# cchao0116/EasyDGL

Hardware: AMD Instinct MI355X
Metric: sequences/sec (fwd+bwd+Adam) B=512 L=100 d=128 |I|=20K (higher is better)
Workload: dtype bf16

## Files before the change

easydgl_amd/_lib.py:

```python
from __future__ import annotations

import ctypes
import os
from ctypes import c_char_p, c_float, c_int, c_int64, c_long, c_uint32, c_uint64, c_void_p

import torch

_HERE = os.path.dirname(os.path.abspath(__file__))
LIB_PATH = os.environ.get("EDGL_LIB_PATH") or os.path.join(_HERE, "libeasydgl_hip.so")

F32, BF16 = 0, 1
EPI_BIAS, EPI_GELU, EPI_SAVE_PRE, EPI_MUL_DGELU, EPI_ACCUM, EPI_OUT_F32, EPI_RELU = 1, 2, 4, 8, 16, 32, 64
MAU_CAUSAL, MAU_NO_DIAG, MAU_DIAG_ZERO = 1, 2, 4
MAU_NO_SKIP = 8
MAU_STREAM = 16
TATTN_CAUSAL = 1
LOSS_SOFTMAX, LOSS_BCE, LOSS_BPR = 0, 1, 2
TATTN_ORDERED = 2

P, I, F, L, U32, I64, U64 = c_void_p, c_int, c_float, c_long, c_uint32, c_int64, c_uint64

SIGNATURES = {
    "edgl_last_error": (c_char_p, []),
    "edgl_version": (I, []),
    "edgl_profile_next": (I, [I, P, P]),
    "edgl_rng_advance": (I, [P, P]),
    "edgl_mask_random": (I, [P, I, I, I, I64, P, U32, P, P, P, P]),
    "edgl_mask_last": (I, [P, I, I, I64, P, P]),
    "edgl_loader_state_words": (I, []),
    "edgl_loader_batch": (I, [P, P, P, L, I, I, I, I, I64, P, U32, P, P, P, P, P]),
    "edgl_loader_advance": (I, [P, I, P]),
    "edgl_encode_fwd": (I, [P, P, P, P, P, P, P, I, I, I, I, I, I64, F, F, P, U32, P, P, P, I, P]),
    "edgl_encode_bwd_workspace": (L, [I, I, I]),
    "edgl_encode_bwd": (I, [P, P, P, I, I, I, I, I, F, P, U32, P, P, P, P, I, P]),
    "edgl_encode_bwd_add": (I, [P, P, P, P, P, I, I, I, I, I, F, P, U32, P, P, P, P, I, P]),
    "edgl_encode_fwd_ct": (I, [P, P, P, P, P, P, P, I, I, I, I, I, I64, F, F, P, U32, P, P, P, I, I, I, P]),
    "edgl_encode_fwd_prep": (I, [P, P, P, P, P, P, P, I, I, I, I, I, I64, F, F, P, U32, P, P, P, I, I, P, I, P, P, P, P, P, P, I, P]),
    "edgl_encode_bwd_add_ct": (I, [P, P, P, P, P, I, I, I, I, I, F, P, U32, P, P, P, P, I, I, P]),
    "edgl_encode_bwd_label_fused": (I, [I, I]),
    "edgl_encode_bwd_add_label": (I, [P, P, P, P, P, I, I, I, I, I, F, P, U32, P, P, P, P, I, P, P, P, P, I, P, I, P]),
    "edgl_dx_encode_supported": (I, [I, I, I, I]),
    "edgl_dx_encode_bwd_label": (I, [P, P, I, I, P, P, P, P, P, I, I, I, I, I, F, P, U32, P, P, P, P, I, P, P, P, P, I, P, I, P]),
    "edgl_segsum_passes": (I, [I]),
    "edgl_segsum_plan_bytes": (L, [I, I]),
    "edgl_segsum_plan": (I, [P, I, P, I, I, I, P, P]),
    "edgl_encode_bwd_add_det": (I, [P, P, P, P, P, I, I, I, I, I, F, P, U32, P, P, P, P, I, P, I, P]),
    "edgl_embed_pos_fwd": (I, [P, P, P, P, P, I, I, I, I, F, F, P, U32, P, P, P, I, P]),
    "edgl_embed_pos_bwd": (I, [P, P, I, I, I, I, F, P, U32, P, P, I, P]),
    "edgl_embed_pos_fwd_ct": (I, [P, P, P, P, P, I, I, I, I, F, F, P, U32, P, P, P, I, I, P]),
    "edgl_embed_pos_bwd_ct": (I, [P, P, I, I, I, I, F, P, U32, P, P, I, I, P]),
    "edgl_embed_pos_bwd_det": (I, [P, P, I, I, I, I, F, P, U32, P, P, I, P, I, P]),
    "edgl_gemm": (I, [P, P, P, I, I, I, I, I, I, I, I, P, P, I, I, P, I, P]),
    "edgl_colsum": (I, [P, I, I, I, P, I, P, I, I, P]),
    "edgl_gemm_dw_workspace": (L, [I, I, I, I]),
    "edgl_gemm_dw": (I, [P, P, P, P, I, I, I, I, I, I, P, I, P]),
    "edgl_gemm_dw_defer": (I, [I, P]),
    "edgl_gemm_dw_ride": (I, [I]),
    "edgl_bimau_pack_bytes": (L, [I, I, I, I]),
    "edgl_bimau_pack": (I, [P, P, P, P, I, I, I, P, I, P]),
    "edgl_bimau_saved_bytes": (L, [I, I, I, I, I]),
    "edgl_bimau_saved_bytes_ex": (L, [I, I, I, I, I, I]),
    "edgl_bimau_form": (I, [I, I, I, I, I]),
    "edgl_bimau_bwd_workspace_ex": (L, [I, I, I, I, I, I, I]),
    "edgl_bimau_mark_group": (I, [I, I, I]),
    "edgl_bimau_fwd": (I, [P, P, I, P, P, P, P, I, I, I, I, I, F, P, U32, P, P, P, I, I, P]),
    "edgl_bimau_fwd_zr": (I, [P, P, I, P, P, P, P, I, I, I, I, I, F, P, U32, P, P, P, P, I, I, P]),
    "edgl_bimau_dropbits_bytes": (L, [I, I, I]),
    "edgl_bimau_dropbits": (I, [I, I, I, F, P, U32, P, P]),
    "edgl_bimau_fwd_db": (I, [P, P, I, P, P, P, P, I, I, I, I, I, F, P, U32, P, F, P, P, P, P, I, I, P]),
    "edgl_bimau_bwd_db": (I, [P, P, P, P, P, P, P, P, P, I, I, I, I, I, F, P, U32, P, F, P, P, P, P, P, P, I, I, P]),
    "edgl_bimau_job_order": (I, [P, I, I, P, P]),
    "edgl_bimau_fwd_ord": (I, [P, P, I, P, P, P, P, I, I, I, I, I, F, P, U32, P, F, P, P, P, P, P, I, I, P]),
    "edgl_bimau_bwd_ord": (I, [P, P, P, P, P, P, P, P, I, P, F, P, P, P, I, I, I, I, I, F, P, U32, P, F, P, P, P, P, P, P, P, I, I, P]),
    "edgl_bimau_bwd_workspace": (L, [I, I, I, I, I, I]),
    "edgl_bimau_bwd": (I, [P, P, P, P, P, P, P, P, P, I, I, I, I, I, F, P, U32, P, P, P, P, P, P, I, I, P]),
    "edgl_add_layernorm_fwd": (I, [P, P, I, P, P, I, I, I, F, P, U32, P, I, P, P, I, P]),
    "edgl_add_layernorm_bwd": (I, [P, P, I, P, P, P, I, I, I, F, P, U32, P, I, P, P, P, P, P, P, I, P]),
    "edgl_add_layernorm_bwd_act": (I, [P, P, I, P, P, P, I, I, I, F, P, U32, P, I, P, P, P, P, P, P, P, I, P]),
    "edgl_add_layernorm_fwd_ct": (I, [P, P, I, P, P, I, I, I, F, P, U32, P, I, P, P, I, I, I, P]),
    "edgl_add_layernorm_bwd_act_ct": (I, [P, P, I, P, P, P, I, I, I, F, P, U32, P, I, P, P, P, P, P, P, P, I, I, I, P]),
    "edgl_score_chunks": (I, [I, I]),
    "edgl_compact_rows": (I, [P, P, I, I, P, P, P, P, P, I, P]),
    "edgl_compact_scan": (I, [P, I, P, P, P, P]),
    "edgl_compact_scan_labels": (I, [P, I, P, P, P, P, P]),
    "edgl_compact_gather": (I, [P, P, P, I, I, P, P, I, P]),
    "edgl_scatter_rows": (I, [P, P, I, I, P, I, P]),
    "edgl_score_lse_fwd": (I, [P, P, P, P, I, I, I, I, I, P, P, P, P, P, I, P]),
    "edgl_ce_loss_fwd": (I, [P, P, P, I, P, P, P]),
    "edgl_ce_loss_fwd_add": (I, [P, P, P, I, P, P, P, P, P]),
    "edgl_ce_loss_fwd_add_w": (I, [P, P, P, I, P, P, P, P, P, P]),
    "edgl_score_bwd_workspace": (L, [I, I, I, I, I]),
    "edgl_score_ce_bwd": (I, [P, P, P, P, P, P, P, I, I, I, I, I, P, P, P, P, P, I, P]),
    "edgl_score_flash_workspace": (L, [I, I, I, I, I]),
    "edgl_score_flash_fwd": (I, [P, P, P, P, I, I, I, I, I, P, P, P, P, I, P]),
    "edgl_score_prepare_table": (I, [P, I, I, I, I, I, P, I, P]),
    "edgl_score_flash_fwd_pre": (I, [P, P, P, P, I, I, I, I, I, P, P, P, P, I, I, P]),
    "edgl_score_flash_fwd_coef": (I, [P, P, P, P, I, I, I, P, P, P, P, P, I, P]),
    "edgl_score_flash_fwd_coef_w": (I, [P, P, P, P, I, I, I, P, P, P, P, P, P, I, P]),
    "edgl_score_flash_fwd_rows_w": (I, [P, P, P, P, I, I, I, P, P, P, P, P, P, P, P, I, P]),
    "edgl_score_ce_nparts": (I, [I, I]),
    "edgl_score_flash_fwd_rows_wp": (I, [P, P, P, P, I, I, I, P, P, P, P, P, P, P, P, P, I, P]),
    "edgl_ce_loss_parts": (I, [P, I, P, P, P, P, P]),
    "edgl_score_flash_bwd": (I, [P, P, P, P, P, P, P, I, I, I, I, I, P, P, P, P, P, I, P]),
    "edgl_score_flash_bwd_ex": (I, [P, P, P, P, P, P, P, I, I, I, I, I, P, P, P, P, P, I, I, P]),
    "edgl_score_flash_label_term": (I, [P, P, P, P, I, I, I, I, I, P, P, P, I, P]),
    "edgl_score_flash_label_term_det": (I, [P, P, P, P, I, I, I, I, I, P, P, P, P, I, P]),
    "edgl_reduce_defer": (I, [I, P]),
    "edgl_reduce_flush": (I, [P]),
    "edgl_reduce_partials": (I, [P, I, I, L, P, I, P]),
    "edgl_reduce_ride": (I, [I]),
    "edgl_mask_topk": (I, [P, I, I, I, P, I, I, P, P, P]),
    "edgl_score_topk_fused_supported": (I, [I, I, I, I, I, I]),
    "edgl_score_topk_fused_workspace": (L, [I, I, I, I, I]),
    "edgl_score_topk_fused": (I, [P, P, P, P, I, I, I, I, I, I, I, P, P, P, I, P]),
    "edgl_score_rank_supported": (I, [I, I, I, I, I]),
    "edgl_score_rank_workspace": (L, [I, I, I, I]),
    "edgl_score_rank_slices": (I, [I, I, I, I]),
    "edgl_score_label_value": (I, [P, P, P, P, I, P, I, I, I, P, I, P]),
    "edgl_score_rank_fused": (I, [P, P, P, P, I, P, P, I, I, I, I, I, P, P, I, P]),
    "edgl_label_value_tile": (I, [P, I, I, I, P, I, P, P, P]),
    "edgl_rank_count_tile": (I, [P, I, I, I, P, I, P, P, P, P]),
    "edgl_rank_metrics_from_rank": (I, [P, I, P, I, P, P]),
    "edgl_score_candidates_chunk": (I, [I, I, I, I]),
    "edgl_score_candidates": (I, [P, P, P, P, P, I, P, I, I, I, I, P, P, P, I, P]),
    "edgl_sample_negatives": (I, [P, I, P, I, I, I, I, I, U64, U64, I, P, P]),
    "edgl_sample_negatives_alias": (I, [P, I, P, I, I, I, I, I, P, U64, U64, I, P, P]),
# ... 182 lines not shown
```

easydgl_amd/csrc/bimau_bwd_impl.h:

```cpp
#pragma once
#include <algorithm>

#include "bimau_common.h"

#ifdef EDGL_PHASE_TIMING
extern __device__ unsigned long long g_phase_cycles[16];
#endif

namespace bimau {


constexpr int KY_ECH = 8;
constexpr int KY_NY = EP / KY_ECH;
constexpr int KY_BLOCKS = 384;

constexpr int WG_NJ64 = 4;
constexpr int big_nj(int dh) { return dh == 64 ? WG_NJ64 : 32 / (dh / 16); }
inline int big_row_splits(int dh, int E) {
    const int nc = big_nj(dh) * 16;
    const int groups = std::max(1, (dh * E + nc - 1) / nc);
    return std::max(16, 512 / groups);
}

struct WsLayout { size_t dz, dh, rowdot, dsc, wpart, total; };
inline WsLayout ws_layout(int B, int T_, int C, int H, int E, long dsc_rows = 0) {
    const int dh = C / H;
    const bool big = dh >= 64;
    const size_t R = (size_t)B * H * T_;
    WsLayout w;
    size_t o = 0;
    auto take = [&](size_t bytes) { const size_t at = o; o += (bytes + 255) & ~(size_t)255; return at; };
    w.dz = take(R * EP * sizeof(float));
    w.dh = take((size_t)(big ? 1 : KY_NY) * R * dh * sizeof(float));
    w.rowdot = take(R * sizeof(float));
    w.dsc = take((size_t)(dsc_rows > 0 ? dsc_rows : (long)B * H) * EP * sizeof(float));
    w.wpart = take((size_t)(big ? big_row_splits(dh, E) : KY_BLOCKS) * ((size_t)(dh + 3) * dh * E + EP) * sizeof(float));
    w.total = o;
    return w;
}

struct BwdP {
    const void* qkvt; const int64_t* ids; const float* spans; const uint8_t* marks; const char* pack;
    const void* d_out; const float* d_lam_ext; const float* lam; const float* z; const void* hin;
    int B, T, C, H, E;
    float rate; const uint64_t* rng; uint32_t stream_id;
    void* d_qkvt;
    float* dz_ws; float* dh_ws; float* rowdot_ws; float* dsc_part; float* wpart;
    int waves;
    int flags;
    int noskip;
    const uint32_t* dbits;
    float qk_scale;
    const void* tpp_desc; int tpp_M; const float* tpp_sums; float tpp_coef;
    const int32_t* order;
    float* tpp_part;
};

template <typename T>
__device__ __forceinline__ void st_frag(T* dst, const f32x4& a) {
    Frag4<T> f = frag_from_acc<T>(a);
    if constexpr (sizeof(T) == 4) *reinterpret_cast<uint4*>(dst) = *reinterpret_cast<uint4*>(&f);
    else *reinterpret_cast<uint2*>(dst) = *reinterpret_cast<uint2*>(&f);
}

template <typename T, int DT, int NT, int EC, bool PREF = true, int FL = -1, bool DB = false, bool TP = false, bool SK = false>
__global__ __launch_bounds__(256) void bimau_bwd_sweep1_kernel(BwdP p) {
    constexpr int dh = 16 * DT, Tp = 16 * NT, LDT = Tp + 4;
    extern __shared__ __attribute__((aligned(16))) char smem[];
    const int E = EC ? EC : p.E;
    const int lane = threadIdx.x & 63, wave = __builtin_amdgcn_readfirstlane(threadIdx.x >> 6);
    const long slot = (long)blockIdx.x * p.waves + wave;
    if (slot >= (long)p.B * p.H) return;
    const int sb = (int)(slot / p.H), head = (int)(slot % p.H);
    const int b = p.order ? __builtin_amdgcn_readfirstlane(p.order[sb]) : sb;
    const long job = (long)b * p.H + head;
    const long bp = (long)head * p.B + b;
    const int g4 = (lane >> 4) * 4, l15 = lane & 15;
    constexpr bool SWZ = img_swz<T>();
    const int g4s = SWZ ? swz_col<16>(l15, g4) : g4;
    int cw[DT];
#pragma unroll
    for (int ub = 0; ub < DT; ++ub) cw[ub] = SWZ ? swz_col<16 * DT>(l15, ub * 16 + g4) : ub * 16 + g4;

    constexpr bool TR = sizeof(T) == 2;
    constexpr size_t EXTRA = TR ? 0 : (size_t)EP * LDT;
    constexpr size_t MASK_ELEMS = (size_t)Tp * sizeof(float) / sizeof(T);
    constexpr size_t WAVE_ELEMS = 2 * (size_t)Tp * dh + (size_t)Tp * EP + EXTRA + MASK_ELEMS;
    T* Ks = reinterpret_cast<T*>(smem) + (size_t)wave * WAVE_ELEMS;
    T* Vs = Ks + Tp * dh;
    T* Ms = Vs + Tp * dh;
    T* MTs = Ms + Tp * EP;
    const T* qkvt = reinterpret_cast<const T*>(p.qkvt) + (long)b * p.T * 4 * p.C;
    const T* dout = reinterpret_cast<const T*>(p.d_out) + (long)b * p.T * p.C;
    T* dqkvt = reinterpret_cast<T*>(p.d_qkvt) + (long)b * p.T * 4 * p.C;
    const int ldq = 4 * p.C;
    const KeyMask<NT> km = stage_wave<T, DT, NT, EC>(
        qkvt + p.C + head * dh, Ks, nullptr, static_cast<const T*>(nullptr), static_cast<T*>(nullptr), static_cast<T*>(nullptr),
        qkvt + 2 * p.C + head * dh, Vs, nullptr, ldq, p.marks + (long)b * p.T * E, E, Ms, TR ? nullptr : MTs,
        p.ids + (long)b * p.T, reinterpret_cast<float*>(Ks + WAVE_ELEMS - MASK_ELEMS), p.T, LDT, lane);
    __builtin_amdgcn_fence(__ATOMIC_RELEASE, "wavefront");
    __builtin_amdgcn_wave_barrier();

    const PackDims pd = pack_dims<T>(dh, E);
    const float* iscs_g = reinterpret_cast<const float*>(p.pack + pd.off_f32) + 3 * pd.JE + EP;
    float isc[4];
#pragma unroll
    for (int i = 0; i < 4; ++i) isc[i] = iscs_g[g4 + i];

    const float cscale = p.qk_scale > 0.f ? p.qk_scale : rsqrtf((float)dh);
    const DropKey dk = make_dropkey(p.rng, p.stream_id, p.rate);
    const Frag4<T> ident = identity_frag<T>(lane);
    const f32x4 zero4 = {0.f, 0.f, 0.f, 0.f};

    struct QOps { Frag4<T> qf[DT], dof[DT]; float4 z; float lam[4], dlx[4]; uint32_t kb; uint32_t nmw; float spr; };
    const float* dlx_src = p.d_lam_ext ? p.d_lam_ext : p.lam;
    const float dlx_on = p.d_lam_ext ? 1.0f : 0.0f;
    TppDesc td{};
    int tp_novf = 0;
    float tp_k = 0.f;
    if constexpr (TP) {
        td = tpp_desc(p.tpp_desc, p.B, p.T, p.tpp_M);
        tp_novf = __builtin_amdgcn_readfirstlane(td.novf[b]);
        int cnt;
        if (p.tpp_sums) {
            cnt = reinterpret_cast<const int*>(p.tpp_sums)[4];
        } else {
            cnt = 0;
            for (int i = lane; i < p.B; i += 64) cnt += td.cntp[i];
            for (int o = 32; o > 0; o >>= 1) cnt += __shfl_xor(cnt, o, 64);
        }
        tp_k = -p.tpp_coef / ((float)cnt * (float)p.H);
        if (job == 0 && lane == 0) reinterpret_cast<int*>(p.tpp_part)[2 * p.B * p.H] = cnt;
    }
    auto load_q = [&](int qt) {
        QOps o;
        const int q = min(qt * 16 + l15, p.T - 1);
        const long row = bp * p.T + q;
#pragma unroll
        for (int ub = 0; ub < DT; ++ub) {
            o.qf[ub] = frag_ld<T>(qkvt + (long)q * ldq + head * dh + ub * 16 + g4);
            o.dof[ub] = frag_ld<T>(dout + (long)q * p.C + head * dh + ub * 16 + g4);
        }
        o.z = *reinterpret_cast<const float4*>(p.z + row * EP + g4);
        if constexpr (DB) o.kb = p.dbits[(bp * NT + qt) * 64 + lane];
        if constexpr (TP) {
            const float4 l4 = *reinterpret_cast<const float4*>(p.lam + row * EC + g4);
            o.lam[0] = l4.x; o.lam[1] = l4.y; o.lam[2] = l4.z; o.lam[3] = l4.w;
            o.dlx[0] = 0.f; o.dlx[1] = 0.f; o.dlx[2] = 0.f; o.dlx[3] = 0.f;
            o.nmw = td.nmw[((long)b * p.T + q) * 4 + (lane >> 4)];
            o.spr = td.spr[(long)b * p.T + q];
        } else if constexpr (EC == 16) {
            const float4 l4 = *reinterpret_cast<const float4*>(p.lam + row * EC + g4), d4 = *reinterpret_cast<const float4*>(dlx_src + row * EC + g4);
            o.lam[0] = l4.x; o.lam[1] = l4.y; o.lam[2] = l4.z; o.lam[3] = l4.w;
            o.dlx[0] = d4.x; o.dlx[1] = d4.y; o.dlx[2] = d4.z; o.dlx[3] = d4.w;
        } else {
#pragma unroll
            for (int i = 0; i < 4; ++i) {
                const int e = min(g4 + i, E - 1);
                o.lam[i] = p.lam[row * E + e];
                o.dlx[i] = dlx_src[row * E + e];
            }
        }
        return o;
    };
    auto mask_q = [&](QOps& o, bool ok) {
#pragma unroll
        for (int ub = 0; ub < DT; ++ub)
            if (!ok) o.dof[ub] = frag_zero<T>();
#pragma unroll
        for (int i = 0; i < 4; ++i) {
            const bool oke = ok && (EC == 16 || (g4 + i) < E);
            o.lam[i] = oke ? o.lam[i] : 0.f;
            o.dlx[i] = oke ? o.dlx[i] * dlx_on : 0.f;
        }
    };
    PH_DECL
    auto run = [&](auto nk_c) {
    constexpr int NK = decltype(nk_c)::value, K0 = NT - NK;
    const KeyMask<NK> kmk = keymask_tail<NK, NT>(km);
    float dsc_acc[4] = {0.f, 0.f, 0.f, 0.f}, tp_a = 0.f, tp_b = 0.f;
    f32x4 dVa[DT][NK];
#pragma unroll
    for (int u = 0; u < DT; ++u)
#pragma unroll
        for (int kt = 0; kt < NK; ++kt) dVa[u][kt] = zero4;
    QOps qcur = load_q(0);
    touch_regs(qcur);
    float pend_dz[4] = {0.f, 0.f, 0.f, 0.f}, pend_rowdot = 0.f;
    int pend_q = p.T;
    auto flush_pending = [&]() {
        if (pend_q < p.T) {
            *reinterpret_cast<float4*>(p.dz_ws + (bp * p.T + pend_q) * EP + g4) = make_float4(pend_dz[0], pend_dz[1], pend_dz[2], pend_dz[3]);
            if (lane < 16) p.rowdot_ws[bp * p.T + pend_q] = pend_rowdot;
        }
    };
    for (int qt = 0; qt < NT; ++qt) {
        asm volatile("" ::: "memory");
        const int q = qt * 16 + l15;
        const bool qok = q < p.T;
        QOps qnext;
        if constexpr (PREF) qnext = load_q(qt + 1 < NT ? qt + 1 : qt);
        asm volatile("" ::: "memory");
        mask_q(qcur, qok);
        if constexpr (TP) {
            float gr[4] = {0.f, 0.f, 0.f, 0.f};
            tpp_slot(qcur.lam, qcur.nmw, qcur.spr, qok && qcur.spr >= 0.f, tp_k, gr, tp_a, tp_b);
            for (int j = 0; j < tp_novf; ++j) {
                const int tj = td.ovf_pos[(long)b * td.M + j];
                if ((tj >> 4) != qt) continue;
                tpp_slot(qcur.lam, td.ovf_nm[((long)b * td.M + j) * 4 + (lane >> 4)], qcur.spr, qok && q == tj, tp_k, gr, tp_a, tp_b);
            }
#pragma unroll
            for (int i = 0; i < 4; ++i) qcur.dlx[i] = gr[i];
        }
        const float zq4[4] = {qcur.z.x, qcur.z.y, qcur.z.z, qcur.z.w};
        f32x4 s[NK];
#pragma unroll
        for (int kt = 0; kt < NK; ++kt) {
            f32x4 a = zero4;
#pragma unroll
            for (int ub = 0; ub < DT; ++ub)
                a = mma16(frag_ld<T>(Ks + ((K0 + kt) * 16 + l15) * dh + cw[ub]), qcur.qf[ub], a);
            s[kt] = a;
        }
        if constexpr (FL == 0) masked_softmax_impl<NK, false, false>(s, kmk, cscale, lane, q, dk.scale);
        else {
            masked_softmax<NK, 0>(s, kmk, cscale, lane, q, (p.flags & MAU_CAUSAL) != 0);
#pragma unroll
            for (int kt = 0; kt < NK; ++kt)
#pragma unroll
                for (int r = 0; r < 4; ++r) s[kt][r] *= dk.scale;
        }
        asm volatile("" ::: "memory");
        flush_pending();
        asm volatile("" ::: "memory");
        PH_MARK(0);
        Frag4<T> lf;
#pragma unroll
        for (int i = 0; i < 4; ++i) lf.v[i] = from_f32<T>(qcur.lam[i]);
        Frag4<T> dOT[DT];
#pragma unroll
        for (int vt = 0; vt < DT; ++vt) dOT[vt] = frag_from_acc<T>(mma16(qcur.dof[vt], ident, zero4));
        float rowdot = 0.f;
        f32x4 dlamT = zero4;
        const uint32_t dbase = (uint32_t)((bp * p.T + q) * p.T);
#pragma unroll
        for (int kt = 0; kt < NK; ++kt) {
            const f32x4 gacc = mma16(frag_ld<T>(Ms + ((K0 + kt) * 16 + l15) * EP + g4s), lf, zero4);
            f32x4 da = zero4;
#pragma unroll
            for (int vb = 0; vb < DT; ++vb)
                da = mma16(frag_ld<T>(Vs + ((K0 + kt) * 16 + l15) * dh + cw[vb]), qcur.dof[vb], da);
            f32x4 ap, dg, gv = gacc;
            const bool dtile = K0 + kt == qt && (FL == 0 || !(p.flags & MAU_NO_DIAG));
            if constexpr (FL == 0) {
#pragma unroll
                for (int r = 0; r < 4; ++r) gv[r] = (dtile && g4 + r == l15) ? 1.0f : gacc[r];
            } else if (dtile) {
#pragma unroll
                for (int r = 0; r < 4; ++r) gv[r] = (g4 + r == l15) ? ((p.flags & MAU_DIAG_ZERO) ? 0.0f : 1.0f) : gacc[r];
            }
            uint64_t hw = 0ull;
            if constexpr (!DB) hw = drop_hash_quad(dk, dbase + (K0 + kt) * 16 + g4);
            const bool keep[4] = {drop_quad_keep<0>(dk, hw), drop_quad_keep<1>(dk, hw), drop_quad_keep<2>(dk, hw), drop_quad_keep<3>(dk, hw)};
#pragma unroll
            for (int r = 0; r < 4; ++r) {
                float fp;
                if constexpr (DB) fp = keep_bit(qcur.kb, (K0 + kt) * 4 + r, s[kt][r]);
                else fp = keep[r] ? s[kt][r] : 0.f;
                ap[r] = gv[r] * fp;
                dg[r] = da[r] * fp;
                rowdot = fmaf(dg[r], gv[r], rowdot);
            }
            if constexpr (FL == 0) {
#pragma unroll
                for (int r = 0; r < 4; ++r) dg[r] = (dtile && g4 + r == l15) ? 0.f : dg[r];
            } else if (dtile) {
#pragma unroll
// ... 14 lines not shown
            dz4[i] = dl * sg;
            if (qok && (EC == 16 || (g4 + i) < E)) dsc_acc[i] += dl * (qcur.lam[i] - zq4[i] * sg);
        }
        pend_rowdot = group_sum4(rowdot);
#pragma unroll
        for (int i = 0; i < 4; ++i) pend_dz[i] = dz4[i];
        pend_q = q;
        if constexpr (PREF) qcur = qnext;
        else if (qt + 1 < NT) qcur = load_q(qt + 1);
        PH_MARK(2);
    }
#pragma unroll
    for (int i = 0; i < 4; ++i) {
        float v = dsc_acc[i];
        v += __shfl_xor(v, 1, 64); v += __shfl_xor(v, 2, 64); v += __shfl_xor(v, 4, 64); v += __shfl_xor(v, 8, 64);
        dsc_acc[i] = v;
    }
    if constexpr (TP) {
#pragma unroll
        for (int o = 1; o < 16; o <<= 1) { tp_a += __shfl_xor(tp_a, o, 64); tp_b += __shfl_xor(tp_b, o, 64); }
    }
    flush_pending();
    if constexpr (TP) {
        if (lane == 0) *reinterpret_cast<float2*>(p.tpp_part + job * 2) = make_float2(tp_a, tp_b);
    }
    if (l15 == 0) *reinterpret_cast<float4*>(p.dsc_part + job * EP + g4) = make_float4(dsc_acc[0], dsc_acc[1], dsc_acc[2], dsc_acc[3]);
#pragma unroll
    for (int kt = 0; kt < NT; ++kt) {
        const int k = kt * 16 + l15;
        if (k < p.T) {
#pragma unroll
            for (int ut = 0; ut < DT; ++ut) {
                T* dst = dqkvt + (long)k * ldq + 2 * p.C + head * dh + ut * 16 + g4;
                if constexpr (K0 > 0) {
                    if (kt < K0) st_frag<T>(dst, zero4);
                    else st_frag<T>(dst, dVa[ut][kt < K0 ? 0 : kt - K0]);
                } else {
                    st_frag<T>(dst, dVa[ut][kt]);
                }
            }
        }
    }
    };
    if constexpr (SK) {
        static_assert(FL == 0 && sizeof(T) == 2, "the key-tile skip exists for the bidirectional bf16 form");
        dispatch_nk<NT>(NT - km.kt0, run);
    } else {
        run(std::integral_constant<int, NT>{});
    }
    PH_MARK(3);
    PH_FLUSH(0);
}

template <typename T, int DT, int NT, int EC, int NYP = KY_NY, bool PREF = true, int FL = -1, bool DB = false, int US = 1, int SL = 0, bool SK = false>
__global__ __launch_bounds__(256) void bimau_bwd_sweep2_kernel(BwdP p) {
    constexpr int dh = 16 * DT, Tp = 16 * NT, LDT = Tp + 4;
    static_assert(DT % US == 0 && SL < US, "channel slices");
    constexpr int DTS = DT / US, U0 = SL * DTS;
    extern __shared__ __attribute__((aligned(16))) char smem[];
    const int E = EC ? EC : p.E;
    const int lane = threadIdx.x & 63, wave = __builtin_amdgcn_readfirstlane(threadIdx.x >> 6);
    const long slot = (long)blockIdx.x * p.waves + wave;
    if (slot >= (long)p.B * p.H) return;
    const int sb = (int)(slot / p.H), head = (int)(slot % p.H);
    const int b = p.order ? __builtin_amdgcn_readfirstlane(p.order[sb]) : sb;
    const long job = (long)b * p.H + head;
    const long bp = (long)head * p.B + b;
    const int g4 = (lane >> 4) * 4, l15 = lane & 15;
    constexpr bool SWZ = img_swz<T>();
    const int g4s = SWZ ? swz_col<16>(l15, g4) : g4;
    int cw[DT];
#pragma unroll
    for (int ub = 0; ub < DT; ++ub) cw[ub] = SWZ ? swz_col<16 * DT>(l15, ub * 16 + g4) : ub * 16 + g4;

    constexpr bool TR = sizeof(T) == 2;
    constexpr size_t EXTRA = TR ? 0 : (size_t)dh * LDT;
    constexpr size_t MASK_ELEMS = (size_t)Tp * sizeof(float) / sizeof(T);
    constexpr size_t WAVE_ELEMS = 3 * (size_t)Tp * dh + (size_t)Tp * EP + EXTRA + MASK_ELEMS;
    T* Ks = reinterpret_cast<T*>(smem) + (size_t)wave * WAVE_ELEMS;
    T* Ts = Ks + Tp * dh;
    T* Vs = Ts + Tp * dh;
    T* Ms = Vs + Tp * dh;
    T* KTs = Ms + Tp * EP;
    const T* qkvt = reinterpret_cast<const T*>(p.qkvt) + (long)b * p.T * 4 * p.C;
    const T* dout = reinterpret_cast<const T*>(p.d_out) + (long)b * p.T * p.C;
    const T* hin = reinterpret_cast<const T*>(p.hin);
    T* dqkvt = reinterpret_cast<T*>(p.d_qkvt) + (long)b * p.T * 4 * p.C;
    const int ldq = 4 * p.C;
    const KeyMask<NT> km = stage_wave<T, DT, NT, EC>(
        qkvt + p.C + head * dh, Ks, TR ? nullptr : KTs, qkvt + 3 * p.C + head * dh, Ts, static_cast<T*>(nullptr),
        qkvt + 2 * p.C + head * dh, Vs, static_cast<T*>(nullptr), ldq, p.marks + (long)b * p.T * E, E, Ms, static_cast<T*>(nullptr),
        p.ids + (long)b * p.T, reinterpret_cast<float*>(Ks + WAVE_ELEMS - MASK_ELEMS), p.T, LDT, lane);
    __builtin_amdgcn_fence(__ATOMIC_RELEASE, "wavefront");
    __builtin_amdgcn_wave_barrier();

    const float cscale = p.qk_scale > 0.f ? p.qk_scale : rsqrtf((float)dh);
    const DropKey dk = make_dropkey(p.rng, p.stream_id, p.rate);
    float cz = cscale;
    if constexpr (FL == 0) {
        bool real = false;
        for (int k = lane; k < Tp; k += 64) real |= km.madd[k] == 0.f;
        cz = __any(real) ? cscale : 0.f;
    }
    (void)cz;
    const Frag4<T> ident = identity_frag<T>(lane);
    const f32x4 zero4 = {0.f, 0.f, 0.f, 0.f};
    const long R = (long)p.B * p.H * p.T;

    struct QOps { Frag4<T> qf[DT], dof[DT], hf[DT]; float4 dHp[DT][NYP]; float lam[4], rowdot; uint32_t kb; };
    auto load_q = [&](int qt) {
        QOps o;
        const int q = min(qt * 16 + l15, p.T - 1);
        const long row = bp * p.T + q;
#pragma unroll
        for (int ub = 0; ub < DT; ++ub) {
            o.qf[ub] = frag_ld<T>(qkvt + (long)q * ldq + head * dh + ub * 16 + g4);
            o.dof[ub] = frag_ld<T>(dout + (long)q * p.C + head * dh + ub * 16 + g4);
            o.hf[ub] = frag_ld<T>(hin + row * dh + ub * 16 + g4);
#pragma unroll
            for (int y = 0; y < NYP; ++y)
                o.dHp[ub][y] = *reinterpret_cast<const float4*>(p.dh_ws + ((long)y * R + row) * dh + ub * 16 + g4);
        }
        if constexpr (EC == 16) {
            const float4 l4 = *reinterpret_cast<const float4*>(p.lam + row * EC + g4);
            o.lam[0] = l4.x; o.lam[1] = l4.y; o.lam[2] = l4.z; o.lam[3] = l4.w;
        } else {
#pragma unroll
            for (int i = 0; i < 4; ++i) o.lam[i] = p.lam[row * E + min(g4 + i, E - 1)];
        }
        o.rowdot = p.rowdot_ws[row];
        if constexpr (DB) o.kb = p.dbits[(bp * NT + qt) * 64 + lane];
        return o;
    };
    PH_DECL
#ifdef EDGL_PHASE_TIMING
    const unsigned long long clk_m0 = __builtin_readcyclecounter(), clk_r0 = wall_clock64();
#endif
    auto run = [&](auto nk_c) {
    constexpr int NK = decltype(nk_c)::value, K0 = NT - NK;
    const KeyMask<NK> kmk = keymask_tail<NK, NT>(km);
    f32x4 dKa[DTS][NK], dTa[DTS][NK];
#pragma unroll
    for (int u = 0; u < DTS; ++u)
#pragma unroll
        for (int kt = 0; kt < NK; ++kt) { dKa[u][kt] = zero4; dTa[u][kt] = zero4; }
    QOps qcur = load_q(0);
    touch_regs(qcur);
    Frag4<T> pend_dq[DTS];
    int pend_q = p.T;
    auto flush_pending = [&]() {
        if (pend_q < p.T) {
#pragma unroll
            for (int ut = 0; ut < DTS; ++ut) {
                T* dst = dqkvt + (long)pend_q * ldq + head * dh + (U0 + ut) * 16 + g4;
                if constexpr (sizeof(T) == 4) *reinterpret_cast<uint4*>(dst) = *reinterpret_cast<uint4*>(&pend_dq[ut]);
                else *reinterpret_cast<uint2*>(dst) = *reinterpret_cast<uint2*>(&pend_dq[ut]);
            }
        }
    };
#pragma unroll
    for (int ut = 0; ut < DTS; ++ut) pend_dq[ut] = frag_zero<T>();
    for (int qt = 0; qt < NT; ++qt) {
        asm volatile("" ::: "memory");
        const int q = qt * 16 + l15;
        const bool qok = q < p.T;
        (void)qok;
        QOps qnext;
        if constexpr (PREF) qnext = load_q(qt + 1 < NT ? qt + 1 : qt);
        asm volatile("" ::: "memory");
        PH_MARK(3);
        f32x4 dHq[DT];
#pragma unroll
        for (int ub = 0; ub < DT; ++ub) {
            f32x4 a = zero4;
#pragma unroll
            for (int y = 0; y < NYP; ++y) {
                a[0] += qcur.dHp[ub][y].x; a[1] += qcur.dHp[ub][y].y; a[2] += qcur.dHp[ub][y].z; a[3] += qcur.dHp[ub][y].w;
            }
#pragma unroll
            for (int r = 0; r < 4; ++r) dHq[ub][r] = qok ? a[r] : 0.f;
            if (!qok) qcur.dof[ub] = frag_zero<T>();
        }
        const float rowdot1 = qok ? qcur.rowdot : 0.f;
        PH_MARK(4);
        f32x4 s[NK];
#pragma unroll
        for (int kt = 0; kt < NK; ++kt) {
            f32x4 a = zero4;
#pragma unroll
            for (int ub = 0; ub < DT; ++ub)
                a = mma16(frag_ld<T>(Ks + ((K0 + kt) * 16 + l15) * dh + cw[ub]), qcur.qf[ub], a);
            s[kt] = a;
        }
        PH_MARK(5);
        if constexpr (FL == 0) masked_softmax_impl<NK, false, false>(s, kmk, cscale, lane, q);
        else masked_softmax<NK, 0>(s, kmk, cscale, lane, q, (p.flags & MAU_CAUSAL) != 0);
        asm volatile("" ::: "memory");
        flush_pending();
        asm volatile("" ::: "memory");
        PH_MARK(0);
        Frag4<T> lf;
#pragma unroll
        for (int i = 0; i < 4; ++i) lf.v[i] = from_f32<T>((EC == 16 || (g4 + i) < E) ? qcur.lam[i] * dk.scale : 0.f);
        float rowdot = 0.f;
        Frag4<T> dhf[DT], QT[DTS], dHT[DTS];
#pragma unroll
        for (int ut = 0; ut < DT; ++ut) {
#pragma unroll
            for (int r = 0; r < 4; ++r) rowdot = fmaf(dHq[ut][r], to_f32(qcur.hf[ut].v[r]), rowdot);
            dhf[ut] = frag_from_acc<T>(dHq[ut]);
        }
#pragma unroll
        for (int ut = 0; ut < DTS; ++ut) {
            QT[ut] = frag_from_acc<T>(mma16(qcur.qf[U0 + ut], ident, zero4));
            dHT[ut] = frag_from_acc<T>(transpose_tile<T>(dHq[U0 + ut], ident));
        }
        rowdot = group_sum4(rowdot) + rowdot1;
        f32x4 dQ[DTS];
#pragma unroll
        for (int ut = 0; ut < DTS; ++ut) dQ[ut] = zero4;
        const uint32_t dbase = (uint32_t)((bp * p.T + q) * p.T);
#pragma unroll
        for (int kt = 0; kt < NK; ++kt) {
            const f32x4 gacc = mma16(frag_ld<T>(Ms + ((K0 + kt) * 16 + l15) * EP + g4s), lf, zero4);
            f32x4 da = zero4;
#pragma unroll
            for (int vb = 0; vb < DT; ++vb)
                da = mma16(frag_ld<T>(Vs + ((K0 + kt) * 16 + l15) * dh + cw[vb]), qcur.dof[vb], da);
            f32x4 gv = gacc;
            if constexpr (FL == 0) {
                const bool dtile = K0 + kt == qt;
#pragma unroll
                for (int r = 0; r < 4; ++r) gv[r] = (dtile && g4 + r == l15) ? dk.scale : gacc[r];
            } else if (kt == qt && !(p.flags & MAU_NO_DIAG)) {
#pragma unroll
                for (int r = 0; r < 4; ++r) gv[r] = (g4 + r == l15) ? ((p.flags & MAU_DIAG_ZERO) ? 0.0f : dk.scale) : gacc[r];
            }
            uint64_t hw = 0ull;
            if constexpr (!DB) hw = drop_hash_quad(dk, dbase + (K0 + kt) * 16 + g4);
            const bool keep[4] = {drop_quad_keep<0>(dk, hw), drop_quad_keep<1>(dk, hw), drop_quad_keep<2>(dk, hw), drop_quad_keep<3>(dk, hw)};
            f32x4 a;
#pragma unroll
            for (int r = 0; r < 4; ++r) {
                if constexpr (DB) a[r] = keep_bit(qcur.kb, (K0 + kt) * 4 + r, da[r] * gv[r]);
                else a[r] = keep[r] ? da[r] * gv[r] : 0.f;
            }
#pragma unroll
            for (int ub = 0; ub < DT; ++ub)
// ... 99 lines not shown
```

easydgl_amd/csrc/bimau_common.h:

```cpp
#pragma once
#include <cstdlib>
#include <type_traits>

#include "edgl_common.h"

namespace bimau {

constexpr int EP = 16;
constexpr float NLOG2E = -1.4426950408889634f;

__device__ __forceinline__ float sigmoid_pre(float xs) { return fast_rcp(1.0f + __builtin_amdgcn_exp2f(xs)); }

constexpr int XW = 8;
struct PackDims {
    int dh, E, JE, LDW, LDR;
    size_t off_w1x, off_f32, off_w1r, fwd_bytes, bytes;
};
template <typename T>
__host__ __device__ inline PackDims pack_dims(int dh, int E) {
    PackDims d;
    d.dh = dh; d.E = E; d.JE = dh * E; d.LDW = dh + 4; d.LDR = d.JE + 4;
    size_t w1t = (size_t)d.JE * d.LDW * sizeof(T);
    w1t = (w1t + 15) & ~(size_t)15;
    const size_t w1x = sizeof(T) == 2 ? (size_t)d.JE * XW * sizeof(T) : 0;
// ... 129 lines not shown
#pragma unroll
    for (int i = NR - 1; i >= 0; --i)
        if (real[i] != 0ull) first = 64 * i + (int)__builtin_ctzll(real[i]);
    return first < 0 ? 0 : first >> 4;
}
template <int NK, int NT>
__device__ __forceinline__ KeyMask<NK> keymask_tail(const KeyMask<NT>& km) {
    constexpr int K0 = NT - NK;
    return KeyMask<NK>{km.madd + K0 * 16, km.pad >> (K0 * 4), 0};
}
inline bool bimau_skip_enabled() {
    return edgl_env_on("EDGL_BIMAU_SKIP");
}
template <int N, typename F>
__device__ __forceinline__ void dispatch_nk(int nk, F&& f) {
    if constexpr (N <= 1) {
        f(std::integral_constant<int, 1>{});
    } else {
        if (nk >= N) f(std::integral_constant<int, N>{});
        else dispatch_nk<N - 1>(nk, f);
    }
}
template <int NT>
__device__ __forceinline__ KeyMask<NT> load_keymask(const int64_t* ids_row, int T, int lane, float* lds_madd) {
    KeyMask<NT> km;
    km.pad = 0ull;
    km.madd = lds_madd;
    constexpr int NR = (16 * NT + 63) / 64;
    uint64_t padded[NR], real[NR];
#pragma unroll
    for (int i = 0; i < NR; ++i) {
        const int k = lane + 64 * i;
        const int64_t id = ids_row[min(k, T - 1)];
        const bool pd = k < T && id == 0;
        padded[i] = __ballot(pd);
        real[i] = __ballot(k < T && id != 0);
        if (k < 16 * NT) lds_madd[k] = k >= T ? -INFINITY : (pd ? -4294967296.0f : 0.f);
    }
    km.kt0 = first_real_tile<NR>(real);
    const int g4 = (lane >> 4) * 4;
#pragma unroll
    for (int kt = 0; kt < NT; ++kt) {
        const uint64_t nib = (padded[kt / 4] >> ((kt % 4) * 16 + g4)) & 0xfull;
        km.pad |= nib << (kt * 4);
    }
    return km;
}

constexpr int MAU_CAUSAL = 1;
constexpr int MAU_NO_DIAG = 2;
constexpr int MAU_DIAG_ZERO = 4;
typedef __attribute__((ext_vector_type(2))) float f32x2;
template <int NT, bool CAUSAL, bool VEC, bool NORM = true>
__device__ __forceinline__ float masked_softmax_impl(f32x4 (&s)[NT], const KeyMask<NT>& km, float cscale, int lane, int q, float post = 1.0f) {
    const float c2 = cscale * 1.4426950408889634f;
    float mx = -INFINITY;
    const float* mrow = km.madd + (lane >> 4) * 4;
#pragma unroll
    for (int kt = 0; kt < NT; ++kt) {
        const f32x4 m4 = *reinterpret_cast<const f32x4*>(mrow + kt * 16);
        f32x4 v;
        if constexpr (VEC) {
            v = s[kt] * f32x4{c2, c2, c2, c2} + m4;
        } else {
#pragma unroll
            for (int r = 0; r < 4; ++r) v[r] = fmaf(s[kt][r], c2, m4[r]);
        }
        if constexpr (CAUSAL) {
#pragma unroll
            for (int r = 0; r < 4; ++r)
                if (kt * 16 + (lane >> 4) * 4 + r > q && m4[r] != -INFINITY) v[r] = -4294967296.0f;
        }
        s[kt] = v;
        mx = fmaxf(fmaxf(mx, v[0]), fmaxf(v[1], fmaxf(v[2], v[3])));
    }
    mx = group_max4(mx);
    float sum;
    if constexpr (VEC) {
        const f32x4 mx4 = {mx, mx, mx, mx};
        f32x4 sum4 = {0.f, 0.f, 0.f, 0.f};
#pragma unroll
        for (int kt = 0; kt < NT; ++kt) {
            const f32x4 d = s[kt] - mx4;
            f32x4 e;
#pragma unroll
            for (int r = 0; r < 4; ++r) e[r] = __builtin_amdgcn_exp2f(d[r]);
            s[kt] = e;
            sum4 += e;
        }
        sum = (sum4[0] + sum4[1]) + (sum4[2] + sum4[3]);
    } else {
        sum = 0.f;
#pragma unroll
        for (int kt = 0; kt < NT; ++kt)
#pragma unroll
            for (int r = 0; r < 4; ++r) {
                const float e = __builtin_amdgcn_exp2f(s[kt][r] - mx);
                s[kt][r] = e;
                sum += e;
            }
    }
    sum = group_sum4(sum);
    const float inv = fast_rcp(sum);
    if constexpr (!NORM) return inv;
    const float f = inv * post;
#pragma unroll
    for (int kt = 0; kt < NT; ++kt) {
        if constexpr (VEC) {
            s[kt] *= f32x4{f, f, f, f};
        } else {
#pragma unroll
            for (int r = 0; r < 4; ++r) s[kt][r] *= f;
        }
    }
    return inv;
}
template <int NT, int MODE = 0>
__device__ __forceinline__ void masked_softmax(f32x4 (&s)[NT], const KeyMask<NT>& km, float cscale, int lane, int q = 0,
                                               bool causal = false) {
    if constexpr (MODE != 0) {
        if (causal) masked_softmax_impl<NT, true, false>(s, km, cscale, lane, q);
        else masked_softmax_impl<NT, false, false>(s, km, cscale, lane, q);
    } else {
        const float c2 = cscale * 1.4426950408889634f;
        float mx = -INFINITY;
        const float* mrow = km.madd + (lane >> 4) * 4;
#pragma unroll
        for (int kt = 0; kt < NT; ++kt) {
            const float4 m4 = *reinterpret_cast<const float4*>(mrow + kt * 16);
            const float mm[4] = {m4.x, m4.y, m4.z, m4.w};
#pragma unroll
            for (int r = 0; r < 4; ++r) {
                float v = fmaf(s[kt][r], c2, mm[r]);
                if (causal && kt * 16 + (lane >> 4) * 4 + r > q && mm[r] != -INFINITY) v = -4294967296.0f;
                s[kt][r] = v;
                mx = fmaxf(mx, v);
            }
        }
        mx = group_max4(mx);
        float sum = 0.f;
#pragma unroll
        for (int kt = 0; kt < NT; ++kt)
#pragma unroll
            for (int r = 0; r < 4; ++r) {
                const float e = __builtin_amdgcn_exp2f(s[kt][r] - mx);
                s[kt][r] = e;
                sum += e;
            }
        sum = group_sum4(sum);
        const float inv = fast_rcp(sum);
#pragma unroll
        for (int kt = 0; kt < NT; ++kt)
#pragma unroll
            for (int r = 0; r < 4; ++r) s[kt][r] *= inv;
    }
}

template <int I>
__device__ __forceinline__ float keep_bit_c(uint32_t kb, float x) {
    int m;
    asm("v_bfe_i32 %0, %1, %2, 1" : "=v"(m) : "v"(kb), "n"(I));
    return __int_as_float(__float_as_int(x) & m);
}
__device__ __forceinline__ float keep_bit(uint32_t kb, int i, float x) {
    switch (i) {
#define EDGL_KB_CASE(n) case n: return keep_bit_c<n>(kb, x);
        EDGL_KB_CASE(0) EDGL_KB_CASE(1) EDGL_KB_CASE(2) EDGL_KB_CASE(3) EDGL_KB_CASE(4) EDGL_KB_CASE(5) EDGL_KB_CASE(6) EDGL_KB_CASE(7)
        EDGL_KB_CASE(8) EDGL_KB_CASE(9) EDGL_KB_CASE(10) EDGL_KB_CASE(11) EDGL_KB_CASE(12) EDGL_KB_CASE(13) EDGL_KB_CASE(14) EDGL_KB_CASE(15)
        EDGL_KB_CASE(16) EDGL_KB_CASE(17) EDGL_KB_CASE(18) EDGL_KB_CASE(19) EDGL_KB_CASE(20) EDGL_KB_CASE(21) EDGL_KB_CASE(22) EDGL_KB_CASE(23)
        EDGL_KB_CASE(24) EDGL_KB_CASE(25) EDGL_KB_CASE(26) EDGL_KB_CASE(27) EDGL_KB_CASE(28) EDGL_KB_CASE(29) EDGL_KB_CASE(30) EDGL_KB_CASE(31)
#undef EDGL_KB_CASE
    }
    return x;
}
template <int NT>
__global__ __launch_bounds__(256) void dropbits_kernel(const uint64_t* rng, uint32_t stream_id, float rate, int T, long njobs, uint32_t* bits) {
    static_assert(NT <= 8, "one 32-bit word per lane and query tile");
    const int lane = threadIdx.x & 63;
    const long job = (long)blockIdx.x * 4 + (threadIdx.x >> 6);
    if (job >= njobs) return;
    const long bp = job / NT;
    const int qt = (int)(job % NT), q = qt * 16 + (lane & 15), g4 = (lane >> 4) * 4;
    const DropKey dk = make_dropkey(rng, stream_id, rate);
    const uint32_t dbase = (uint32_t)((bp * T + q) * T);
    uint32_t w = 0u;
#pragma unroll
    for (int kt = 0; kt < NT; ++kt) {
        const uint64_t hw = drop_hash_quad(dk, dbase + kt * 16 + g4);
        w |= (drop_quad_keep<0>(dk, hw) ? 1u : 0u) << (kt * 4);
        w |= (drop_quad_keep<1>(dk, hw) ? 1u : 0u) << (kt * 4 + 1);
        w |= (drop_quad_keep<2>(dk, hw) ? 1u : 0u) << (kt * 4 + 2);
        w |= (drop_quad_keep<3>(dk, hw) ? 1u : 0u) << (kt * 4 + 3);
    }
    bits[job * 64 + lane] = w;
}

struct TppDesc {
    const uint32_t* nmw;
    const float* spr;
    const int32_t* novf;
    const int32_t* ovf_pos;
    const uint32_t* ovf_nm;
    const int32_t* cntp;
    int M;
};
struct TppLayout { size_t off_spr, off_novf, off_ovf_pos, off_ovf_nm, off_cntp, bytes; };
__host__ __device__ inline TppLayout tpp_layout(int B, int T, int M) {
    TppLayout l;
    l.off_spr = (size_t)B * T * 16;
// ... 283 lines not shown
```

easydgl_amd/csrc/bimau_fwd_impl.h:

```cpp
#pragma once
#include <type_traits>

#include "bimau_common.h"

namespace bimau {

constexpr int FWD_WAVES = 2;

struct FwdP {
    const void* qkvt; const void* resid; int ld_res;
    const int64_t* ids; const float* spans; const uint8_t* marks;
    const char* pack;
    int B, T, C, H, E;
    float rate; const uint64_t* rng; uint32_t stream_id;
    void* out; float* lam;
    void* hin_out; float* z_out;
    float* zero_rows;
    int waves;
    int flags;
    const uint32_t* dbits;
    float qk_scale;
    const int32_t* order;
    int noskip;
};

template <typename T, int DT, int NT, int PHASE>
__host__ __device__ constexpr size_t fwd_wave_bytes() {
    constexpr size_t dh = 16 * DT, Tp = 16 * NT, LDT = Tp + 4;
    constexpr size_t kv = sizeof(T) == 2 ? Tp * dh : dh * LDT;
    return (Tp * dh + (PHASE != 2 ? kv : 0) + (PHASE != 1 ? kv : 0) + (PHASE != 1 ? Tp * EP : 0)) * sizeof(T) + Tp * sizeof(float);
}

template <typename T, int DT, int NT, int EC, int PHASE = 0, bool DB = false, bool SK = false>
__global__ __launch_bounds__(256, (sizeof(T) == 2 && DT == 1 && EC == 16 && PHASE == 0) ? FWD_WAVES : 1) void bimau_fwd_kernel(FwdP p) {
    constexpr int dh = 16 * DT, Tp = 16 * NT, LDT = Tp + 4;
    extern __shared__ __attribute__((aligned(16))) char smem[];
    const int E = EC ? EC : p.E;
    constexpr bool FUSED = PHASE == 0, HAS_T = PHASE != 2, HAS_V = PHASE != 1, HAS_M = PHASE != 1;
    const PackDims pd = pack_dims<T>(dh, E);
    const size_t pack_bytes = FUSED ? pd.fwd_bytes : 0;
    if constexpr (FUSED) copy_pack_to_lds(smem, p.pack, pd.fwd_bytes);
    const T* W1T = reinterpret_cast<const T*>(smem);
    const T* W1X = reinterpret_cast<const T*>(smem + pd.off_w1x);
    const float* fW = reinterpret_cast<const float*>(smem + pd.off_f32);
    const float* w1s = fW; const float* b1s = fW + pd.JE; const float* wvs = fW + 2 * pd.JE;
    const float* scs = fW + 3 * pd.JE; const float* iscs = scs + EP;
    (void)W1T; (void)W1X; (void)w1s; (void)b1s; (void)wvs; (void)scs; (void)iscs;
    if constexpr (FUSED) __syncthreads();

    const int lane = threadIdx.x & 63, wave = __builtin_amdgcn_readfirstlane(threadIdx.x >> 6);
    const long slot = (long)blockIdx.x * p.waves + wave;
    if (slot >= (long)p.B * p.H) return;
    const int sb = (int)(slot / p.H), head = (int)(slot % p.H);
    const int b = p.order ? __builtin_amdgcn_readfirstlane(p.order[sb]) : sb;
    const long job = (long)b * p.H + head;
    const long bp = (long)head * p.B + b;

    constexpr bool TR = sizeof(T) == 2;
    constexpr size_t KV_ELEMS = TR ? (size_t)Tp * dh : (size_t)dh * LDT;
    constexpr size_t MASK_ELEMS = (size_t)Tp * sizeof(float) / sizeof(T);
    constexpr size_t WAVE_ELEMS = (size_t)Tp * dh + (HAS_T ? KV_ELEMS : 0) + (HAS_V ? KV_ELEMS : 0) + (HAS_M ? (size_t)Tp * EP : 0) + MASK_ELEMS;
    static_assert(WAVE_ELEMS * sizeof(T) == fwd_wave_bytes<T, DT, NT, PHASE>(), "host / device LDS layouts differ");
    T* Ks = reinterpret_cast<T*>(smem + pack_bytes) + (size_t)wave * WAVE_ELEMS;
    T* Ts = Ks + Tp * dh;
    T* Vs = Ts + (HAS_T ? KV_ELEMS : 0);
    T* Ms = Vs + (HAS_V ? KV_ELEMS : 0);
    const T* qkvt = reinterpret_cast<const T*>(p.qkvt) + (long)b * p.T * 4 * p.C;
    const int ldq = 4 * p.C;
    const KeyMask<NT> km = stage_wave<T, DT, NT, EC>(
        qkvt + p.C + head * dh, Ks, nullptr,
        HAS_T ? qkvt + 3 * p.C + head * dh : nullptr, TR ? Ts : nullptr, TR ? nullptr : Ts,
        HAS_V ? qkvt + 2 * p.C + head * dh : nullptr, TR ? Vs : nullptr, TR ? nullptr : Vs, ldq,
        HAS_M ? p.marks + (long)b * p.T * E : nullptr, E, Ms, nullptr, p.ids + (long)b * p.T,
        reinterpret_cast<float*>(Ms + (HAS_M ? Tp * EP : 0)), p.T, LDT, lane);
    __builtin_amdgcn_fence(__ATOMIC_RELEASE, "wavefront");
    __builtin_amdgcn_wave_barrier();
// ... 10 lines not shown
    struct QOps { Frag4<T> qf[DT], rf[DT]; float span; float lam[4]; uint32_t kb; };
    auto load_q = [&](int qt) {
        QOps o;
        const int q = min(qt * 16 + l15, p.T - 1);
#pragma unroll
        for (int ub = 0; ub < DT; ++ub) {
            o.qf[ub] = frag_ld<T>(qkvt + (long)q * ldq + head * dh + ub * 16 + g4);
            o.rf[ub] = frag_ld<T>(reinterpret_cast<const T*>(p.resid) + ((long)b * p.T + q) * p.ld_res + head * dh + ub * 16 + g4);
        }
        o.span = p.spans[(long)b * p.T + q];
        if constexpr (DB) o.kb = p.dbits[(bp * NT + qt) * 64 + lane];
        if constexpr (PHASE == 2) {
#pragma unroll
            for (int i = 0; i < 4; ++i) o.lam[i] = p.lam[(bp * p.T + q) * E + min(g4 + i, E - 1)];
        }
        return o;
    };
    auto run = [&](auto nk_c) {
    constexpr int NK = decltype(nk_c)::value, K0 = NT - NK;
    const KeyMask<NK> kmk = keymask_tail<NK, NT>(km);
    QOps qcur = load_q(0);
    touch_regs(qcur);
    Frag4<T> pend_o[DT];
#pragma unroll
    for (int ut = 0; ut < DT; ++ut) pend_o[ut] = frag_zero<T>();
    int pend_q = p.T;
    auto flush_pending = [&]() {
        if (pend_q < p.T) {
#pragma unroll
            for (int ut = 0; ut < DT; ++ut) {
                T* dst = reinterpret_cast<T*>(p.out) + ((long)b * p.T + pend_q) * p.C + head * dh + ut * 16 + g4;
                if constexpr (sizeof(T) == 4) *reinterpret_cast<uint4*>(dst) = *reinterpret_cast<uint4*>(&pend_o[ut]);
                else *reinterpret_cast<uint2*>(dst) = *reinterpret_cast<uint2*>(&pend_o[ut]);
            }
        }
    };
    for (int qt = 0; qt < NT; ++qt) {
        const int q = qt * 16 + l15;
        const bool qok = q < p.T;
        const QOps qnext = load_q(qt + 1 < NT ? qt + 1 : qt);
        asm volatile("" ::: "memory");
        Frag4<T> qf[DT];
#pragma unroll
        for (int ub = 0; ub < DT; ++ub) qf[ub] = qcur.qf[ub];
        f32x4 s[NK];
#pragma unroll
        for (int kt = 0; kt < NK; ++kt) {
            f32x4 a = {0.f, 0.f, 0.f, 0.f};
#pragma unroll
            for (int ub = 0; ub < DT; ++ub)
                a = mma16(frag_ld<T>(Ks + ((K0 + kt) * 16 + l15) * dh + cw[ub]), qf[ub], a);
            s[kt] = a;
        }
        float pinv = 1.0f;
        if constexpr (TR) {
            if constexpr (K0 == 0) {
                if (p.flags & MAU_CAUSAL) pinv = masked_softmax_impl<NT, true, false, false>(s, kmk, cscale, lane, q);
                else pinv = masked_softmax_impl<NT, false, false, false>(s, kmk, cscale, lane, q);
            } else {
                pinv = masked_softmax_impl<NK, false, false, false>(s, kmk, cscale, lane, q);
            }
        } else {
            masked_softmax<NT, 0>(s, kmk, cscale, lane, q, (p.flags & MAU_CAUSAL) != 0);
        }
        const float gfac = pinv * dk.scale;
        asm volatile("" ::: "memory");
        flush_pending();
        asm volatile("" ::: "memory");
        Frag4<T> pf[NK];
#pragma unroll
        for (int kt = 0; kt < NK; ++kt) pf[kt] = frag_from_acc<T>(s[kt]);
        Frag4<T> hf[DT];
        if constexpr (HAS_T) {
#pragma unroll
            for (int ut = 0; ut < DT; ++ut) {
                f32x4 a = {0.f, 0.f, 0.f, 0.f};
#pragma unroll
                for (int kt = 0; kt < NK; ++kt)
                    a = mma16(kfrag<T, SWZ ? 16 * DT : 0>(Ts, dh, Ts, LDT, (K0 + kt) * 16, ut * 16, lane), pf[kt], a);
                if constexpr (TR) {
#pragma unroll
                    for (int r = 0; r < 4; ++r) a[r] *= pinv;
                }
                hf[ut] = frag_from_acc<T>(a);
                if (p.hin_out && qok) {
                    T* dst = reinterpret_cast<T*>(p.hin_out) + (bp * p.T + q) * dh + ut * 16 + g4;
                    if constexpr (sizeof(T) == 4) *reinterpret_cast<uint4*>(dst) = *reinterpret_cast<uint4*>(&hf[ut]);
                    else *reinterpret_cast<uint2*>(dst) = *reinterpret_cast<uint2*>(&hf[ut]);
                }
            }
        }
        if constexpr (PHASE == 1) {
            qcur = qnext;
            continue;
        }
        Frag4<T> lf;
        if constexpr (FUSED) {
        const float span = qcur.span;
        float zp[16];
        struct MlpOps { Frag4<T> w[DT]; Frag4<T> wx; f32x4 ws, bs, wv; };
        Frag4<T> sf;
        if constexpr (TR) sf = span_frag(span, lane);
        auto load_ops = [&](int jt) {
            MlpOps o;
#pragma unroll
            for (int ub = 0; ub < DT; ++ub) o.w[ub] = frag_ld<T>(W1T + (jt * 16 + l15) * pd.LDW + ub * 16 + g4);
            if constexpr (TR) {
                o.wx = frag_ld<T>(W1X + (jt * 16 + l15) * XW + (g4 & 4));
            } else {
                o.ws = *reinterpret_cast<const f32x4*>(w1s + jt * 16 + g4);
                o.bs = *reinterpret_cast<const f32x4*>(b1s + jt * 16 + g4);
            }
            o.wv = *reinterpret_cast<const f32x4*>(wvs + jt * 16 + g4);
// ... 12 lines not shown
        };
        auto tile_post = [&](const f32x4& a, const MlpOps& o, float& acc, bool first) {
            float sg[4];
#pragma unroll
            for (int r = 0; r < 4; ++r) sg[r] = fast_rcp(1.0f + __builtin_amdgcn_exp2f(a[r]));
            acc = first ? sg[0] * o.wv[0] : fmaf(sg[0], o.wv[0], acc);
#pragma unroll
            for (int r = 1; r < 4; ++r) acc = fmaf(sg[r], o.wv[r], acc);
        };
        if constexpr (EC == 16) {
            MlpOps c0 = load_ops(0), c1 = load_ops(1);
            MlpOps n0 = load_ops(2), n1 = load_ops(3);
            f32x4 a0 = tile_pre(c0), a1 = tile_pre(c1);
            float zacc;
#pragma unroll
            for (int jt = 0; jt < 16 * DT; jt += 2) {
                const int jn = jt + 4 < 16 * DT ? jt + 4 : jt;
                const MlpOps m0 = load_ops(jn), m1 = load_ops(jn + 1);
                EDGL_PIN();
                f32x4 b0 = a0, b1 = a1;
                if (jt + 2 < 16 * DT) { b0 = tile_pre(n0); b1 = tile_pre(n1); }
                const int e0 = jt / DT, e1 = (jt + 1) / DT;
                tile_post(a0, c0, zacc, jt % DT == 0);
                if (e1 != e0) zp[e0] = zacc;
                tile_post(a1, c1, zacc, (jt + 1) % DT == 0);
                if ((jt + 2) % DT == 0) zp[e1] = zacc;
                c0 = n0; c1 = n1; n0 = m0; n1 = m1; a0 = b0; a1 = b1;
                EDGL_PIN();
            }
        } else {
            MlpOps cur = load_ops(0);
#pragma unroll
            for (int e = 0; e < 16; ++e) {
                zp[e] = 0.f;
                if (e < E) {
                    float zacc;
#pragma unroll
                    for (int d = 0; d < DT; ++d) {
                        const int jt = e * DT + d;
                        const MlpOps nxt = load_ops(jt + 1 < E * DT ? jt + 1 : jt);
                        EDGL_PIN();
                        const f32x4 a = tile_pre(cur);
                        tile_post(a, cur, zacc, d == 0);
                        cur = nxt;
                        EDGL_PIN();
                    }
                    zp[e] = zacc;
                }
            }
        }
        float z4[4];
        reduce_scatter16(zp, z4, lane);
        if (p.z_out && qok) *reinterpret_cast<float4*>(p.z_out + (bp * p.T + q) * EP + g4) = make_float4(z4[0], z4[1], z4[2], z4[3]);
        float lam4[4];
#pragma unroll
        for (int i = 0; i < 4; ++i) {
            const float sc = scs[g4 + i], isc = iscs[g4 + i];
            lam4[i] = sc * __logf(1.0f + __expf(z4[i] * isc));
            lf.v[i] = from_f32<T>(lam4[i] * gfac);
        }
        if (qok) {
            float* dst = p.lam + (bp * p.T + q) * E + g4;
            if constexpr (EC == 16) {
                *reinterpret_cast<float4*>(dst) = make_float4(lam4[0], lam4[1], lam4[2], lam4[3]);
                if (p.zero_rows) *reinterpret_cast<float4*>(p.zero_rows + (bp * p.T + q) * E + g4) = make_float4(0.f, 0.f, 0.f, 0.f);
            } else {
#pragma unroll
                for (int i = 0; i < 4; ++i)
                    if (g4 + i < E) { dst[i] = lam4[i]; if (p.zero_rows) p.zero_rows[(bp * p.T + q) * E + g4 + i] = 0.f; }
            }
        }
        } else {
#pragma unroll
            for (int i = 0; i < 4; ++i) lf.v[i] = from_f32<T>(qcur.lam[i] * gfac);
        }
        const uint32_t dbase = (uint32_t)((bp * p.T + q) * p.T);
        const bool set_diag = !(p.flags & MAU_NO_DIAG);
        const float dval = (p.flags & MAU_DIAG_ZERO) ? 0.0f : gfac;
        auto modulate = [&](auto drop_on) {
#pragma unroll
            for (int kt = 0; kt < NK; ++kt) {
                f32x4 gacc = mma16(frag_ld<T>(Ms + ((K0 + kt) * 16 + l15) * EP + g4s), lf, f32x4{0.f, 0.f, 0.f, 0.f});
                const bool dtile = set_diag && K0 + kt == qt;
#pragma unroll
                for (int r = 0; r < 4; ++r) {
                    gacc[r] = (dtile && g4 + r == l15) ? dval : gacc[r];
                    s[kt][r] = gacc[r] * s[kt][r];
                }
                if constexpr (decltype(drop_on)::value) {
                    if constexpr (DB) {
#pragma unroll
                        for (int r = 0; r < 4; ++r) s[kt][r] = keep_bit(qcur.kb, (K0 + kt) * 4 + r, s[kt][r]);
                    } else {
                        const uint64_t hw = drop_hash_quad(dk, dbase + (K0 + kt) * 16 + g4);
                        s[kt][0] = drop_quad_keep<0>(dk, hw) ? s[kt][0] : 0.f;
                        s[kt][1] = drop_quad_keep<1>(dk, hw) ? s[kt][1] : 0.f;
                        s[kt][2] = drop_quad_keep<2>(dk, hw) ? s[kt][2] : 0.f;
                        s[kt][3] = drop_quad_keep<3>(dk, hw) ? s[kt][3] : 0.f;
                    }
                }
                pf[kt] = frag_from_acc<T>(s[kt]);
            }
        };
        if (dk.thresh != 0u) modulate(std::true_type{});
        else modulate(std::false_type{});
#pragma unroll
// ... 84 lines not shown
```

easydgl_amd/csrc/k_bimau_bwd.hip:

```cpp
#include <algorithm>
#include <cstdlib>

#include "bimau_bwd_impl.h"

#ifdef EDGL_PHASE_TIMING
__device__ unsigned long long g_phase_cycles[16];
#endif

namespace {
using namespace bimau;

template <typename T>
constexpr int intensity_bwd_nreg(int DT) {
    return KY_ECH * DT * DT * 4 + (sizeof(T) == 2 ? (KY_ECH / 4) * DT * 4 : 2 * KY_ECH * DT) + KY_ECH * DT;
}

struct MlpP {
    const void* hin; const float* dz_ws; const float* spans; const char* pack;
    long R; int B, T, E; float* dh_ws; float* wpart; const float* dsc_part; long njobs;
    int slab_epi;
};

template <typename T, int DT, int EC>
__global__ __launch_bounds__(256, (sizeof(T) == 2 && DT == 1) ? 3 : 1) void intensity_bwd_kernel(MlpP p) {
// ... 292 lines not shown
size_t intensity_bwd_lds(int dh, int E) {
    const int NACC = dh * E * (dh + 4);
    return pack_dims<T>(dh, E).bytes + ((size_t)((NACC + 3) & ~3) + 4 * (16 * KY_ECH + 16)) * sizeof(float);
}

template <typename T, int DT>
int launch_intensity_bwd(const BwdP& p, long dsc_rows, hipStream_t st) {
    constexpr int dh = 16 * DT;
    MlpP mp{p.hin, p.dz_ws, p.spans, p.pack, (long)p.B * p.H * p.T, p.B, p.T, p.E, p.dh_ws, p.wpart, p.dsc_part, dsc_rows, 0};
    size_t smem_b = intensity_bwd_lds<T>(dh, p.E);
    const size_t slab_b = (size_t)4 * intensity_bwd_nreg<T>(DT) * 64 * sizeof(float);
    mp.slab_epi = slab_b <= std::max(smem_b, (size_t)52 * 1024);
    if (mp.slab_epi) smem_b = std::max(smem_b, slab_b);
    EDGL_REQUIRE(smem_b <= 160 * 1024, EDGL_ERR_SHAPE, "edgl_bimau_bwd: intensity kernel needs %zu B of LDS", smem_b);
    EDGL_REQUIRE((long)p.B * p.H * p.T < (1l << 31) - 16, EDGL_ERR_SHAPE, "edgl_bimau_bwd: B*H*T = %ld rows exceed the 32-bit row index", (long)p.B * p.H * p.T);
    auto kb = intensity_bwd_kernel<T, DT, 0>;
    EDGL_LDS_LIMIT(kb, smem_b, "edgl_bimau_bwd");
    hipLaunchKernelGGL(kb, dim3(KY_BLOCKS, KY_NY), dim3(256), smem_b, st, mp);
    EDGL_LAUNCH_CHECK();
    return EDGL_OK;
}

template <typename T, int DT, int NT>
int launch_bwd(BwdP p, char* ws, float* dW1, float* db1, float* dw, float* dscaling, hipStream_t st) {
    constexpr int dh = 16 * DT, Tp = 16 * NT, LDT = Tp + 4;
    const PackDims pd = pack_dims<T>(dh, p.E);
    const WsLayout wl = ws_layout(p.B, p.T, p.C, p.H, p.E);
    p.dz_ws = reinterpret_cast<float*>(ws + wl.dz); p.dh_ws = reinterpret_cast<float*>(ws + wl.dh);
    p.rowdot_ws = reinterpret_cast<float*>(ws + wl.rowdot);
    p.dsc_part = reinterpret_cast<float*>(ws + wl.dsc); p.wpart = reinterpret_cast<float*>(ws + wl.wpart);
    const long jobs = (long)p.B * p.H;
    constexpr bool TR = sizeof(T) == 2;
    edgl_prof_begin(EDGL_KERNEL_BIMAU_BWD_ALL, st);
    {
        const size_t wave_bytes = (2 * (size_t)Tp * dh + (size_t)Tp * EP + (TR ? 0 : (size_t)EP * LDT)) * sizeof(T) + (size_t)Tp * sizeof(float);
        int waves = 4;
        while (waves > 1 && waves * wave_bytes > 64 * 1024) waves >>= 1;
        const size_t smem = waves * wave_bytes;
        p.waves = waves;
        constexpr bool SPEC = sizeof(T) == 2 && DT == 1;
        auto kern = p.E == 16 ? bimau_bwd_sweep1_kernel<T, DT, NT, 16> : bimau_bwd_sweep1_kernel<T, DT, NT, 0>;
        if constexpr (SPEC) {
            if (p.flags == 0) kern = p.E == 16 ? bimau_bwd_sweep1_kernel<T, DT, NT, 16, true, 0> : bimau_bwd_sweep1_kernel<T, DT, NT, 0, true, 0>;
            if constexpr (NT <= 8) {
                constexpr bool SKC = NT >= 2;
                const bool sk = SKC && p.flags == 0 && p.E == 16 && bimau_skip_enabled() && !p.noskip;
                const bool db = p.dbits && p.rate > 0.f;
                if (p.flags == 0 && p.E == 16 && db) kern = sk ? bimau_bwd_sweep1_kernel<T, DT, NT, 16, true, 0, true, false, SKC> : bimau_bwd_sweep1_kernel<T, DT, NT, 16, true, 0, true>;
                else if (sk) kern = bimau_bwd_sweep1_kernel<T, DT, NT, 16, true, 0, false, false, SKC>;
                if (p.tpp_desc) {
                    if (sk) kern = db ? bimau_bwd_sweep1_kernel<T, DT, NT, 16, true, 0, true, true, SKC> : bimau_bwd_sweep1_kernel<T, DT, NT, 16, true, 0, false, true, SKC>;
                    else kern = db ? bimau_bwd_sweep1_kernel<T, DT, NT, 16, true, 0, true, true> : bimau_bwd_sweep1_kernel<T, DT, NT, 16, true, 0, false, true>;
                }
            }
        }
        EDGL_LDS_LIMIT(kern, smem, "edgl_bimau_bwd");
        hipLaunchKernelGGL(kern, dim3((unsigned)((jobs + waves - 1) / waves)), dim3(64 * waves), smem, st, p);
        EDGL_LAUNCH_CHECK();
    }
    {
        const int rc = launch_intensity_bwd<T, DT>(p, jobs, st);
        if (rc) return rc;
    }
    {
        const size_t wave_bytes = (3 * (size_t)Tp * dh + (size_t)Tp * EP + (TR ? 0 : (size_t)dh * LDT)) * sizeof(T) + (size_t)Tp * sizeof(float);
        int waves = 4;
        while (waves > 1 && waves * wave_bytes > 80 * 1024) waves >>= 1;
        const size_t smem = waves * wave_bytes;
        EDGL_REQUIRE(smem <= 160 * 1024, EDGL_ERR_SHAPE, "edgl_bimau_bwd: needs %zu B of LDS", smem);
        p.waves = waves;
        constexpr bool SPEC = sizeof(T) == 2 && DT == 1;
        auto kern = p.E == 16 ? bimau_bwd_sweep2_kernel<T, DT, NT, 16> : bimau_bwd_sweep2_kernel<T, DT, NT, 0>;
        if constexpr (SPEC) {
            if (p.flags == 0) kern = p.E == 16 ? bimau_bwd_sweep2_kernel<T, DT, NT, 16, KY_NY, true, 0> : bimau_bwd_sweep2_kernel<T, DT, NT, 0, KY_NY, true, 0>;
            if constexpr (NT <= 8) {
                constexpr bool SKC = NT >= 2;
                const bool sk = SKC && p.flags == 0 && p.E == 16 && bimau_skip_enabled() && !p.noskip;
                if (p.flags == 0 && p.E == 16 && p.dbits && p.rate > 0.f) kern = sk ? bimau_bwd_sweep2_kernel<T, DT, NT, 16, KY_NY, true, 0, true, 1, 0, SKC> : bimau_bwd_sweep2_kernel<T, DT, NT, 16, KY_NY, true, 0, true>;
                else if (sk) kern = bimau_bwd_sweep2_kernel<T, DT, NT, 16, KY_NY, true, 0, false, 1, 0, SKC>;
            }
        }
        EDGL_LDS_LIMIT(kern, smem, "edgl_bimau_bwd");
        edgl_prof_begin(EDGL_KERNEL_BIMAU_BWD, st);
        hipLaunchKernelGGL(kern, dim3((unsigned)((jobs + waves - 1) / waves)), dim3(64 * waves), smem, st, p);
        edgl_prof_end(EDGL_KERNEL_BIMAU_BWD, st);
        edgl_prof_end(EDGL_KERNEL_BIMAU_BWD_ALL, st);
        EDGL_LAUNCH_CHECK();
    }
    return reduce_wparts(p.wpart, KY_BLOCKS, dh, p.E, dW1, db1, dw, dscaling, st);
}

template <typename T, int DT>
int dispatch_nt(BwdP p, char* ws, float* dW1, float* db1, float* dw, float* dsc, hipStream_t st) {
    switch ((p.T + 15) / 16) {
        case 1: return launch_bwd<T, DT, 1>(p, ws, dW1, db1, dw, dsc, st);
        case 2: return launch_bwd<T, DT, 2>(p, ws, dW1, db1, dw, dsc, st);
        case 3: return launch_bwd<T, DT, 3>(p, ws, dW1, db1, dw, dsc, st);
        case 4: return launch_bwd<T, DT, 4>(p, ws, dW1, db1, dw, dsc, st);
        case 5: return launch_bwd<T, DT, 5>(p, ws, dW1, db1, dw, dsc, st);
        case 6: return launch_bwd<T, DT, 6>(p, ws, dW1, db1, dw, dsc, st);
        case 7: return launch_bwd<T, DT, 7>(p, ws, dW1, db1, dw, dsc, st);
        case 8: return launch_bwd<T, DT, 8>(p, ws, dW1, db1, dw, dsc, st);
        case 9: return launch_bwd<T, DT, 9>(p, ws, dW1, db1, dw, dsc, st);
        case 10: return launch_bwd<T, DT, 10>(p, ws, dW1, db1, dw, dsc, st);
        case 11: return launch_bwd<T, DT, 11>(p, ws, dW1, db1, dw, dsc, st);
        case 12: return launch_bwd<T, DT, 12>(p, ws, dW1, db1, dw, dsc, st);
        case 13: return launch_bwd<T, DT, 13>(p, ws, dW1, db1, dw, dsc, st);
    }
    edgl_set_error("edgl_bimau_bwd: T=%d not supported (T <= 208)", p.T);
    return EDGL_ERR_SHAPE;
}

}

namespace bimau {
int intensity_bwd_small(const BwdP& p, long dsc_rows, float* dW1, float* db1, float* dw, float* dsc, int dtype, hipStream_t st) {
    const bool f = dtype == EDGL_F32;
    const int dh = p.C / p.H;
    int rc;
    if (dh == 16) rc = f ? launch_intensity_bwd<float, 1>(p, dsc_rows, st) : launch_intensity_bwd<bf16, 1>(p, dsc_rows, st);
    else if (dh == 32) rc = f ? launch_intensity_bwd<float, 2>(p, dsc_rows, st) : launch_intensity_bwd<bf16, 2>(p, dsc_rows, st);
    else { edgl_set_error("edgl_bimau_bwd: head dim %d has no weights-in-LDS intensity backward (16 or 32)", dh); return EDGL_ERR_SHAPE; }
    if (rc) return rc;
    return reduce_wparts(p.wpart, KY_BLOCKS, dh, p.E, dW1, db1, dw, dsc, st);
}
}

extern "C" long edgl_bimau_bwd_workspace_ex(int B, int T, int C, int H, int E, int dtype, int flags) {
    if (H <= 0 || C % H) return -1;
    const int form = bimau::bimau_form(T, C, H, dtype == EDGL_BF16 ? EDGL_BF16 : EDGL_F32, flags);
    return (long)ws_layout_form(B, T, C, H, E, form).total;
}
extern "C" long edgl_bimau_bwd_workspace(int B, int T, int C, int H, int E, int dtype) {
    return edgl_bimau_bwd_workspace_ex(B, T, C, H, E, dtype, 0);
}

extern "C" int edgl_bimau_mark_group(int C, int H, int dtype) {
    if (H <= 0 || C % H || (dtype != EDGL_F32 && dtype != EDGL_BF16)) return -1;
    const int dh = C / H;
    if (dh >= 64) return bimau::EP;
    for (int E = bimau::EP; E >= 1; --E) {
        const size_t b = dtype == EDGL_BF16 ? intensity_bwd_lds<bf16>(dh, E) : intensity_bwd_lds<float>(dh, E);
        if (b <= 160 * 1024) return E;
    }
    return -1;
}

extern "C" int edgl_bimau_bwd_db(const void* qkvt, const int64_t* ids, const float* spans, const uint8_t* marks,
                                 const void* pack, const void* d_out, const float* d_lam_ext, const float* lam,
                                 const void* saved, int B, int T, int C, int H, int E, float drop_rate,
                                 const uint64_t* rng_state, uint32_t stream_id, const uint32_t* dropbits, float qk_scale, void* d_qkvt,
                                 float* dW1, float* db1, float* dw, float* dscaling, void* workspace, int flags, int dtype, void* stream);
extern "C" int edgl_bimau_bwd(const void* qkvt, const int64_t* ids, const float* spans, const uint8_t* marks,
                              const void* pack, const void* d_out, const float* d_lam_ext, const float* lam,
                              const void* saved, int B, int T, int C, int H, int E, float drop_rate,
                              const uint64_t* rng_state, uint32_t stream_id, void* d_qkvt, float* dW1, float* db1,
                              float* dw, float* dscaling, void* workspace, int flags, int dtype, void* stream) {
    return edgl_bimau_bwd_db(qkvt, ids, spans, marks, pack, d_out, d_lam_ext, lam, saved, B, T, C, H, E, drop_rate, rng_state, stream_id,
                             nullptr, 0.f, d_qkvt, dW1, db1, dw, dscaling, workspace, flags, dtype, stream);
}
static int bimau_bwd_impl(const void* qkvt, const int64_t* ids, const float* spans, const uint8_t* marks,
                          const void* pack, const void* d_out, const float* d_lam_ext, const float* lam,
                          const void* saved, int B, int T, int C, int H, int E, float drop_rate,
                          const uint64_t* rng_state, uint32_t stream_id, const uint32_t* dropbits, float qk_scale, void* d_qkvt,
                          float* dW1, float* db1, float* dw, float* dscaling, void* workspace, const void* tpp_desc, int tpp_M,
                          const float* tpp_sums, float tpp_coef, float* tpp_part, const int32_t* order, int flags, int dtype, void* stream) {
    EDGL_REQUIRE(qkvt && ids && spans && marks && pack && d_out && lam && saved && d_qkvt && dW1 && db1 && dw && dscaling && workspace,
                 EDGL_ERR_NULL, "edgl_bimau_bwd: null pointer");
    EDGL_REQUIRE(B > 0 && T > 0 && H > 0 && C % H == 0 && E >= 1 && E <= bimau::EP, EDGL_ERR_SHAPE,
                 "edgl_bimau_bwd: bad shape B=%d T=%d C=%d H=%d E=%d", B, T, C, H, E);
    EDGL_REQUIRE(dtype == EDGL_F32 || dtype == EDGL_BF16, EDGL_ERR_DTYPE, "edgl_bimau_bwd: bad dtype %d", dtype);
    EDGL_REQUIRE(drop_rate == 0.f || rng_state, EDGL_ERR_NULL, "edgl_bimau_bwd: dropout without rng_state");
    EDGL_REQUIRE((double)B * H * T * T < 4294967296.0, EDGL_ERR_SHAPE, "edgl_bimau_bwd: H*B*T*T must be < 2^32");
    BwdP p{};
    p.qkvt = qkvt; p.ids = ids; p.spans = spans; p.marks = marks; p.pack = (const char*)pack; p.d_out = d_out;
    p.d_lam_ext = d_lam_ext; p.lam = lam;
    const bimau::SavedLayout sl = bimau::saved_layout(B, T, C, H, dtype == EDGL_BF16 ? 2 : 4);
    p.hin = (const char*)saved + sl.off_hin;
    p.z = reinterpret_cast<const float*>((const char*)saved + sl.off_z);
    p.B = B; p.T = T; p.C = C; p.H = H; p.E = E; p.rate = drop_rate; p.rng = rng_state;
    p.noskip = (flags & EDGL_MAU_NO_SKIP) ? 1 : 0; flags &= ~EDGL_MAU_NO_SKIP;
    p.stream_id = stream_id; p.d_qkvt = d_qkvt; p.flags = flags; p.dbits = dropbits; p.qk_scale = qk_scale;
    p.tpp_desc = tpp_desc; p.tpp_M = tpp_M; p.tpp_sums = tpp_sums; p.tpp_coef = tpp_coef; p.tpp_part = tpp_part; p.order = order;
    EDGL_REQUIRE(!tpp_desc || (dtype == EDGL_BF16 && C / H == 16 && E == 16 && T <= 128 && flags == 0 && tpp_part && tpp_M > 0 && !d_lam_ext),
                 EDGL_ERR_SHAPE, "edgl_bimau_bwd_tpp: the fused TPP form exists for bf16, head dim 16, 16 marks, T <= 128, BiMAU flags "
                 "(C/H=%d E=%d T=%d flags=%d)", C / H, E, T, flags);
    hipStream_t st = (hipStream_t)stream;
    const int dh = C / H;
    char* ws = (char*)workspace;
    const int form = bimau::bimau_form(T, C, H, dtype, flags);
    p.flags = flags & ~EDGL_MAU_STREAM;
    if (form < 0) {
        edgl_set_error("edgl_bimau_bwd: head dim %d with T=%d not supported (head dims 16, 32, 64 or 128; T <= %d)", dh, T, bimau::STREAM_MAX_T);
        return EDGL_ERR_SHAPE;
    }
    if (form == 1) {
        EDGL_REQUIRE(!tpp_desc, EDGL_ERR_SHAPE, "edgl_bimau_bwd_tpp: the fused TPP form does not exist on the key-streamed path (T=%d, T <= 128)", T);
        const WsLayout wl = ws_layout_form(B, T, C, H, E, 1);
        p.dz_ws = reinterpret_cast<float*>(ws + wl.dz); p.dh_ws = reinterpret_cast<float*>(ws + wl.dh);
        p.rowdot_ws = reinterpret_cast<float*>(ws + wl.rowdot);
        p.dsc_part = reinterpret_cast<float*>(ws + wl.dsc); p.wpart = reinterpret_cast<float*>(ws + wl.wpart);
        const bimau::SavedLayoutStream ss = bimau::saved_layout_stream(B, T, C, H, dtype == EDGL_BF16 ? 2 : 4);
        return bimau::stream_bwd(p, reinterpret_cast<const float*>((const char*)saved + ss.off_stats), dW1, db1, dw, dscaling, dtype, st);
    }
    if (dtype == EDGL_F32) {
        if (dh == 16) return dispatch_nt<float, 1>(p, ws, dW1, db1, dw, dscaling, st);
        if (dh == 32) return dispatch_nt<float, 2>(p, ws, dW1, db1, dw, dscaling, st);
    } else {
        if (dh == 16) return dispatch_nt<bf16, 1>(p, ws, dW1, db1, dw, dscaling, st);
        if (dh == 32) return dispatch_nt<bf16, 2>(p, ws, dW1, db1, dw, dscaling, st);
    }
    if (dh == 64 || dh == 128) return bimau::big_bwd(p, ws, dW1, db1, dw, dscaling, dtype, st);
    edgl_set_error("edgl_bimau_bwd: head dim %d not supported (16, 32, 64 or 128)", dh);
    return EDGL_ERR_SHAPE;
}
extern "C" int edgl_bimau_bwd_db(const void* qkvt, const int64_t* ids, const float* spans, const uint8_t* marks,
                                 const void* pack, const void* d_out, const float* d_lam_ext, const float* lam,
                                 const void* saved, int B, int T, int C, int H, int E, float drop_rate,
                                 const uint64_t* rng_state, uint32_t stream_id, const uint32_t* dropbits, float qk_scale, void* d_qkvt,
                                 float* dW1, float* db1, float* dw, float* dscaling, void* workspace, int flags, int dtype, void* stream) {
    return bimau_bwd_impl(qkvt, ids, spans, marks, pack, d_out, d_lam_ext, lam, saved, B, T, C, H, E, drop_rate, rng_state, stream_id,
                          dropbits, qk_scale, d_qkvt, dW1, db1, dw, dscaling, workspace, nullptr, 0, nullptr, 0.f, nullptr, nullptr, flags, dtype, stream);
}
extern "C" int edgl_bimau_bwd_tpp(const void* qkvt, const int64_t* ids, const float* spans, const uint8_t* marks,
                                  const void* pack, const void* d_out, const void* tpp_desc, int M, const float* tpp_sums, float coef,
                                  float* tpp_part, const float* lam, const void* saved, int B, int T, int C, int H, int E, float drop_rate,
                                  const uint64_t* rng_state, uint32_t stream_id, const uint32_t* dropbits, float qk_scale, void* d_qkvt,
                                  float* dW1, float* db1, float* dw, float* dscaling, void* workspace, int flags, int dtype, void* stream) {
    EDGL_REQUIRE(tpp_desc && tpp_part, EDGL_ERR_NULL, "edgl_bimau_bwd_tpp: null pointer");
    return bimau_bwd_impl(qkvt, ids, spans, marks, pack, d_out, nullptr, lam, saved, B, T, C, H, E, drop_rate, rng_state, stream_id,
                          dropbits, qk_scale, d_qkvt, dW1, db1, dw, dscaling, workspace, tpp_desc, M, tpp_sums, coef, tpp_part, nullptr, flags, dtype,
                          stream);
}
extern "C" int edgl_bimau_bwd_ord(const void* qkvt, const int64_t* ids, const float* spans, const uint8_t* marks, const void* pack,
                                  const void* d_out, const float* d_lam_ext, const void* tpp_desc, int M, const float* tpp_sums, float coef,
                                  float* tpp_part, const float* lam, const void* saved, int B, int T, int C, int H, int E, float drop_rate,
                                  const uint64_t* rng_state, uint32_t stream_id, const uint32_t* dropbits, float qk_scale, void* d_qkvt,
                                  float* dW1, float* db1, float* dw, float* dscaling, void* workspace, const int32_t* order, int flags,
                                  int dtype, void* stream) {
    EDGL_REQUIRE(!tpp_desc || tpp_part, EDGL_ERR_NULL, "edgl_bimau_bwd_ord: tpp_desc without tpp_part");
    return bimau_bwd_impl(qkvt, ids, spans, marks, pack, d_out, d_lam_ext, lam, saved, B, T, C, H, E, drop_rate, rng_state, stream_id,
                          dropbits, qk_scale, d_qkvt, dW1, db1, dw, dscaling, workspace, tpp_desc, M, tpp_sums, coef, tpp_part, order, flags,
                          dtype, stream);
}

#ifdef EDGL_PHASE_TIMING
extern "C" int edgl_debug_phase_cycles(unsigned long long* out16, int reset) {
    if (hipMemcpyFromSymbol(out16, HIP_SYMBOL(g_phase_cycles), 16 * sizeof(unsigned long long)) != hipSuccess) return -1;
    if (reset) {
        unsigned long long z[16] = {0};
        if (hipMemcpyToSymbol(HIP_SYMBOL(g_phase_cycles), z, sizeof(z)) != hipSuccess) return -1;
    }
    return 0;
}
#endif
```

easydgl_amd/csrc/k_bimau_fwd.hip:

```cpp
#include "bimau_fwd_impl.h"

namespace {
using namespace bimau;

template <typename T>
int dispatch_dt(FwdP p, hipStream_t st) {
    const int dh = p.C / p.H;
    if (dh == 16) return dispatch_nt<T, 1>(p, st);
    if (dh == 32) return dispatch_nt<T, 2>(p, st);
    edgl_set_error("edgl_bimau_fwd: head dim %d not supported (16, 32, 64 or 128)", dh);
    return EDGL_ERR_SHAPE;
}

}

extern "C" long edgl_bimau_pack_bytes(int C, int H, int E, int dtype) {
    const int dh = C / (H > 0 ? H : 1);
    return (long)(dtype == EDGL_BF16 ? bimau::pack_dims<bf16>(dh, E).bytes : bimau::pack_dims<float>(dh, E).bytes);
}

extern "C" int edgl_bimau_form(int T, int C, int H, int dtype, int flags) {
    return bimau::bimau_form(T, C, H, dtype, flags);
}
extern "C" long edgl_bimau_saved_bytes_ex(int B, int T, int C, int H, int dtype, int flags) {
    if (H <= 0 || C % H) return -1;
    const size_t es = dtype == EDGL_BF16 ? 2 : 4;
    if (bimau::bimau_form(T, C, H, dtype == EDGL_BF16 ? EDGL_BF16 : EDGL_F32, flags) == 1) return (long)bimau::saved_layout_stream(B, T, C, H, es).bytes;
    return (long)bimau::saved_layout(B, T, C, H, es).bytes;
}
extern "C" long edgl_bimau_saved_bytes(int B, int T, int C, int H, int dtype) {
    return edgl_bimau_saved_bytes_ex(B, T, C, H, dtype, 0);
}

extern "C" int edgl_bimau_pack(const float* W1, const float* b1, const float* w, const float* scaling, int C, int H,
                               int E, void* pack, int dtype, void* stream) {
    EDGL_REQUIRE(W1 && b1 && w && scaling && pack, EDGL_ERR_NULL, "edgl_bimau_pack: null pointer");
    EDGL_REQUIRE(H > 0 && C % H == 0 && E >= 1 && E <= bimau::EP, EDGL_ERR_SHAPE, "edgl_bimau_pack: bad C=%d H=%d E=%d", C, H, E);
    const int dh = C / H;
    hipStream_t st = (hipStream_t)stream;
    if (dtype == EDGL_F32) hipLaunchKernelGGL((bimau::pack_kernel<float>), dim3(16), dim3(256), 0, st, W1, b1, w, scaling, dh, E, (char*)pack);
    else if (dtype == EDGL_BF16) hipLaunchKernelGGL((bimau::pack_kernel<bf16>), dim3(16), dim3(256), 0, st, W1, b1, w, scaling, dh, E, (char*)pack);
    else { edgl_set_error("edgl_bimau_pack: bad dtype %d", dtype); return EDGL_ERR_DTYPE; }
    EDGL_LAUNCH_CHECK();
    return EDGL_OK;
}

extern "C" int edgl_bimau_fwd_zr(const void* qkvt, const void* resid, int ld_res, const int64_t* ids, const float* spans,
                                 const uint8_t* marks, const void* pack, int B, int T, int C, int H, int E,
                                 float drop_rate, const uint64_t* rng_state, uint32_t stream_id, void* out,
                                 float* lam_out, void* saved, float* zero_rows, int flags, int dtype, void* stream);
extern "C" int edgl_bimau_fwd_db(const void* qkvt, const void* resid, int ld_res, const int64_t* ids, const float* spans,
                                 const uint8_t* marks, const void* pack, int B, int T, int C, int H, int E,
                                 float drop_rate, const uint64_t* rng_state, uint32_t stream_id, const uint32_t* dropbits, float qk_scale,
                                 void* out, float* lam_out, void* saved, float* zero_rows, int flags, int dtype, void* stream);

extern "C" int edgl_bimau_fwd_ord(const void* qkvt, const void* resid, int ld_res, const int64_t* ids, const float* spans,
                                  const uint8_t* marks, const void* pack, int B, int T, int C, int H, int E,
                                  float drop_rate, const uint64_t* rng_state, uint32_t stream_id, const uint32_t* dropbits, float qk_scale,
                                  void* out, float* lam_out, void* saved, float* zero_rows, const int32_t* order, int flags, int dtype,
                                  void* stream);

extern "C" long edgl_bimau_dropbits_bytes(int B, int T, int H) {
    if (B <= 0 || T <= 0 || H <= 0) return -1;
    const int nt = (T + 15) / 16;
    return nt <= 8 ? (long)B * H * nt * 64 * (long)sizeof(uint32_t) : 0;
}
extern "C" int edgl_bimau_dropbits(int B, int T, int H, float drop_rate, const uint64_t* rng_state, uint32_t stream_id,
                                   uint32_t* bits, void* stream) {
    EDGL_REQUIRE(rng_state && bits, EDGL_ERR_NULL, "edgl_bimau_dropbits: null pointer");
    EDGL_REQUIRE(B > 0 && T > 0 && H > 0 && T <= 128, EDGL_ERR_SHAPE, "edgl_bimau_dropbits: bad shape B=%d T=%d H=%d (T <= 128)", B, T, H);
    EDGL_REQUIRE((double)B * H * T * T < 4294967296.0, EDGL_ERR_SHAPE, "edgl_bimau_dropbits: H*B*T*T must be < 2^32");
    const int nt = (T + 15) / 16;
    const long njobs = (long)B * H * nt;
    const dim3 grid((unsigned)((njobs + 3) / 4));
    hipStream_t st = (hipStream_t)stream;
    switch (nt) {
#define EDGL_DB_CASE(N) case N: hipLaunchKernelGGL((bimau::dropbits_kernel<N>), grid, dim3(256), 0, st, rng_state, stream_id, drop_rate, T, njobs, bits); break;
        EDGL_DB_CASE(1) EDGL_DB_CASE(2) EDGL_DB_CASE(3) EDGL_DB_CASE(4) EDGL_DB_CASE(5) EDGL_DB_CASE(6) EDGL_DB_CASE(7) EDGL_DB_CASE(8)
#undef EDGL_DB_CASE
    }
    EDGL_LAUNCH_CHECK();
    return EDGL_OK;
}
extern "C" int edgl_bimau_fwd(const void* qkvt, const void* resid, int ld_res, const int64_t* ids, const float* spans,
                              const uint8_t* marks, const void* pack, int B, int T, int C, int H, int E,
                              float drop_rate, const uint64_t* rng_state, uint32_t stream_id, void* out,
                              float* lam_out, void* saved, int flags, int dtype, void* stream) {
    return edgl_bimau_fwd_zr(qkvt, resid, ld_res, ids, spans, marks, pack, B, T, C, H, E, drop_rate, rng_state, stream_id, out, lam_out,
                             saved, nullptr, flags, dtype, stream);
}
extern "C" int edgl_bimau_fwd_zr(const void* qkvt, const void* resid, int ld_res, const int64_t* ids, const float* spans,
                                 const uint8_t* marks, const void* pack, int B, int T, int C, int H, int E,
                                 float drop_rate, const uint64_t* rng_state, uint32_t stream_id, void* out,
                                 float* lam_out, void* saved, float* zero_rows, int flags, int dtype, void* stream) {
    return edgl_bimau_fwd_db(qkvt, resid, ld_res, ids, spans, marks, pack, B, T, C, H, E, drop_rate, rng_state, stream_id, nullptr, 0.f, out,
                             lam_out, saved, zero_rows, flags, dtype, stream);
}
extern "C" int edgl_bimau_fwd_db(const void* qkvt, const void* resid, int ld_res, const int64_t* ids, const float* spans,
                                 const uint8_t* marks, const void* pack, int B, int T, int C, int H, int E,
                                 float drop_rate, const uint64_t* rng_state, uint32_t stream_id, const uint32_t* dropbits, float qk_scale,
                                 void* out, float* lam_out, void* saved, float* zero_rows, int flags, int dtype, void* stream) {
    return edgl_bimau_fwd_ord(qkvt, resid, ld_res, ids, spans, marks, pack, B, T, C, H, E, drop_rate, rng_state, stream_id, dropbits, qk_scale,
                              out, lam_out, saved, zero_rows, nullptr, flags, dtype, stream);
}

namespace {
__global__ __launch_bounds__(256) void job_tiles_kernel(const int64_t* ids, int B, int T, int32_t* nk) {
    const int lane = threadIdx.x & 63, b = blockIdx.x * 4 + (threadIdx.x >> 6);
    if (b >= B) return;
    const int NT = (T + 15) / 16, NR = (T + 63) / 64;
    int first = -1;
    for (int r0 = 0; r0 < NR; r0 += 4) {
        int64_t v[4];
// ... 3 lines not shown
        for (int j = 3; j >= 0; --j) {
            const int k = lane + 64 * (r0 + j);
            const uint64_t real = __ballot(k < T && v[j] != 0);
            if (real != 0ull && (first < 0 || 64 * (r0 + j) < first)) first = 64 * (r0 + j) + (int)__builtin_ctzll(real);
        }
        if (first >= 0) break;
    }
    if (lane == 0) nk[b] = first < 0 ? NT : NT - (first >> 4);
}
constexpr int ORD_THREADS = 256;
__global__ __launch_bounds__(ORD_THREADS) void job_rank_kernel(const int32_t* nk, int B, int32_t* order) {
    extern __shared__ __attribute__((aligned(16))) int nk_s[];
    for (int b = threadIdx.x; b < B; b += ORD_THREADS) nk_s[b] = nk[b];
    __syncthreads();
    for (int b = threadIdx.x; b < B; b += ORD_THREADS) {
        const int mine = nk_s[b];
        int rank = 0;
        int o = 0;
        for (; o + 32 <= B; o += 32) {
            int4 v[8];
#pragma unroll
            for (int j = 0; j < 8; ++j) v[j] = *reinterpret_cast<const int4*>(nk_s + o + 4 * j);
#pragma unroll
            for (int j = 0; j < 8; ++j) {
                const int oo = o + 4 * j;
                rank += (v[j].x > mine || (v[j].x == mine && oo < b)) ? 1 : 0;
                rank += (v[j].y > mine || (v[j].y == mine && oo + 1 < b)) ? 1 : 0;
                rank += (v[j].z > mine || (v[j].z == mine && oo + 2 < b)) ? 1 : 0;
                rank += (v[j].w > mine || (v[j].w == mine && oo + 3 < b)) ? 1 : 0;
            }
        }
        for (; o < B; ++o) {
            const int v = nk_s[o];
            rank += (v > mine || (v == mine && o < b)) ? 1 : 0;
        }
        order[rank] = b;
    }
}
}
extern "C" int edgl_bimau_job_order(const int64_t* ids, int B, int T, int32_t* order, void* stream) {
    EDGL_REQUIRE(ids && order, EDGL_ERR_NULL, "edgl_bimau_job_order: null pointer");
    EDGL_REQUIRE(B > 0 && T > 0 && B <= 16384, EDGL_ERR_SHAPE, "edgl_bimau_job_order: bad shape B=%d T=%d (B <= 16384)", B, T);
    hipLaunchKernelGGL(job_tiles_kernel, dim3((B + 3) / 4), dim3(256), 0, (hipStream_t)stream, ids, B, T, order + B);
    hipLaunchKernelGGL(job_rank_kernel, dim3(1), dim3(ORD_THREADS), (size_t)((B + 3) & ~3) * sizeof(int), (hipStream_t)stream, order + B, B, order);
    EDGL_LAUNCH_CHECK();
    return EDGL_OK;
}

extern "C" int edgl_bimau_fwd_ord(const void* qkvt, const void* resid, int ld_res, const int64_t* ids, const float* spans,
                                  const uint8_t* marks, const void* pack, int B, int T, int C, int H, int E,
                                  float drop_rate, const uint64_t* rng_state, uint32_t stream_id, const uint32_t* dropbits, float qk_scale,
                                  void* out, float* lam_out, void* saved, float* zero_rows, const int32_t* order, int flags, int dtype,
                                  void* stream) {
    EDGL_REQUIRE(qkvt && resid && ids && spans && marks && pack && out && lam_out, EDGL_ERR_NULL,
                 "edgl_bimau_fwd: null pointer");
    EDGL_REQUIRE(B > 0 && T > 0 && H > 0 && C % H == 0 && E >= 1 && E <= bimau::EP, EDGL_ERR_SHAPE,
                 "edgl_bimau_fwd: bad shape B=%d T=%d C=%d H=%d E=%d", B, T, C, H, E);
    EDGL_REQUIRE(drop_rate == 0.f || rng_state, EDGL_ERR_NULL, "edgl_bimau_fwd: dropout without rng_state");
    EDGL_REQUIRE(ld_res % 4 == 0, EDGL_ERR_SHAPE, "edgl_bimau_fwd: ld_res must be a multiple of 4");
    EDGL_REQUIRE((double)B * H * T * T < 4294967296.0, EDGL_ERR_SHAPE, "edgl_bimau_fwd: H*B*T*T must be < 2^32");
    EDGL_REQUIRE(dtype == EDGL_F32 || dtype == EDGL_BF16, EDGL_ERR_DTYPE, "edgl_bimau_fwd: bad dtype %d", dtype);
    const int form = bimau::bimau_form(T, C, H, dtype, flags);
    flags &= ~EDGL_MAU_STREAM;
    FwdP p{qkvt, resid, ld_res, ids, spans, marks, (const char*)pack, B, T, C, H, E, drop_rate, rng_state, stream_id,
           out, lam_out, nullptr, nullptr, nullptr, 4, flags & ~EDGL_MAU_NO_SKIP, dropbits, qk_scale, order, (flags & EDGL_MAU_NO_SKIP) ? 1 : 0};
    flags &= ~EDGL_MAU_NO_SKIP;
    hipStream_t st = (hipStream_t)stream;
    if (form < 0) {
        edgl_set_error("edgl_bimau_fwd: head dim %d with T=%d not supported (head dims 16, 32, 64 or 128; T <= %d)", C / H, T, bimau::STREAM_MAX_T);
        return EDGL_ERR_SHAPE;
    }
    if (form == 1) {
        if (zero_rows && hipMemsetAsync(zero_rows, 0, (size_t)H * B * T * E * sizeof(float), st) != hipSuccess) {
            edgl_set_error("edgl_bimau_fwd: memset failed");
            return EDGL_ERR_LAUNCH;
        }
        float* stats = nullptr;
        if (saved) {
            const bimau::SavedLayoutStream ss = bimau::saved_layout_stream(B, T, C, H, dtype == EDGL_BF16 ? 2 : 4);
            p.hin_out = (char*)saved + ss.off_hin;
            p.z_out = reinterpret_cast<float*>((char*)saved + ss.off_z);
            stats = reinterpret_cast<float*>((char*)saved + ss.off_stats);
        }
        edgl_prof_begin(EDGL_KERNEL_BIMAU_FWD, st);
        const int rc = bimau::stream_fwd(p, stats, dtype, st);
        edgl_prof_end(EDGL_KERNEL_BIMAU_FWD, st);
        return rc;
    }
    if (C / H == 64 || C / H == 128) {
        if (zero_rows && hipMemsetAsync(zero_rows, 0, (size_t)H * B * T * E * sizeof(float), st) != hipSuccess) {
            edgl_set_error("edgl_bimau_fwd: memset failed");
            return EDGL_ERR_LAUNCH;
        }
    } else {
        p.zero_rows = zero_rows;
    }
    if (saved) {
        const bimau::SavedLayout sl = bimau::saved_layout(B, T, C, H, dtype == EDGL_BF16 ? 2 : 4);
        p.hin_out = (char*)saved + sl.off_hin;
        p.z_out = reinterpret_cast<float*>((char*)saved + sl.off_z);
    }
    EDGL_REQUIRE(dtype == EDGL_F32 || dtype == EDGL_BF16, EDGL_ERR_DTYPE, "edgl_bimau_fwd: bad dtype %d", dtype);
    edgl_prof_begin(EDGL_KERNEL_BIMAU_FWD, st);
    int rc;
    if (C / H == 64 || C / H == 128) rc = bimau::big_fwd(p, dtype, st);
    else if (dtype == EDGL_F32) rc = dispatch_dt<float>(p, st);
    else rc = dispatch_dt<bf16>(p, st);
    edgl_prof_end(EDGL_KERNEL_BIMAU_FWD, st);
    return rc;
}
```

easydgl_amd/csrc/k_bimau_stream.hip:

```cpp
#include "bimau_bwd_impl.h"
#include "bimau_fwd_impl.h"

namespace {
using namespace bimau;

constexpr float PAD_SCORE = -4294967296.0f;

template <typename T, int DT> constexpr bool stream_pref() { return sizeof(T) * DT <= 16; }

struct TileId { long bp; int b, head, t; };
__device__ __forceinline__ bool tile_of_wave(int B, int H, int NT, TileId& id) {
    const int wave = __builtin_amdgcn_readfirstlane(threadIdx.x >> 6);
    const long tile = (long)blockIdx.x * 4 + wave;
    if (tile >= (long)B * H * NT) return false;
    id.bp = tile / NT;
    id.t = (int)(tile - id.bp * NT);
    id.head = (int)(id.bp / B);
    id.b = (int)(id.bp - (long)id.head * B);
    return true;
}

__device__ __forceinline__ f32x4 key_madd(const int64_t* ids_row, int T, int kg) {
    f32x4 m;
#pragma unroll
// ... 127 lines not shown
__global__ __launch_bounds__(256) void stream_values_kernel(FwdP p, const float* stats) {
    constexpr int dh = 16 * DT;
    const int NT = (p.T + 15) / 16, E = p.E;
    TileId id;
    if (!tile_of_wave(p.B, p.H, NT, id)) return;
    const int lane = threadIdx.x & 63, g4 = (lane >> 4) * 4, l15 = lane & 15;
    const long ldq = 4 * (long)p.C;
    const T* qkvt = reinterpret_cast<const T*>(p.qkvt) + (long)id.b * p.T * ldq + id.head * dh + g4;
    const int64_t* ids = p.ids + (long)id.b * p.T;
    const uint8_t* marks = p.marks + (long)id.b * p.T * E;
    const int qt = id.t, q = qt * 16 + l15, qc = min(q, p.T - 1);
    const long row = id.bp * p.T + qc;
    const float cscale = p.qk_scale > 0.f ? p.qk_scale : rsqrtf((float)dh);
    const float c2 = cscale * 1.4426950408889634f;
    const bool causal = (p.flags & MAU_CAUSAL) != 0;
    const DropKey dk = make_dropkey(p.rng, p.stream_id, p.rate);
    const Frag4<T> ident = identity_frag<T>(lane);
    const f32x4 zero4 = {0.f, 0.f, 0.f, 0.f};
    Frag4<T> qf[DT], rf[DT];
    load_rows<T, DT>(qf, qkvt, ldq, q, p.T);
    load_rows<T, DT>(rf, reinterpret_cast<const T*>(p.resid) + (long)id.b * p.T * p.ld_res + id.head * dh + g4, p.ld_res, q, p.T);
    const float2 st = *reinterpret_cast<const float2*>(stats + row * 2);
    const float mx = st.x, gfac = st.y * dk.scale;
    Frag4<T> lf;
#pragma unroll
    for (int i = 0; i < 4; ++i) lf.v[i] = from_f32<T>(g4 + i < E ? p.lam[row * E + g4 + i] * gfac : 0.f);
    const bool set_diag = !(p.flags & MAU_NO_DIAG);
    const float dval = (p.flags & MAU_DIAG_ZERO) ? 0.0f : gfac;
    const uint32_t dbase = (uint32_t)((id.bp * p.T + q) * p.T);

    struct KOps { Frag4<T> kf[DT], vf[DT], mf; f32x4 madd; };
    auto load_k = [&](int kt) {
        KOps o;
        load_rows<T, DT>(o.kf, qkvt + p.C, ldq, kt * 16 + l15, p.T);
        load_rows<T, DT>(o.vf, qkvt + 2 * p.C, ldq, kt * 16 + l15, p.T);
        o.mf = marks_row_frag<T>(marks, E, p.T, kt * 16 + l15, g4);
        o.madd = key_madd(ids, p.T, kt * 16 + g4);
        return o;
    };
    f32x4 Oacc[DT];
#pragma unroll
    for (int vt = 0; vt < DT; ++vt) Oacc[vt] = zero4;
    KOps cur = load_k(0);
    for (int kt = 0; kt < NT; ++kt) {
        KOps nxt;
        if constexpr (stream_pref<T, DT>()) nxt = load_k(min(kt + 1, NT - 1));
        const f32x4 v = score_tile<T, DT>(cur.kf, qf, cur.madd, c2, causal, kt * 16 + g4, q);
        const f32x4 gacc = mma16(cur.mf, lf, zero4);
        const bool dtile = set_diag && kt == qt;
        f32x4 s;
#pragma unroll
        for (int r = 0; r < 4; ++r) {
            const float g = (dtile && g4 + r == l15) ? dval : gacc[r];
            s[r] = g * __builtin_amdgcn_exp2f(v[r] - mx);
        }
        if (dk.thresh != 0u) {
            bool keep[4];
            keep4<T>(dk, dbase + kt * 16 + g4, keep);
#pragma unroll
            for (int r = 0; r < 4; ++r) s[r] = keep[r] ? s[r] : 0.f;
        }
        const Frag4<T> pf = frag_from_acc<T>(s);
#pragma unroll
        for (int vt = 0; vt < DT; ++vt) Oacc[vt] = mma16(rows_to_contraction<T>(cur.vf[vt], ident), pf, Oacc[vt]);
        if constexpr (stream_pref<T, DT>()) cur = nxt;
        else if (kt + 1 < NT) cur = load_k(kt + 1);
    }
    if (q < p.T) {
#pragma unroll
        for (int vt = 0; vt < DT; ++vt) {
            f32x4 o4;
#pragma unroll
            for (int r = 0; r < 4; ++r) o4[r] = Oacc[vt][r] + to_f32(rf[vt].v[r]);
            st_frag<T>(reinterpret_cast<T*>(p.out) + ((long)id.b * p.T + q) * p.C + id.head * dh + vt * 16 + g4, o4);
        }
    }
}

template <typename T, int DT>
__global__ __launch_bounds__(256) void stream_sweep1_kernel(BwdP p, const float* stats) {
    constexpr int dh = 16 * DT;
    const int NT = (p.T + 15) / 16, E = p.E;
    TileId id;
    if (!tile_of_wave(p.B, p.H, NT, id)) return;
    const int lane = threadIdx.x & 63, g4 = (lane >> 4) * 4, l15 = lane & 15;
    const long ldq = 4 * (long)p.C;
    const T* qkvt = reinterpret_cast<const T*>(p.qkvt) + (long)id.b * p.T * ldq + id.head * dh + g4;
    const T* dout = reinterpret_cast<const T*>(p.d_out) + (long)id.b * p.T * p.C + id.head * dh + g4;
    const int64_t* ids = p.ids + (long)id.b * p.T;
    const uint8_t* marks = p.marks + (long)id.b * p.T * E;
    const int qt = id.t, q = qt * 16 + l15, qc = min(q, p.T - 1);
    const bool qok = q < p.T;
    const long row = id.bp * p.T + qc;
    const float cscale = p.qk_scale > 0.f ? p.qk_scale : rsqrtf((float)dh);
    const float c2 = cscale * 1.4426950408889634f;
    const bool causal = (p.flags & MAU_CAUSAL) != 0;
    const DropKey dk = make_dropkey(p.rng, p.stream_id, p.rate);
    const f32x4 zero4 = {0.f, 0.f, 0.f, 0.f};
    const PackDims pd = pack_dims<T>(dh, E);
    const float* iscs_g = reinterpret_cast<const float*>(p.pack + pd.off_f32) + 3 * pd.JE + EP;

    Frag4<T> qf[DT], dof[DT];
    load_rows<T, DT>(qf, qkvt, ldq, q, p.T);
    load_rows<T, DT>(dof, dout, p.C, q, p.T);
    if (!qok) {
#pragma unroll
        for (int ub = 0; ub < DT; ++ub) dof[ub] = frag_zero<T>();
    }
    const float4 z4v = *reinterpret_cast<const float4*>(p.z + row * EP + g4);
    const float zq4[4] = {z4v.x, z4v.y, z4v.z, z4v.w};
    float lam[4], dlx[4];
    Frag4<T> lf;
#pragma unroll
    for (int i = 0; i < 4; ++i) {
        const bool oke = qok && g4 + i < E;
        const long at = row * E + min(g4 + i, E - 1);
        lam[i] = oke ? p.lam[at] : 0.f;
        dlx[i] = (oke && p.d_lam_ext) ? p.d_lam_ext[at] : 0.f;
        lf.v[i] = from_f32<T>(lam[i]);
    }
    const float2 st = *reinterpret_cast<const float2*>(stats + row * 2);
    const float mx = st.x, pfac = st.y * dk.scale;
    const uint32_t dbase = (uint32_t)((id.bp * p.T + q) * p.T);
    const bool diag_on = !(p.flags & MAU_NO_DIAG);
    const float dval = (p.flags & MAU_DIAG_ZERO) ? 0.0f : 1.0f;

    struct KOps { Frag4<T> kf[DT], vf[DT], mf, mc; f32x4 madd; };
    auto load_k = [&](int kt) {
        KOps o;
        load_rows<T, DT>(o.kf, qkvt + p.C, ldq, kt * 16 + l15, p.T);
        load_rows<T, DT>(o.vf, qkvt + 2 * p.C, ldq, kt * 16 + l15, p.T);
        o.mf = marks_row_frag<T>(marks, E, p.T, kt * 16 + l15, g4);
        o.mc = marks_col_frag<T>(marks, E, p.T, kt * 16 + g4, l15);
        o.madd = key_madd(ids, p.T, kt * 16 + g4);
        return o;
    };
    float rowdot = 0.f;
    f32x4 dlamT = zero4;
    KOps cur = load_k(0);
    for (int kt = 0; kt < NT; ++kt) {
        KOps nxt;
        if constexpr (stream_pref<T, DT>()) nxt = load_k(min(kt + 1, NT - 1));
        const f32x4 v = score_tile<T, DT>(cur.kf, qf, cur.madd, c2, causal, kt * 16 + g4, q);
        const f32x4 gacc = mma16(cur.mf, lf, zero4);
        f32x4 da = zero4;
#pragma unroll
        for (int vb = 0; vb < DT; ++vb) da = mma16(cur.vf[vb], dof[vb], da);
        const bool dtile = diag_on && kt == qt;
        bool keep[4];
        keep4<T>(dk, dbase + kt * 16 + g4, keep);
        f32x4 dg;
#pragma unroll
        for (int r = 0; r < 4; ++r) {
            const bool dg_el = dtile && g4 + r == l15;
            const float gv = dg_el ? dval : gacc[r];
            const float fp = keep[r] ? __builtin_amdgcn_exp2f(v[r] - mx) * pfac : 0.f;
            const float d = da[r] * fp;
            rowdot = fmaf(d, gv, rowdot);
            dg[r] = dg_el ? 0.f : d;
        }
        dlamT = mma16(cur.mc, frag_from_acc<T>(dg), dlamT);
        if constexpr (stream_pref<T, DT>()) cur = nxt;
        else if (kt + 1 < NT) cur = load_k(kt + 1);
    }
    float dz4[4], dsc[4];
#pragma unroll
    for (int i = 0; i < 4; ++i) {
        const float dl = dlamT[i] + dlx[i];
        const float sg = sigmoid_f(zq4[i] * iscs_g[g4 + i]);
        dz4[i] = dl * sg;
        dsc[i] = (qok && g4 + i < E) ? dl * (lam[i] - zq4[i] * sg) : 0.f;
    }
    rowdot = group_sum4(rowdot);
#pragma unroll
    for (int i = 0; i < 4; ++i) {
        float s = dsc[i];
        s += __shfl_xor(s, 1, 64); s += __shfl_xor(s, 2, 64); s += __shfl_xor(s, 4, 64); s += __shfl_xor(s, 8, 64);
        dsc[i] = s;
    }
    if (qok) {
        *reinterpret_cast<float4*>(p.dz_ws + row * EP + g4) = make_float4(dz4[0], dz4[1], dz4[2], dz4[3]);
        if (lane < 16) p.rowdot_ws[row] = rowdot;
    }
    if (l15 == 0) *reinterpret_cast<float4*>(p.dsc_part + (id.bp * NT + qt) * EP + g4) = make_float4(dsc[0], dsc[1], dsc[2], dsc[3]);
}

template <typename T, int DT>
struct S2Q {
    Frag4<T> qf[DT], dof[DT];
    f32x4 dHq[DT];
    Frag4<T> lf;
    float mx, inv, rowdot;
};
template <typename T, int DT, bool FINAL>
__device__ __forceinline__ S2Q<T, DT> load_s2q(const BwdP& p, const float* stats, const TileId& id, int qt, int nyp, float scale, int lane) {
    constexpr int dh = 16 * DT;
    const int g4 = (lane >> 4) * 4, l15 = lane & 15, E = p.E;
    const long ldq = 4 * (long)p.C, R = (long)p.B * p.H * p.T;
    const int q = qt * 16 + l15;
    const bool qok = q < p.T;
    const long row = id.bp * p.T + min(q, p.T - 1);
    S2Q<T, DT> o;
    load_rows<T, DT>(o.qf, reinterpret_cast<const T*>(p.qkvt) + (long)id.b * p.T * ldq + id.head * dh + g4, ldq, q, p.T);
    load_rows<T, DT>(o.dof, reinterpret_cast<const T*>(p.d_out) + (long)id.b * p.T * p.C + id.head * dh + g4, p.C, q, p.T);
    float hdot = 0.f;
#pragma unroll
    for (int ub = 0; ub < DT; ++ub) {
        f32x4 a = {0.f, 0.f, 0.f, 0.f};
        for (int y = 0; y < nyp; ++y) {
            const float4 d = *reinterpret_cast<const float4*>(p.dh_ws + ((long)y * R + row) * dh + ub * 16 + g4);
            a[0] += d.x; a[1] += d.y; a[2] += d.z; a[3] += d.w;
        }
#pragma unroll
        for (int r = 0; r < 4; ++r) o.dHq[ub][r] = qok ? a[r] : 0.f;
        if (!qok) o.dof[ub] = frag_zero<T>();
        if constexpr (!FINAL) {
            const Frag4<T> hf = frag_ld<T>(reinterpret_cast<const T*>(p.hin) + row * dh + ub * 16 + g4);
#pragma unroll
            for (int r = 0; r < 4; ++r) hdot = fmaf(o.dHq[ub][r], to_f32(hf.v[r]), hdot);
        }
    }
#pragma unroll
    for (int i = 0; i < 4; ++i) o.lf.v[i] = from_f32<T>(g4 + i < E ? p.lam[row * E + g4 + i] * scale : 0.f);
    const float2 st = *reinterpret_cast<const float2*>(stats + row * 2);
    o.mx = st.x; o.inv = st.y;
    o.rowdot = qok ? p.rowdot_ws[row] : 0.f;
    if constexpr (!FINAL) o.rowdot += group_sum4(hdot);
    return o;
}
template <typename T, int DT>
__device__ __forceinline__ void s2_tile(const S2Q<T, DT>& qo, const Frag4<T> (&kf)[DT], const Frag4<T> (&tf)[DT], const Frag4<T> (&vf)[DT],
                                        const Frag4<T>& mf, const f32x4& madd, const DropKey& dk, uint32_t dbase, int flags, float cscale,
                                        int kt, int qt, int lane, f32x4& P, f32x4& ap, f32x4& ds) {
    const int g4 = (lane >> 4) * 4, l15 = lane & 15, q = qt * 16 + l15;
    const f32x4 zero4 = {0.f, 0.f, 0.f, 0.f};
    const bool causal = (flags & MAU_CAUSAL) != 0;
    const f32x4 v = score_tile<T, DT>(kf, qo.qf, madd, cscale * 1.4426950408889634f, causal, kt * 16 + g4, q);
    const f32x4 gacc = mma16(mf, qo.lf, zero4);
    f32x4 da = zero4;
#pragma unroll
    for (int vb = 0; vb < DT; ++vb) da = mma16(vf[vb], qo.dof[vb], da);
    const bool dtile = kt == qt && !(flags & MAU_NO_DIAG);
    const float dval = (flags & MAU_DIAG_ZERO) ? 0.0f : dk.scale;
    bool keep[4];
    keep4<T>(dk, dbase + kt * 16 + g4, keep);
    f32x4 a;
#pragma unroll
    for (int r = 0; r < 4; ++r) {
        const float gv = (dtile && g4 + r == l15) ? dval : gacc[r];
        P[r] = __builtin_amdgcn_exp2f(v[r] - qo.mx) * qo.inv;
        ap[r] = keep[r] ? gv * P[r] : 0.f;
        a[r] = keep[r] ? da[r] * gv : 0.f;
    }
#pragma unroll
    for (int ub = 0; ub < DT; ++ub) a = mma16(tf[ub], frag_from_acc<T>(qo.dHq[ub]), a);
#pragma unroll
    for (int r = 0; r < 4; ++r) {
        const bool replaced = madd[r] != 0.f || (causal && kt * 16 + g4 + r > q);
        ds[r] = replaced ? 0.f : P[r] * (a[r] - qo.rowdot) * cscale;
    }
}

template <typename T, int DT>
__global__ __launch_bounds__(256) void stream_sweep2q_kernel(BwdP p, const float* stats, int nyp) {
    constexpr int dh = 16 * DT;
    const int NT = (p.T + 15) / 16, E = p.E;
    TileId id;
    if (!tile_of_wave(p.B, p.H, NT, id)) return;
    const int lane = threadIdx.x & 63, g4 = (lane >> 4) * 4, l15 = lane & 15;
    const long ldq = 4 * (long)p.C;
    const T* qkvt = reinterpret_cast<const T*>(p.qkvt) + (long)id.b * p.T * ldq + id.head * dh + g4;
    const int64_t* ids = p.ids + (long)id.b * p.T;
    const uint8_t* marks = p.marks + (long)id.b * p.T * E;
    const int qt = id.t, q = qt * 16 + l15;
    const float cscale = p.qk_scale > 0.f ? p.qk_scale : rsqrtf((float)dh);
    const DropKey dk = make_dropkey(p.rng, p.stream_id, p.rate);
    const Frag4<T> ident = identity_frag<T>(lane);
    const f32x4 zero4 = {0.f, 0.f, 0.f, 0.f};
    const uint32_t dbase = (uint32_t)((id.bp * p.T + q) * p.T);
    const S2Q<T, DT> qo = load_s2q<T, DT, false>(p, stats, id, qt, nyp, dk.scale, lane);
    if (q < p.T && lane < 16) p.rowdot_ws[id.bp * p.T + q] = qo.rowdot;

    struct KOps { Frag4<T> kf[DT], tf[DT], vf[DT], mf; f32x4 madd; };
    auto load_k = [&](int kt) {
        KOps o;
        load_rows<T, DT>(o.kf, qkvt + p.C, ldq, kt * 16 + l15, p.T);
        load_rows<T, DT>(o.tf, qkvt + 3 * p.C, ldq, kt * 16 + l15, p.T);
        load_rows<T, DT>(o.vf, qkvt + 2 * p.C, ldq, kt * 16 + l15, p.T);
        o.mf = marks_row_frag<T>(marks, E, p.T, kt * 16 + l15, g4);
        o.madd = key_madd(ids, p.T, kt * 16 + g4);
        return o;
    };
    f32x4 dQ[DT];
#pragma unroll
    for (int ut = 0; ut < DT; ++ut) dQ[ut] = zero4;
    KOps cur = load_k(0);
    for (int kt = 0; kt < NT; ++kt) {
        KOps nxt;
        if constexpr (stream_pref<T, DT>()) nxt = load_k(min(kt + 1, NT - 1));
        f32x4 P, ap, ds;
        s2_tile<T, DT>(qo, cur.kf, cur.tf, cur.vf, cur.mf, cur.madd, dk, dbase, p.flags, cscale, kt, qt, lane, P, ap, ds);
        const Frag4<T> dsf = frag_from_acc<T>(ds);
#pragma unroll
// ... 136 lines not shown
```

easydgl_amd/engine.py:

```python
from __future__ import annotations

import ctypes
import os
from typing import Dict, Optional

import torch

from . import _lib, ops
from ._lib import check, lib
from .ops import _ptr, _stream

EPI_BIAS, EPI_GELU, EPI_SAVE_PRE, EPI_MUL_DGELU, EPI_ACCUM, EPI_OUT_F32 = 1, 2, 4, 8, 16, 32


class TrainEngine:
    _SIDE_STREAMS = {}

    def __init__(self, model, batch: int, use_graph: bool = True, process_group=None, fused_tail=None, flash_ce=None,
                 deterministic=None):
        if int(getattr(model, "train_negatives", 0) or 0) > 0:
            raise _lib.EdglError("TrainEngine: the static engine scores the whole catalogue; a model with train_negatives > 0 "
                                 "(sampled-softmax training, DESIGN 4.13) trains on the autograd path: model.train_step")
        if int(getattr(model, "shared_negatives", 0) or 0) > 0:
            raise _lib.EdglError("TrainEngine: the static engine scores the whole catalogue; a model with shared_negatives > 0 "
                                 "(sampled-softmax training, DESIGN 4.15) trains on the autograd path: model.train_step")
        if not getattr(model, "static_engine_ok", True):
            raise _lib.EdglError(f"TrainEngine: {type(model).__name__} is not run by the static engine (DESIGN 4.17: its step, with the "
                                 "model's own Adam hyper-parameters and gradient clipping, is model.train_step / graphed_train_step)")
        env = os.environ.get
        self.sw_flash_ce = env("EDGL_FLASH_CE", "1") != "0"
        self.sw_tpp_fused = env("EDGL_TPP_FUSED", "1") != "0"
        self.sw_prep_in_encoder = env("EDGL_PREP_IN_ENCODER", "1") != "0"
        self.sw_bimau_order = env("EDGL_BIMAU_ORDER", "0") == "1"
        self.sw_ce_parts = env("EDGL_CE_PARTS", "1") != "0"
        self.sw_defer_loss = env("EDGL_DEFER_LOSS", "1") != "0"
        self.sw_adam_ex = env("EDGL_ADAM_EX", "1") != "0"
        self.sw_reduce_ride = env("EDGL_REDUCE_RIDE", "1") != "0"
        self.sw_reduce_ride_behind = env("EDGL_REDUCE_RIDE", "1") == "2"
        self.sw_dx_encode = env("EDGL_DX_ENCODE", "1") != "0"
        self.sw_dw_ride = env("EDGL_DW_RIDE", "1") != "0"
        self.sw_score_strip = env("EDGL_SCORE_STRIP", "1") != "0"
        self.m = model
        self.B = batch
        self.use_graph = use_graph
        self.deterministic = bool(getattr(model, "deterministic", False)) if deterministic is None else bool(deterministic)
        self.group = process_group
        self.graph: Optional[torch.cuda.CUDAGraph] = None
        self.loader = None
        self._feed = False
        self._graph_feeds = False
        m = model
        dev = m._arena.device
        self.dev = dev
        self.dt = m.act_dtype
        self.code = ops._DT[self.dt]
        B, T, C, H, E, M, I = batch, m.seqslen, m.num_units, m.num_heads, m.num_events, m.masklen, m.num_items
        self.T, self.C, self.H, self.E, self.M, self.I = T, C, H, E, M, I
        self.pad = tuple(m.pad)
        self.c_true = int(m.width_true) if self.pad[0] else 0
        self.qk_scale = float(m.qk_scale)
        gmax = int(lib.edgl_bimau_mark_group(C, H, self.code))
        if gmax <= 0:
            raise _lib.EdglError(f"TrainEngine: head dim {C // H} / {self.dt} unsupported by the attention kernels")
        self.mgroups = [(e0, min(E, e0 + gmax)) for e0 in range(0, E, gmax)] if E > gmax else []
        self.R = B * M
        self.rows = B * T
        nb = len(m.layers)
        self.flash_ce = self.sw_flash_ce if flash_ce is None else bool(flash_ce)
        self.fused_tpp = (self.code == _lib.BF16 and C // H == 16 and E == 16 and not self.mgroups and M <= 256 and T <= 128
                          and m.ct_reg != 0.0 and self.flash_ce and nb > 0 and self.sw_tpp_fused)
        e = lambda *s, dtype=None: torch.empty(s, device=dev, dtype=dtype or self.dt)
        f32 = torch.float32
        self.ids = torch.zeros((B, T), device=dev, dtype=torch.int64)
        self.ts = torch.zeros((B, T), device=dev, dtype=f32)
        self.mpos = torch.zeros((B, M), device=dev, dtype=torch.int64)
        self.labels = torch.zeros((B, M), device=dev, dtype=torch.int64)
        self.x0 = e(B, T, 3 * C)
        self.spans = e(B, T, dtype=f32)
        self.marks = e(B, T, E, dtype=torch.uint8)
        self.blk = []
        for i in range(nb):
            d = dict(qkvt=e(B, T, 4 * C), att=e(B, T, C), lam=e(H * B, T, E, dtype=f32), ao=e(B, T, C), a1=e(B, T, C),
                     st1=e(B, 2, dtype=f32), pre_f=e(B, T, 2 * C), f=e(B, T, 2 * C), o=e(B, T, C), y=e(B, T, C),
                     st2=e(B, 2, dtype=f32),
                     pack=e(0 if self.mgroups else lib.edgl_bimau_pack_bytes(C, H, E, self.code), dtype=torch.uint8),
                     saved=e(0 if self.mgroups else lib.edgl_bimau_saved_bytes(B, T, C, H, self.code), dtype=torch.uint8),
                     dlam=None if self.fused_tpp else e(H * B, T, E, dtype=f32),
                     tpp_part=torch.zeros((B * H + 1, 2), device=dev, dtype=f32) if self.fused_tpp else None,
                     tpp=torch.zeros(max(lib.edgl_tpp_workspace(), lib.edgl_tpp_rows_workspace(B, H, M)), device=dev, dtype=f32))
            nb_bits = int(lib.edgl_bimau_dropbits_bytes(B, T, H)) if m.attention_probs_dropout_rate > 0 else 0
            d["dbits"] = e(nb_bits // 4, dtype=torch.int32) if nb_bits > 0 else None
            if self.mgroups:
                dh = C // H
                d["grp"] = []
                for (e0, e1) in self.mgroups:
                    eg = e1 - e0
                    d["grp"].append(dict(
                        marks=e(B, T, eg, dtype=torch.uint8), W1=e(dh + 1, dh * eg, dtype=f32), dW1=e(dh + 1, dh * eg, dtype=f32),
                        pack=e(lib.edgl_bimau_pack_bytes(C, H, eg, self.code), dtype=torch.uint8),
                        saved=e(lib.edgl_bimau_saved_bytes(B, T, C, H, self.code), dtype=torch.uint8),
                        lam=e(H * B, T, eg, dtype=f32), dlam=e(H * B, T, eg, dtype=f32),
                        out=e(B, T, C) if e0 else None, dqkvt=e(B, T, 4 * C) if e0 else None))
            self.blk.append(d)
        self.job_order = (torch.arange(2 * B, device=dev, dtype=torch.int32)
                          if (not self.mgroups and B <= 16384 and nb > 0 and self.sw_bimau_order) else None)
        self.tpp_desc = torch.zeros(int(lib.edgl_tpp_prep_bytes(B, T, M)), device=dev, dtype=torch.uint8) if self.fused_tpp else None
        self.zero_resid = torch.zeros((B, T, C), device=dev, dtype=self.dt) if self.mgroups else None
        self.pre_t, self.so, self.st3 = e(B, T, C), e(B, T, C), e(B, 2, dtype=f32)
        if m.ct_reg != 0.0 and (M > 256 or T > 1024):
            raise _lib.EdglError(f"TrainEngine: masklen {M} > 256 or T {T} > 1024 exceeds the fused TPP kernel (edgl_tpp_fwd_bwd_ex)")
        ok = bool(lib.edgl_tail_supported(T, C, self.code)) and M <= 256
        self.fused_tail = ok if fused_tail is None else (bool(fused_tail) and ok)
        self.tail_pack = [e(int(lib.edgl_tail_pack_elems(C))) for _ in range(nb)] if self.fused_tail else []
        if self.fused_tail:
            self.d_pre_t, self.d_o, self.d_pre_f, self.d_ao = e(B, T, C), e(B, T, C), e(B, T, 2 * C), e(B, T, C)
        self.ws_flash = e(int(lib.edgl_score_flash_workspace(self.R, C, I, I, self.code)), dtype=f32) if self.flash_ce else None
        self.hrows, self.hrows_c = e(self.R, C), e(self.R, C)
        self.hrows_c.zero_()
        self.labels_c = torch.zeros(self.R, device=dev, dtype=torch.int64)
        self.perm, self.inv = e(self.R, dtype=torch.int32), e(self.R, dtype=torch.int32)
        self.nvalid = torch.zeros(1, device=dev, dtype=torch.int32)
        self.lse, self.lab_logit, self.coef = e(self.R, dtype=f32), e(self.R, dtype=f32), e(self.R, dtype=f32)
        self.loss = e(1, dtype=f32)
        self.ce_nparts = int(lib.edgl_score_ce_nparts(self.R, C)) if (self.flash_ce and self.sw_ce_parts) else 0
        self.ce_part = torch.zeros(self.ce_nparts + 1, device=dev, dtype=f32) if self.ce_nparts > 0 else None
        self.loss_aux, self.loss_tpp = torch.zeros(1, device=dev, dtype=f32), torch.zeros(1, device=dev, dtype=f32)
        self.ws_l2 = e(1024, dtype=f32)
        self.l2_nparts = int(lib.edgl_adam_l2_parts(m._arena.numel()))
        self.l2_parts = [torch.zeros(self.l2_nparts, device=dev, dtype=f32) for _ in range(2)] \
            if (m.l2_reg != 0.0 and not use_graph and not self.deterministic) else None
        self._l2p_cur, self._l2p_ready = 0, False
        key = (dev.type, dev.index if dev.index is not None else torch.cuda.current_device())
        if key not in TrainEngine._SIDE_STREAMS:
            TrainEngine._SIDE_STREAMS[key] = (torch.cuda.Stream(device=dev), torch.cuda.Stream(device=dev))
        self.side, self.side2 = TrainEngine._SIDE_STREAMS[key]
        self._pending_loss = None
        self.accumulate_loss = False
        self.loss_sum = torch.zeros(1, device=dev, dtype=torch.float64)
        self._pending_label = None
        self._lazy_loss, self._side_has_grads, self._loss_unjoined = False, False, False
        self._label_fused = False
        self.mau_flags = _lib.MAU_NO_SKIP
        self.adam_ex = (not use_graph) and self.sw_adam_ex and not self.deterministic
        self.reduce_ride = self.sw_reduce_ride and not self.deterministic
# ... 176 lines not shown
                    for (e0, e1), gb in zip(self.mgroups, b["grp"]):
                        gb["W1"].copy_(att.st_kernel[:, e0 * dh:e1 * dh])
                        check(lib.edgl_bimau_pack(_ptr(gb["W1"]), _ptr(att.st_bias[e0 * dh:e1 * dh]), _ptr(att.weight[e0:e1]),
                                                  _ptr(att.scaling[e0:e1]), C, H, e1 - e0, _ptr(gb["pack"]), code, sst), "edgl_bimau_pack")
                else:
                    check(lib.edgl_bimau_pack(_ptr(att.st_kernel), _ptr(att.st_bias), _ptr(att.weight), _ptr(att.scaling), C, H, E,
                                              _ptr(b["pack"]), code, sst), "edgl_bimau_pack")
                if b["dbits"] is not None:
                    check(lib.edgl_bimau_dropbits(B, T, H, float(ad), _ptr(m._rng_state), 10 + 4 * i, _ptr(b["dbits"]), sst),
                          "edgl_bimau_dropbits")
            l2_behind = l2_from_parts and bool(self.blk)
            if not l2_behind:
                self._l2_term(l2_from_parts, sst)
            if not self.sw_prep_in_encoder:
                side.wait_stream(side2)
            ev_pack = side.record_event()
            if self._deferred_loss is not None:
                self._deferred_loss(sst)
                self._deferred_loss = None
            if l2_behind:
                self._l2_term(l2_from_parts, sst)
        return ev_pack

    def _issue_forward(self, main, ev_pack, drop, tab_c, st):
        m = self.m
        B, T, C, H, E, M, I, R = self.B, self.T, self.C, self.H, self.E, self.M, self.I, self.R
        code = self.code
        hd, ad = m.hidden_dropout_rate, m.attention_probs_dropout_rate
        d0 = drop(hd, 1)
        if self.sw_prep_in_encoder:
            check(lib.edgl_encode_fwd_prep(_ptr(self.ids), _ptr(self.ts), _ptr(tab_c), _ptr(m.pcoding.pembs.lookup_table),
                                           _ptr(m.mark_embs.lookup_table), _ptr(m.mark_lookup_table), _ptr(m.tcoding.scale), B, T, C,
                                           E, I, int(m.mask), float(m.time_scale), float(d0.rate), d0.ptr(), d0.stream_id,
                                           _ptr(self.x0), _ptr(self.spans), _ptr(self.marks), self.pad[0], self.pad[1],
                                           _ptr(self.labels), M, _ptr(self.perm), _ptr(self.inv), _ptr(self.nvalid), _ptr(self.labels_c),
                                           _ptr(self.mpos), _ptr(self.tpp_desc) if self.fused_tpp else None, code, st),
                  "edgl_encode_fwd_prep")
        else:
            check(lib.edgl_encode_fwd_ct(_ptr(self.ids), _ptr(self.ts), _ptr(tab_c), _ptr(m.pcoding.pembs.lookup_table),
                                         _ptr(m.mark_embs.lookup_table), _ptr(m.mark_lookup_table), _ptr(m.tcoding.scale), B, T, C,
                                         E, I, int(m.mask), float(m.time_scale), float(d0.rate), d0.ptr(), d0.stream_id,
                                         _ptr(self.x0), _ptr(self.spans), _ptr(self.marks), self.pad[0], self.pad[1], code, st),
                  "edgl_encode_fwd")
        x, cin = self.x0, 3 * C
        for i, (blk, b) in enumerate(zip(m.layers, self.blk)):
            att = blk.attention
            self._dense_fwd(x, att.dense_kernel, att.dense_bias, b["qkvt"], cin, 4 * C)
            if i == 0:
                main.wait_event(ev_pack)
            da = drop(ad, 10 + 4 * i)
            if self.mgroups:
                self._attention_fwd_groups(b, x, cin, da, st)
            else:
                check(lib.edgl_bimau_fwd_ord(_ptr(b["qkvt"]), x.data_ptr(), cin, _ptr(self.ids), _ptr(self.spans), _ptr(self.marks),
                                             _ptr(b["pack"]), B, T, C, H, E, float(da.rate), da.ptr(), da.stream_id, _ptr(b["dbits"]),
                                             self.qk_scale, _ptr(b["att"]), _ptr(b["lam"]), _ptr(b["saved"]),
                                             _ptr(b["dlam"]) if (m.ct_reg != 0.0 and not self.fused_tpp) else None, _ptr(self.job_order),
                                             self.mau_flags, code, st), "edgl_bimau_fwd_ord")
            if m.ct_reg != 0.0 and not self.fused_tpp:
                check(lib.edgl_tpp_fwd_bwd_rows(_ptr(b["lam"]), _ptr(self.mpos), _ptr(self.labels), _ptr(self.ts),
                                                _ptr(m.mark_lookup_table), B, T, H, E, M, float(m.ct_reg / H), _ptr(b["tpp"]),
                                                _ptr(self.loss_tpp), 1 if i > 0 else 0, _ptr(b["dlam"]), st), "edgl_tpp_fwd_bwd_rows")
            if self.fused_tail:
                last = i == len(self.blk) - 1
                pk = self.tail_pack[i]
                dh1 = drop(hd, 11 + 4 * i)
                check(lib.edgl_tail_fwd_ct(_ptr(b["att"]), x.data_ptr(), cin, _ptr(pk), _ptr(blk.att_out.bias), _ptr(blk.inter.bias),
                                        _ptr(blk.out.bias), _ptr(m.transform.bias), _ptr(blk.att_ln.gamma), _ptr(blk.att_ln.beta),
                                        _ptr(blk.out_ln.gamma), _ptr(blk.out_ln.beta), _ptr(m.transform_ln.gamma),
                                        _ptr(m.transform_ln.beta), B, T, C, float(dh1.rate), dh1.ptr(), 11 + 4 * i, 12 + 4 * i,
                                        _ptr(self.mpos), M, int(last), _ptr(b["ao"]), _ptr(b["a1"]), _ptr(b["st1"]), _ptr(b["pre_f"]),
                                        _ptr(b["f"]), _ptr(b["o"]), _ptr(b["y"]), _ptr(b["st2"]), _ptr(self.pre_t), _ptr(self.so),
                                        _ptr(self.st3), _ptr(self.hrows_c), _ptr(self.inv), self.pad[0], self.pad[1], code, st), "edgl_tail_fwd")
            else:
                self._dense_fwd(b["att"], blk.att_out.kernel, blk.att_out.bias, b["ao"], C, C)
                self._ln_fwd(b["ao"], x, cin, blk.att_ln, drop(hd, 11 + 4 * i), b["a1"], b["st1"])
                self._dense_fwd(b["a1"], blk.inter.kernel, blk.inter.bias, b["f"], C, 2 * C, gelu=True, pre=b["pre_f"])
                self._dense_fwd(b["f"], blk.out.kernel, blk.out.bias, b["o"], 2 * C, C)
                self._ln_fwd(b["o"], b["a1"], C, blk.out_ln, drop(hd, 12 + 4 * i), b["y"], b["st2"])
            x, cin = b["y"], C
        if not self.blk:
            main.wait_event(ev_pack)
        if not (self.fused_tail and self.blk):
            self._dense_fwd(x, m.transform.kernel, m.transform.bias, self.so, cin, C, gelu=True, pre=self.pre_t)
            self._ln_fwd(self.so, None, 0, m.transform_ln, ops.NO_DROP, self.hrows, self.st3, gpos=self.mpos)
        if not (self.fused_tail and self.blk):
            check(lib.edgl_compact_gather(_ptr(self.hrows), _ptr(self.labels), _ptr(self.perm), R, C, _ptr(self.hrows_c),
                                          _ptr(self.labels_c), code, st), "edgl_compact_gather")

    def _issue_scoring_fwd(self, tab_c, lab, st):
        m = self.m
        C, I, R, code = self.C, self.I, self.R, self.code
        aux = _ptr(self.loss_aux) if m.l2_reg != 0.0 else None
        tpp = _ptr(self.loss_tpp) if (m.ct_reg != 0.0 and self.blk) else None
        if self.flash_ce:
            wtot = self.counts.data_ptr() if self._dp else None
            check(lib.edgl_score_flash_fwd_rows_wp(_ptr(self.hrows_c), _ptr(tab_c), _ptr(m.output_bias), _ptr(lab), R, C, I,
                                                   _ptr(self.nvalid), wtot, None, _ptr(self.lse), _ptr(self.lab_logit), _ptr(self.coef),
                                                   _ptr(self.d_rows), _ptr(self.ce_part), _ptr(self.ws_flash), code, st),
                  "edgl_score_flash_fwd_rows")
            if self.ce_part is not None:
                self._pending_loss = lambda s, cp=self.ce_part: check(lib.edgl_ce_loss_parts(_ptr(cp), self.ce_nparts, _ptr(self.loss), aux,
                                                                                             tpp, wtot, s), "edgl_ce_loss_parts")
            else:
                self._pending_loss = lambda s: check(lib.edgl_ce_loss_fwd_add_w(_ptr(self.lse), _ptr(self.lab_logit), _ptr(lab), R,
                                                                                _ptr(self.loss), None, aux, tpp, wtot, s),
                                                     "edgl_ce_loss_fwd_add")
        else:
            check(lib.edgl_score_lse_fwd(_ptr(self.hrows_c), _ptr(tab_c), _ptr(m.output_bias), _ptr(lab), R, C, I, 0, I,
                                         _ptr(self.nvalid), _ptr(self.lse), _ptr(self.lab_logit), None, _ptr(self.ws), code, st),
                  "edgl_score_lse_fwd")
# ... 43 lines not shown
                                        _ptr(m.output_bias.grad), _ptr(self.ws), code, st), "edgl_score_ce_bwd")
        y_last, c_last = (self.blk[-1]["y"], C) if self.blk else (self.x0, 3 * C)
        if not (self.fused_tail and self.blk):
            self._ln_bwd(self.so, None, 0, m.transform_ln, self.st3, self.d_rows, ops.NO_DROP, self.G1, None, gpos=self.mpos,
                         rowmap=self.inv, act_pre=self.pre_t)
            self._dense_dw(y_last, self.G1, m.transform.kernel, m.transform.bias, c_last, C)
            self._dense_dx(self.G1, m.transform.kernel, self.G2 if self.blk else self.G3c, c_last, C)
        dY = self.G2 if self.blk else self.G3c
        for i in reversed(range(len(self.blk))):
            blk, b = m.layers[i], self.blk[i]
            x_in, cin = (self.x0, 3 * C) if i == 0 else (self.blk[i - 1]["y"], C)
            dh2, dh1 = drop(hd, 12 + 4 * i), drop(hd, 11 + 4 * i)
            if self.fused_tail:
                check(lib.edgl_gemm_dw_defer(1, st), "edgl_gemm_dw_defer")
                last = i == len(self.blk) - 1
                tl = m.transform_ln
                check(lib.edgl_tail_bwd_ct(x_in.data_ptr(), cin, _ptr(b["ao"]), _ptr(b["a1"]), _ptr(b["pre_f"]), _ptr(b["o"]),
                                        _ptr(self.pre_t), _ptr(self.so), _ptr(b["st1"]), _ptr(b["st2"]), _ptr(self.st3),
                                        _ptr(m.compute(blk.att_out.kernel)), _ptr(m.compute(blk.inter.kernel)),
                                        _ptr(m.compute(blk.out.kernel)), _ptr(m.compute(m.transform.kernel)),
                                        _ptr(blk.att_ln.gamma), _ptr(blk.out_ln.gamma), _ptr(tl.gamma), B, T, C, float(dh1.rate),
                                        dh1.ptr(), 11 + 4 * i, 12 + 4 * i, int(last), _ptr(self.d_rows), _ptr(self.mpos), M,
                                        _ptr(self.inv), None if last else _ptr(dY), _ptr(self.d_pre_t), _ptr(self.d_o),
                                        _ptr(self.d_pre_f), _ptr(self.d_ao), _ptr(self.G1), _ptr(self.G2),
                                        _ptr(blk.att_ln.gamma.grad), _ptr(blk.att_ln.beta.grad), _ptr(blk.out_ln.gamma.grad),
                                        _ptr(blk.out_ln.beta.grad), _ptr(tl.gamma.grad), _ptr(tl.beta.grad),
                                        _ptr(self._ws(lib.edgl_tail_bwd_workspace(B, C))), self.pad[0], self.pad[1], code, st), "edgl_tail_bwd")
                if self._pending_label is not None:
                    self.side.wait_stream(torch.cuda.current_stream())
                    self._pending_label(self.side.cuda_stream)
                    self._pending_label = None
                if last:
                    self._dense_dw(y_last, self.d_pre_t, m.transform.kernel, m.transform.bias, C, C)
                self._dense_dw(b["f"], self.d_o, blk.out.kernel, blk.out.bias, 2 * C, C)
                self._dense_dw(b["a1"], self.d_pre_f, blk.inter.kernel, blk.inter.bias, C, 2 * C)
                self._dense_dw(b["att"], self.d_ao, blk.att_out.kernel, blk.att_out.bias, C, C)
            else:
                self._ln_bwd(b["o"], b["a1"], C, blk.out_ln, b["st2"], dY, dh2, self.G3, self.G4 if dh2.active else None)
                d_o = self.G4 if dh2.active else self.G3
                self._dense_dw(b["f"], d_o, blk.out.kernel, blk.out.bias, 2 * C, C)
                self._dense_dx(d_o, blk.out.kernel, self.G2c, 2 * C, C, flags=EPI_MUL_DGELU, aux=b["pre_f"])
                self._dense_dw(b["a1"], self.G2c, blk.inter.kernel, blk.inter.bias, C, 2 * C)
                self._dense_dx(self.G2c, blk.inter.kernel, self.G3, C, 2 * C, flags=EPI_ACCUM)
                self._ln_bwd(b["ao"], x_in, cin, blk.att_ln, b["st1"], self.G3, dh1, self.G1, self.G4 if dh1.active else None)
                d_ao = self.G4 if dh1.active else self.G1
                self._dense_dw(b["att"], d_ao, blk.att_out.kernel, blk.att_out.bias, C, C)
                self._dense_dx(d_ao, blk.att_out.kernel, self.G2, C, C)
            att = blk.attention
            da = drop(ad, 10 + 4 * i)
            if self.mgroups:
                self._attention_bwd_groups(att, b, da, st)
            else:
                tp = self.fused_tpp
                check(lib.edgl_bimau_bwd_ord(_ptr(b["qkvt"]), _ptr(self.ids), _ptr(self.spans), _ptr(self.marks), _ptr(b["pack"]),
                                             _ptr(self.G2), None if tp else (_ptr(b["dlam"]) if m.ct_reg != 0.0 else None),
                                             _ptr(self.tpp_desc) if tp else None, M, (_ptr(b["tpp"]) if self._dp else None) if tp else None,
                                             float(m.ct_reg / H), _ptr(b["tpp_part"]) if tp else None,
                                             _ptr(b["lam"]), _ptr(b["saved"]), B, T, C, H, E,
                                             float(da.rate), da.ptr(), da.stream_id, _ptr(b["dbits"]), self.qk_scale, _ptr(self.G4c),
                                             _ptr(att.st_kernel.grad), _ptr(att.st_bias.grad), _ptr(att.weight.grad),
                                             _ptr(att.scaling.grad),
                                             _ptr(self._ws(lib.edgl_bimau_bwd_workspace(B, T, C, H, E, code), torch.uint8)),
                                             _ptr(self.job_order), self.mau_flags, code, st), "edgl_bimau_bwd_ord")
            self._dense_dw(x_in, self.G4c, att.dense_kernel, att.dense_bias, cin, 4 * C)
            dx_encode = i == 0 and self._label_fused and self.sw_dx_encode and not self.deterministic and cin == 3 * C and \
                bool(lib.edgl_dx_encode_supported(B, T, C, code))
            dw_ride = dx_encode and self.dw_ride and self.fused_tail and not self.mgroups
            if self.fused_tail and not dw_ride:
                check(lib.edgl_gemm_dw_defer(0, st), "edgl_gemm_dw_defer")
            d_in = self.G3c if i == 0 else self.G3
            if dx_encode:
                self._issue_backward_end()
                if self.reduce_ride:
                    check(lib.edgl_reduce_ride(2 if self.sw_reduce_ride_behind else 1), "edgl_reduce_ride")
                if dw_ride:
                    check(lib.edgl_gemm_dw_ride(1), "edgl_gemm_dw_ride")
                d0 = drop(hd, 1)
                check(lib.edgl_dx_encode_bwd_label(_ptr(self.G4c), _ptr(self.m.compute(att.dense_kernel)), 4 * C, 4 * C, None,
                                                   _ptr(self.ids), _ptr(self.marks), _ptr(self.G1), _ptr(self.G2), B, T, C, E, I,
                                                   float(d0.rate), d0.ptr(), d0.stream_id, _ptr(tab.grad),
                                                   _ptr(m.pcoding.pembs.lookup_table.grad), _ptr(m.mark_embs.lookup_table.grad),
                                                   _ptr(self._ws(lib.edgl_encode_bwd_workspace(B, T, C))), self.c_true,
                                                   _ptr(self.hrows_c), _ptr(lab), _ptr(self.coef), _ptr(self.nvalid), R,
                                                   _ptr(m.output_bias.grad), code, st), "edgl_dx_encode_bwd_label")
                if dw_ride:
                    check(lib.edgl_gemm_dw_defer(0, st), "edgl_gemm_dw_defer")
                return
            self._dense_dx(self.G4c, att.dense_kernel, d_in, cin, 4 * C)
            if i == 0:
                self._issue_backward_end()
            if i > 0:
                check(lib.edgl_add_cols(_ptr(d_in), cin, _ptr(self.G1), _ptr(self.G2), C, self.rows, C, code, st), "edgl_add_cols")
                self.G2.copy_(self.G3)
                dY = self.G2
            else:
                dY = d_in
        d0 = drop(hd, 1)
        add1, add2 = (self.G1, self.G2) if self.blk else (None, None)
        if self.deterministic:
            check(lib.edgl_encode_bwd_add_det(_ptr(self.ids), _ptr(self.marks), _ptr(dY), _ptr(add1), _ptr(add2), B, T, C, E, I,
                                              float(d0.rate), d0.ptr(), d0.stream_id, _ptr(tab.grad), _ptr(m.pcoding.pembs.lookup_table.grad),
                                              _ptr(m.mark_embs.lookup_table.grad), _ptr(self._ws(lib.edgl_encode_bwd_workspace(B, T, C))),
                                              self.c_true, _ptr(self.plan_emb), code, st), "edgl_encode_bwd_add_det")
            return
        if self.reduce_ride:
            check(lib.edgl_reduce_ride(2 if self.sw_reduce_ride_behind else 1), "edgl_reduce_ride")
        if self._label_fused:
            check(lib.edgl_encode_bwd_add_label(_ptr(self.ids), _ptr(self.marks), _ptr(dY), _ptr(add1), _ptr(add2), B, T, C, E, I,
                                                float(d0.rate), d0.ptr(), d0.stream_id, _ptr(tab.grad),
                                                _ptr(m.pcoding.pembs.lookup_table.grad), _ptr(m.mark_embs.lookup_table.grad),
                                                _ptr(self._ws(lib.edgl_encode_bwd_workspace(B, T, C))), self.c_true,
                                                _ptr(self.hrows_c), _ptr(lab), _ptr(self.coef), _ptr(self.nvalid), R,
                                                _ptr(m.output_bias.grad), code, st), "edgl_encode_bwd_add_label")
        else:
            check(lib.edgl_encode_bwd_add_ct(_ptr(self.ids), _ptr(self.marks), _ptr(dY), _ptr(add1), _ptr(add2), B, T, C, E, I,
                                             float(d0.rate), d0.ptr(), d0.stream_id, _ptr(tab.grad), _ptr(m.pcoding.pembs.lookup_table.grad),
# ... 264 lines not shown
```

include/easydgl_hip.h:

```cpp
#ifndef EASYDGL_HIP_H
#define EASYDGL_HIP_H

#include <stdint.h>

#ifdef __cplusplus
extern "C" {
#endif

typedef enum { EDGL_F32 = 0, EDGL_BF16 = 1 } edgl_dtype;

enum {
    EDGL_OK = 0,
    EDGL_ERR_SHAPE = -1,
    EDGL_ERR_DTYPE = -2,
    EDGL_ERR_LAUNCH = -3,
    EDGL_ERR_NULL = -4,
    EDGL_ERR_WORKSPACE = -5
};

enum {
    EDGL_EPI_BIAS = 1,
    EDGL_EPI_GELU = 2,
    EDGL_EPI_SAVE_PRE = 4,
    EDGL_EPI_MUL_DGELU = 8,
// ... 89 lines not shown
int edgl_gemm(const void* A, const void* Bm, void* Cm, int M, int N, int K, int lda, int ldb, int ldc,
              int a_kc, int b_kc, const float* bias, void* aux, int epi_flags, int splitk, float* workspace,
              int dtype, void* stream);

long edgl_gemm_dw_workspace(int R, int Kf, int N, int dtype);
int edgl_gemm_dw(const void* X, const void* dY, float* dW, float* dbias, int R, int Kf, int N, int ldx, int ldy,
                 int accumulate, float* workspace, int dtype, void* stream);
int edgl_gemm_dw_defer(int on, void* stream);
int edgl_gemm_dw_ride(int on);

int edgl_colsum(const void* X, int M, int N, int ld, float* out, int accumulate, float* workspace,
                int x_f32, int dtype, void* stream);

#define EDGL_MAU_CAUSAL 1
#define EDGL_MAU_NO_DIAG 2
#define EDGL_MAU_DIAG_ZERO 4
#define EDGL_MAU_NO_SKIP 8
#define EDGL_MAU_STREAM 16
int edgl_bimau_form(int T, int C, int H, int dtype, int flags);
long edgl_bimau_pack_bytes(int C, int H, int E, int dtype);
long edgl_bimau_saved_bytes(int B, int T, int C, int H, int dtype);
long edgl_bimau_saved_bytes_ex(int B, int T, int C, int H, int dtype, int flags);
int edgl_bimau_mark_group(int C, int H, int dtype);
int edgl_bimau_pack(const float* W1, const float* b1, const float* w, const float* scaling, int C, int H, int E,
                    void* pack, int dtype, void* stream);
int edgl_bimau_fwd(const void* qkvt, const void* resid, int ld_res, const int64_t* ids, const float* spans,
                   const uint8_t* marks, const void* pack, int B, int T, int C, int H, int E, float drop_rate,
                   const uint64_t* rng_state, uint32_t stream_id, void* out, float* lam_out, void* saved,
                   int flags, int dtype, void* stream);
int edgl_bimau_fwd_zr(const void* qkvt, const void* resid, int ld_res, const int64_t* ids, const float* spans,
                      const uint8_t* marks, const void* pack, int B, int T, int C, int H, int E, float drop_rate,
                      const uint64_t* rng_state, uint32_t stream_id, void* out, float* lam_out, void* saved,
                      float* zero_rows, int flags, int dtype, void* stream);

long edgl_bimau_dropbits_bytes(int B, int T, int H);
int edgl_bimau_dropbits(int B, int T, int H, float drop_rate, const uint64_t* rng_state, uint32_t stream_id, uint32_t* bits,
                        void* stream);
int edgl_bimau_fwd_db(const void* qkvt, const void* resid, int ld_res, const int64_t* ids, const float* spans,
                      const uint8_t* marks, const void* pack, int B, int T, int C, int H, int E, float drop_rate,
                      const uint64_t* rng_state, uint32_t stream_id, const uint32_t* dropbits, float qk_scale, void* out,
                      float* lam_out, void* saved, float* zero_rows, int flags, int dtype, void* stream);

int edgl_bimau_job_order(const int64_t* ids, int B, int T, int32_t* order, void* stream);
int edgl_bimau_fwd_ord(const void* qkvt, const void* resid, int ld_res, const int64_t* ids, const float* spans,
                       const uint8_t* marks, const void* pack, int B, int T, int C, int H, int E, float drop_rate,
                       const uint64_t* rng_state, uint32_t stream_id, const uint32_t* dropbits, float qk_scale, void* out,
                       float* lam_out, void* saved, float* zero_rows, const int32_t* order, int flags, int dtype, void* stream);
int edgl_bimau_bwd_ord(const void* qkvt, const int64_t* ids, const float* spans, const uint8_t* marks, const void* pack,
                       const void* d_out, const float* d_lam_ext, const void* tpp_desc, int M, const float* tpp_sums, float coef,
                       float* tpp_part, const float* lam, const void* saved, int B, int T, int C, int H, int E, float drop_rate,
                       const uint64_t* rng_state, uint32_t stream_id, const uint32_t* dropbits, float qk_scale, void* d_qkvt,
                       float* dW1, float* db1, float* dw, float* dscaling, void* workspace, const int32_t* order, int flags,
                       int dtype, void* stream);

long edgl_bimau_bwd_workspace(int B, int T, int C, int H, int E, int dtype);
long edgl_bimau_bwd_workspace_ex(int B, int T, int C, int H, int E, int dtype, int flags);
int edgl_bimau_bwd(const void* qkvt, const int64_t* ids, const float* spans, const uint8_t* marks,
                   const void* pack, const void* d_out, const float* d_lam_ext, const float* lam,
                   const void* saved, int B, int T, int C, int H, int E, float drop_rate,
                   const uint64_t* rng_state, uint32_t stream_id, void* d_qkvt, float* dW1, float* db1,
                   float* dw, float* dscaling, void* workspace, int flags, int dtype, void* stream);
int edgl_bimau_bwd_db(const void* qkvt, const int64_t* ids, const float* spans, const uint8_t* marks,
                      const void* pack, const void* d_out, const float* d_lam_ext, const float* lam,
                      const void* saved, int B, int T, int C, int H, int E, float drop_rate,
                      const uint64_t* rng_state, uint32_t stream_id, const uint32_t* dropbits, float qk_scale, void* d_qkvt,
                      float* dW1, float* db1, float* dw, float* dscaling, void* workspace, int flags, int dtype, void* stream);

int edgl_add_layernorm_fwd(const void* x, const void* resid, int ld_res, const float* gamma,
                           const float* beta, int B, int T, int C, float drop_rate,
                           const uint64_t* rng_state, uint32_t stream_id, const int64_t* gather_pos,
                           int Mg, void* y, float* stats, int dtype, void* stream);

int edgl_add_layernorm_bwd(const void* x, const void* resid, int ld_res, const float* gamma,
                           const float* stats, const void* dy, int B, int T, int C, float drop_rate,
                           const uint64_t* rng_state, uint32_t stream_id, const int64_t* gather_pos,
                           int Mg, const int32_t* dy_rowmap, void* dsum, void* dx_drop, float* dgamma,
                           float* dbeta, float* workspace, int dtype, void* stream);
int edgl_add_layernorm_bwd_act(const void* x, const void* resid, int ld_res, const float* gamma,
                               const float* stats, const void* dy, int B, int T, int C, float drop_rate,
                               const uint64_t* rng_state, uint32_t stream_id, const int64_t* gather_pos,
                               int Mg, const int32_t* dy_rowmap, const void* act_pre, void* dsum, void* dx_drop,
                               float* dgamma, float* dbeta, float* workspace, int dtype, void* stream);
int edgl_add_layernorm_fwd_ct(const void* x, const void* resid, int ld_res, const float* gamma, const float* beta, int B, int T,
                              int C, float drop_rate, const uint64_t* rng_state, uint32_t stream_id, const int64_t* gather_pos,
                              int Mg, void* y, float* stats, int dh_pad, int dh_true, int dtype, void* stream);
int edgl_add_layernorm_bwd_act_ct(const void* x, const void* resid, int ld_res, const float* gamma, const float* stats,
                                  const void* dy, int B, int T, int C, float drop_rate, const uint64_t* rng_state,
                                  uint32_t stream_id, const int64_t* gather_pos, int Mg, const int32_t* dy_rowmap,
                                  const void* act_pre, void* dsum, void* dx_drop, float* dgamma, float* dbeta, float* workspace,
                                  int dh_pad, int dh_true, int dtype, void* stream);

int edgl_score_chunks(int R, int n_items);
int edgl_compact_rows(const void* rows, const int64_t* labels, int R, int C, int32_t* perm, int32_t* inv,
                      int32_t* nvalid, void* rows_c, int64_t* labels_c, int dtype, void* stream);
int edgl_compact_scan(const int64_t* labels, int R, int32_t* perm, int32_t* inv, int32_t* nvalid, void* stream);
int edgl_compact_scan_labels(const int64_t* labels, int R, int32_t* perm, int32_t* inv, int32_t* nvalid, int64_t* labels_c,
                             void* stream);
int edgl_compact_gather(const void* rows, const int64_t* labels, const int32_t* perm, int R, int C, void* rows_c,
                        int64_t* labels_c, int dtype, void* stream);
int edgl_scatter_rows(const void* rows_c, const int32_t* inv, int R, int C, void* rows, int dtype,
                      void* stream);
int edgl_score_lse_fwd(const void* rows, const void* table, const float* out_bias, const int64_t* labels,
                       int R, int C, int I, int i0, int i1, const int32_t* nvalid, float* row_lse,
                       float* label_logit, float* logits, float* workspace, int dtype, void* stream);
int edgl_ce_loss_fwd(const float* row_lse, const float* label_logit, const int64_t* labels, int R,
                     float* loss_out, float* coef, void* stream);
// ... 322 lines not shown
```

Baseline: 755,200.

## Save softmax row max and inverse sum in forward for reuse in backward

The forward attention kernel now writes each query row's softmax max and inverse normalizer to a small stats buffer. Both backward sweeps can then rebuild probabilities directly from these saved statistics, skipping the max and sum reductions, when the bidirectional, unskipped, 16-mark form is in use. This adds a small global write in forward and a read per row in backward, in exchange for fewer cross-lane reductions. New API entry points and an engine buffer route the stats through.

```diff
diff --git a/easydgl_amd/_lib.py b/easydgl_amd/_lib.py
--- a/easydgl_amd/_lib.py
+++ b/easydgl_amd/_lib.py
@@ -72,6 +72,9 @@
     "edgl_bimau_job_order": (I, [P, I, I, P, P]),
     "edgl_bimau_fwd_ord": (I, [P, P, I, P, P, P, P, I, I, I, I, I, F, P, U32, P, F, P, P, P, P, P, I, I, P]),
     "edgl_bimau_bwd_ord": (I, [P, P, P, P, P, P, P, P, I, P, F, P, P, P, I, I, I, I, I, F, P, U32, P, F, P, P, P, P, P, P, P, I, I, P]),
+    "edgl_bimau_stats_bytes": (L, [I, I, I, I, I, I]),
+    "edgl_bimau_fwd_st": (I, [P, P, I, P, P, P, P, I, I, I, I, I, F, P, U32, P, F, P, P, P, P, P, P, I, I, P]),
+    "edgl_bimau_bwd_st": (I, [P, P, P, P, P, P, P, P, I, P, F, P, P, P, I, I, I, I, I, F, P, U32, P, F, P, P, P, P, P, P, P, P, I, I, P]),
     "edgl_bimau_bwd_workspace": (L, [I, I, I, I, I, I]),
     "edgl_bimau_bwd": (I, [P, P, P, P, P, P, P, P, P, I, I, I, I, I, F, P, U32, P, P, P, P, P, P, I, I, P]),
     "edgl_add_layernorm_fwd": (I, [P, P, I, P, P, I, I, I, F, P, U32, P, I, P, P, I, P]),
diff --git a/easydgl_amd/csrc/bimau_bwd_impl.h b/easydgl_amd/csrc/bimau_bwd_impl.h
--- a/easydgl_amd/csrc/bimau_bwd_impl.h
+++ b/easydgl_amd/csrc/bimau_bwd_impl.h
@@ -53,6 +53,7 @@
     float qk_scale;
     const void* tpp_desc; int tpp_M; const float* tpp_sums; float tpp_coef;
     const int32_t* order;
+    const float* stats;
     float* tpp_part;
 };
 
@@ -63,8 +64,9 @@
     else *reinterpret_cast<uint2*>(dst) = *reinterpret_cast<uint2*>(&f);
 }
 
-template <typename T, int DT, int NT, int EC, bool PREF = true, int FL = -1, bool DB = false, bool TP = false, bool SK = false>
+template <typename T, int DT, int NT, int EC, bool PREF = true, int FL = -1, bool DB = false, bool TP = false, bool SK = false, bool ST = false>
 __global__ __launch_bounds__(256) void bimau_bwd_sweep1_kernel(BwdP p) {
+    static_assert(!ST || (FL == 0 && !SK), "row statistics: the bidirectional, unskipped form");
     constexpr int dh = 16 * DT, Tp = 16 * NT, LDT = Tp + 4;
     extern __shared__ __attribute__((aligned(16))) char smem[];
     const int E = EC ? EC : p.E;
@@ -112,7 +114,7 @@
     const Frag4<T> ident = identity_frag<T>(lane);
     const f32x4 zero4 = {0.f, 0.f, 0.f, 0.f};
 
-    struct QOps { Frag4<T> qf[DT], dof[DT]; float4 z; float lam[4], dlx[4]; uint32_t kb; uint32_t nmw; float spr; };
+    struct QOps : StatOps<ST> { Frag4<T> qf[DT], dof[DT]; float4 z; float lam[4], dlx[4]; uint32_t kb; uint32_t nmw; float spr; };
     const float* dlx_src = p.d_lam_ext ? p.d_lam_ext : p.lam;
     const float dlx_on = p.d_lam_ext ? 1.0f : 0.0f;
     TppDesc td{};
@@ -143,6 +145,7 @@
         }
         o.z = *reinterpret_cast<const float4*>(p.z + row * EP + g4);
         if constexpr (DB) o.kb = p.dbits[(bp * NT + qt) * 64 + lane];
+        if constexpr (ST) { const float2 st = *reinterpret_cast<const float2*>(p.stats + row * 2); o.mx = st.x; o.inv = st.y; }
         if constexpr (TP) {
             const float4 l4 = *reinterpret_cast<const float4*>(p.lam + row * EC + g4);
             o.lam[0] = l4.x; o.lam[1] = l4.y; o.lam[2] = l4.z; o.lam[3] = l4.w;
@@ -223,7 +226,8 @@
                 a = mma16(frag_ld<T>(Ks + ((K0 + kt) * 16 + l15) * dh + cw[ub]), qcur.qf[ub], a);
             s[kt] = a;
         }
-        if constexpr (FL == 0) masked_softmax_impl<NK, false, false>(s, kmk, cscale, lane, q, dk.scale);
+        if constexpr (ST) masked_softmax_from_stats<NK>(s, kmk, cscale, lane, qcur.mx, qcur.inv * dk.scale);
+        else if constexpr (FL == 0) masked_softmax_impl<NK, false, false>(s, kmk, cscale, lane, q, dk.scale);
         else {
             masked_softmax<NK, 0>(s, kmk, cscale, lane, q, (p.flags & MAU_CAUSAL) != 0);
 #pragma unroll
@@ -344,8 +348,10 @@
     PH_FLUSH(0);
 }
 
-template <typename T, int DT, int NT, int EC, int NYP = KY_NY, bool PREF = true, int FL = -1, bool DB = false, int US = 1, int SL = 0, bool SK = false>
+template <typename T, int DT, int NT, int EC, int NYP = KY_NY, bool PREF = true, int FL = -1, bool DB = false, int US = 1, int SL = 0, bool SK = false,
+          bool ST = false>
 __global__ __launch_bounds__(256) void bimau_bwd_sweep2_kernel(BwdP p) {
+    static_assert(!ST || (FL == 0 && !SK), "row statistics: the bidirectional, unskipped form");
     constexpr int dh = 16 * DT, Tp = 16 * NT, LDT = Tp + 4;
     static_assert(DT % US == 0 && SL < US, "channel slices");
     constexpr int DTS = DT / US, U0 = SL * DTS;
@@ -399,7 +405,7 @@
     const f32x4 zero4 = {0.f, 0.f, 0.f, 0.f};
     const long R = (long)p.B * p.H * p.T;
 
-    struct QOps { Frag4<T> qf[DT], dof[DT], hf[DT]; float4 dHp[DT][NYP]; float lam[4], rowdot; uint32_t kb; };
+    struct QOps : StatOps<ST> { Frag4<T> qf[DT], dof[DT], hf[DT]; float4 dHp[DT][NYP]; float lam[4], rowdot; uint32_t kb; };
     auto load_q = [&](int qt) {
         QOps o;
         const int q = min(qt * 16 + l15, p.T - 1);
@@ -422,6 +428,7 @@
         }
         o.rowdot = p.rowdot_ws[row];
         if constexpr (DB) o.kb = p.dbits[(bp * NT + qt) * 64 + lane];
+        if constexpr (ST) { const float2 st = *reinterpret_cast<const float2*>(p.stats + row * 2); o.mx = st.x; o.inv = st.y; }
         return o;
     };
     PH_DECL
@@ -485,7 +492,8 @@
             s[kt] = a;
         }
         PH_MARK(5);
-        if constexpr (FL == 0) masked_softmax_impl<NK, false, false>(s, kmk, cscale, lane, q);
+        if constexpr (ST) masked_softmax_from_stats<NK>(s, kmk, cscale, lane, qcur.mx, qcur.inv);
+        else if constexpr (FL == 0) masked_softmax_impl<NK, false, false>(s, kmk, cscale, lane, q);
         else masked_softmax<NK, 0>(s, kmk, cscale, lane, q, (p.flags & MAU_CAUSAL) != 0);
         asm volatile("" ::: "memory");
         flush_pending();
diff --git a/easydgl_amd/csrc/bimau_common.h b/easydgl_amd/csrc/bimau_common.h
--- a/easydgl_amd/csrc/bimau_common.h
+++ b/easydgl_amd/csrc/bimau_common.h
@@ -205,7 +205,8 @@
 constexpr int MAU_DIAG_ZERO = 4;
 typedef __attribute__((ext_vector_type(2))) float f32x2;
 template <int NT, bool CAUSAL, bool VEC, bool NORM = true>
-__device__ __forceinline__ float masked_softmax_impl(f32x4 (&s)[NT], const KeyMask<NT>& km, float cscale, int lane, int q, float post = 1.0f) {
+__device__ __forceinline__ float masked_softmax_impl(f32x4 (&s)[NT], const KeyMask<NT>& km, float cscale, int lane, int q, float post = 1.0f,
+                                                     float* mx_out = nullptr) {
     const float c2 = cscale * 1.4426950408889634f;
     float mx = -INFINITY;
     const float* mrow = km.madd + (lane >> 4) * 4;
@@ -228,6 +229,7 @@
         mx = fmaxf(fmaxf(mx, v[0]), fmaxf(v[1], fmaxf(v[2], v[3])));
     }
     mx = group_max4(mx);
+    if (mx_out) *mx_out = mx;
     float sum;
     if constexpr (VEC) {
         const f32x4 mx4 = {mx, mx, mx, mx};
@@ -308,6 +310,21 @@
             for (int r = 0; r < 4; ++r) s[kt][r] *= inv;
     }
 }
+
+__device__ __forceinline__ float softmax_from_stats(float v, float mx, float f) { return __builtin_amdgcn_exp2f(v - mx) * f; }
+template <int NT>
+__device__ __forceinline__ void masked_softmax_from_stats(f32x4 (&s)[NT], const KeyMask<NT>& km, float cscale, int lane, float mx, float f) {
+    const float c2 = cscale * 1.4426950408889634f;
+    const float* mrow = km.madd + (lane >> 4) * 4;
+#pragma unroll
+    for (int kt = 0; kt < NT; ++kt) {
+        const f32x4 m4 = *reinterpret_cast<const f32x4*>(mrow + kt * 16);
+#pragma unroll
+        for (int r = 0; r < 4; ++r) s[kt][r] = softmax_from_stats(fmaf(s[kt][r], c2, m4[r]), mx, f);
+    }
+}
+template <bool ST> struct StatOps {};
+template <> struct StatOps<true> { float mx, inv; };
 
 template <int I>
 __device__ __forceinline__ float keep_bit_c(uint32_t kb, float x) {
diff --git a/easydgl_amd/csrc/bimau_fwd_impl.h b/easydgl_amd/csrc/bimau_fwd_impl.h
--- a/easydgl_amd/csrc/bimau_fwd_impl.h
+++ b/easydgl_amd/csrc/bimau_fwd_impl.h
@@ -22,6 +22,7 @@
     float qk_scale;
     const int32_t* order;
     int noskip;
+    float* stats_out;
 };
 
 template <typename T, int DT, int NT, int PHASE>
@@ -138,13 +139,13 @@
                 a = mma16(frag_ld<T>(Ks + ((K0 + kt) * 16 + l15) * dh + cw[ub]), qf[ub], a);
             s[kt] = a;
         }
-        float pinv = 1.0f;
+        float pinv = 1.0f, pmx = 0.f;
         if constexpr (TR) {
             if constexpr (K0 == 0) {
-                if (p.flags & MAU_CAUSAL) pinv = masked_softmax_impl<NT, true, false, false>(s, kmk, cscale, lane, q);
-                else pinv = masked_softmax_impl<NT, false, false, false>(s, kmk, cscale, lane, q);
+                if (p.flags & MAU_CAUSAL) pinv = masked_softmax_impl<NT, true, false, false>(s, kmk, cscale, lane, q, 1.0f, &pmx);
+                else pinv = masked_softmax_impl<NT, false, false, false>(s, kmk, cscale, lane, q, 1.0f, &pmx);
             } else {
-                pinv = masked_softmax_impl<NK, false, false, false>(s, kmk, cscale, lane, q);
+                pinv = masked_softmax_impl<NK, false, false, false>(s, kmk, cscale, lane, q, 1.0f, &pmx);
             }
         } else {
             masked_softmax<NT, 0>(s, kmk, cscale, lane, q, (p.flags & MAU_CAUSAL) != 0);
@@ -263,6 +264,9 @@
         float z4[4];
         reduce_scatter16(zp, z4, lane);
         if (p.z_out && qok) *reinterpret_cast<float4*>(p.z_out + (bp * p.T + q) * EP + g4) = make_float4(z4[0], z4[1], z4[2], z4[3]);
+        if constexpr (TR) {
+            if (p.stats_out && qok && g4 == 0) *reinterpret_cast<float2*>(p.stats_out + (bp * p.T + q) * 2) = make_float2(pmx, pinv);
+        }
         float lam4[4];
 #pragma unroll
         for (int i = 0; i < 4; ++i) {
diff --git a/easydgl_amd/csrc/k_bimau_bwd.hip b/easydgl_amd/csrc/k_bimau_bwd.hip
--- a/easydgl_amd/csrc/k_bimau_bwd.hip
+++ b/easydgl_amd/csrc/k_bimau_bwd.hip
@@ -368,6 +368,10 @@
                     if (sk) kern = db ? bimau_bwd_sweep1_kernel<T, DT, NT, 16, true, 0, true, true, SKC> : bimau_bwd_sweep1_kernel<T, DT, NT, 16, true, 0, false, true, SKC>;
                     else kern = db ? bimau_bwd_sweep1_kernel<T, DT, NT, 16, true, 0, true, true> : bimau_bwd_sweep1_kernel<T, DT, NT, 16, true, 0, false, true>;
                 }
+                if (p.stats && p.flags == 0 && p.E == 16 && !sk) {
+                    if (p.tpp_desc) kern = db ? bimau_bwd_sweep1_kernel<T, DT, NT, 16, true, 0, true, true, false, true> : bimau_bwd_sweep1_kernel<T, DT, NT, 16, true, 0, false, true, false, true>;
+                    else kern = db ? bimau_bwd_sweep1_kernel<T, DT, NT, 16, true, 0, true, false, false, true> : bimau_bwd_sweep1_kernel<T, DT, NT, 16, true, 0, false, false, false, true>;
+                }
             }
         }
         EDGL_LDS_LIMIT(kern, smem, "edgl_bimau_bwd");
@@ -394,6 +398,9 @@
                 const bool sk = SKC && p.flags == 0 && p.E == 16 && bimau_skip_enabled() && !p.noskip;
                 if (p.flags == 0 && p.E == 16 && p.dbits && p.rate > 0.f) kern = sk ? bimau_bwd_sweep2_kernel<T, DT, NT, 16, KY_NY, true, 0, true, 1, 0, SKC> : bimau_bwd_sweep2_kernel<T, DT, NT, 16, KY_NY, true, 0, true>;
                 else if (sk) kern = bimau_bwd_sweep2_kernel<T, DT, NT, 16, KY_NY, true, 0, false, 1, 0, SKC>;
+                if (p.stats && p.flags == 0 && p.E == 16 && !sk)
+                    kern = (p.dbits && p.rate > 0.f) ? bimau_bwd_sweep2_kernel<T, DT, NT, 16, KY_NY, true, 0, true, 1, 0, false, true>
+                                                     : bimau_bwd_sweep2_kernel<T, DT, NT, 16, KY_NY, true, 0, false, 1, 0, false, true>;
             }
         }
         EDGL_LDS_LIMIT(kern, smem, "edgl_bimau_bwd");
@@ -480,7 +487,8 @@
                           const void* saved, int B, int T, int C, int H, int E, float drop_rate,
                           const uint64_t* rng_state, uint32_t stream_id, const uint32_t* dropbits, float qk_scale, void* d_qkvt,
                           float* dW1, float* db1, float* dw, float* dscaling, void* workspace, const void* tpp_desc, int tpp_M,
-                          const float* tpp_sums, float tpp_coef, float* tpp_part, const int32_t* order, int flags, int dtype, void* stream) {
+                          const float* tpp_sums, float tpp_coef, float* tpp_part, const int32_t* order, const float* stats, int flags, int dtype,
+                          void* stream) {
     EDGL_REQUIRE(qkvt && ids && spans && marks && pack && d_out && lam && saved && d_qkvt && dW1 && db1 && dw && dscaling && workspace,
                  EDGL_ERR_NULL, "edgl_bimau_bwd: null pointer");
     EDGL_REQUIRE(B > 0 && T > 0 && H > 0 && C % H == 0 && E >= 1 && E <= bimau::EP, EDGL_ERR_SHAPE,
@@ -498,6 +506,7 @@
     p.noskip = (flags & EDGL_MAU_NO_SKIP) ? 1 : 0; flags &= ~EDGL_MAU_NO_SKIP;
     p.stream_id = stream_id; p.d_qkvt = d_qkvt; p.flags = flags; p.dbits = dropbits; p.qk_scale = qk_scale;
     p.tpp_desc = tpp_desc; p.tpp_M = tpp_M; p.tpp_sums = tpp_sums; p.tpp_coef = tpp_coef; p.tpp_part = tpp_part; p.order = order;
+    p.stats = stats;
     EDGL_REQUIRE(!tpp_desc || (dtype == EDGL_BF16 && C / H == 16 && E == 16 && T <= 128 && flags == 0 && tpp_part && tpp_M > 0 && !d_lam_ext),
                  EDGL_ERR_SHAPE, "edgl_bimau_bwd_tpp: the fused TPP form exists for bf16, head dim 16, 16 marks, T <= 128, BiMAU flags "
                  "(C/H=%d E=%d T=%d flags=%d)", C / H, E, T, flags);
@@ -536,7 +545,7 @@
                                  const uint64_t* rng_state, uint32_t stream_id, const uint32_t* dropbits, float qk_scale, void* d_qkvt,
                                  float* dW1, float* db1, float* dw, float* dscaling, void* workspace, int flags, int dtype, void* stream) {
     return bimau_bwd_impl(qkvt, ids, spans, marks, pack, d_out, d_lam_ext, lam, saved, B, T, C, H, E, drop_rate, rng_state, stream_id,
-                          dropbits, qk_scale, d_qkvt, dW1, db1, dw, dscaling, workspace, nullptr, 0, nullptr, 0.f, nullptr, nullptr, flags, dtype, stream);
+                          dropbits, qk_scale, d_qkvt, dW1, db1, dw, dscaling, workspace, nullptr, 0, nullptr, 0.f, nullptr, nullptr, nullptr, flags, dtype, stream);
 }
 extern "C" int edgl_bimau_bwd_tpp(const void* qkvt, const int64_t* ids, const float* spans, const uint8_t* marks,
                                   const void* pack, const void* d_out, const void* tpp_desc, int M, const float* tpp_sums, float coef,
@@ -545,18 +554,34 @@
                                   float* dW1, float* db1, float* dw, float* dscaling, void* workspace, int flags, int dtype, void* stream) {
     EDGL_REQUIRE(tpp_desc && tpp_part, EDGL_ERR_NULL, "edgl_bimau_bwd_tpp: null pointer");
     return bimau_bwd_impl(qkvt, ids, spans, marks, pack, d_out, nullptr, lam, saved, B, T, C, H, E, drop_rate, rng_state, stream_id,
-                          dropbits, qk_scale, d_qkvt, dW1, db1, dw, dscaling, workspace, tpp_desc, M, tpp_sums, coef, tpp_part, nullptr, flags, dtype,
+                          dropbits, qk_scale, d_qkvt, dW1, db1, dw, dscaling, workspace, tpp_desc, M, tpp_sums, coef, tpp_part, nullptr, nullptr, flags, dtype,
                           stream);
 }
+extern "C" int edgl_bimau_bwd_st(const void* qkvt, const int64_t* ids, const float* spans, const uint8_t* marks, const void* pack,
+                                 const void* d_out, const float* d_lam_ext, const void* tpp_desc, int M, const float* tpp_sums, float coef,
+                                 float* tpp_part, const float* lam, const void* saved, int B, int T, int C, int H, int E, float drop_rate,
+                                 const uint64_t* rng_state, uint32_t stream_id, const uint32_t* dropbits, float qk_scale, void* d_qkvt,
+                                 float* dW1, float* db1, float* dw, float* dscaling, void* workspace, const int32_t* order, const float* stats,
+                                 int flags, int dtype, void* stream);
 extern "C" int edgl_bimau_bwd_ord(const void* qkvt, const int64_t* ids, const float* spans, const uint8_t* marks, const void* pack,
                                   const void* d_out, const float* d_lam_ext, const void* tpp_desc, int M, const float* tpp_sums, float coef,
                                   float* tpp_part, const float* lam, const void* saved, int B, int T, int C, int H, int E, float drop_rate,
                                   const uint64_t* rng_state, uint32_t stream_id, const uint32_t* dropbits, float qk_scale, void* d_qkvt,
                                   float* dW1, float* db1, float* dw, float* dscaling, void* workspace, const int32_t* order, int flags,
                                   int dtype, void* stream) {
+    return edgl_bimau_bwd_st(qkvt, ids, spans, marks, pack, d_out, d_lam_ext, tpp_desc, M, tpp_sums, coef, tpp_part, lam, saved, B, T, C, H, E,
+                             drop_rate, rng_state, stream_id, dropbits, qk_scale, d_qkvt, dW1, db1, dw, dscaling, workspace, order, nullptr, flags,
+                             dtype, stream);
+}
+extern "C" int edgl_bimau_bwd_st(const void* qkvt, const int64_t* ids, const float* spans, const uint8_t* marks, const void* pack,
+                                 const void* d_out, const float* d_lam_ext, const void* tpp_desc, int M, const float* tpp_sums, float coef,
+                                 float* tpp_part, const float* lam, const void* saved, int B, int T, int C, int H, int E, float drop_rate,
+                                 const uint64_t* rng_state, uint32_t stream_id, const uint32_t* dropbits, float qk_scale, void* d_qkvt,
+                                 float* dW1, float* db1, float* dw, float* dscaling, void* workspace, const int32_t* order, const float* stats,
+                                 int flags, int dtype, void* stream) {
     EDGL_REQUIRE(!tpp_desc || tpp_part, EDGL_ERR_NULL, "edgl_bimau_bwd_ord: tpp_desc without tpp_part");
     return bimau_bwd_impl(qkvt, ids, spans, marks, pack, d_out, d_lam_ext, lam, saved, B, T, C, H, E, drop_rate, rng_state, stream_id,
-                          dropbits, qk_scale, d_qkvt, dW1, db1, dw, dscaling, workspace, tpp_desc, M, tpp_sums, coef, tpp_part, order, flags,
+                          dropbits, qk_scale, d_qkvt, dW1, db1, dw, dscaling, workspace, tpp_desc, M, tpp_sums, coef, tpp_part, order, stats, flags,
                           dtype, stream);
 }
 
diff --git a/easydgl_amd/csrc/k_bimau_fwd.hip b/easydgl_amd/csrc/k_bimau_fwd.hip
--- a/easydgl_amd/csrc/k_bimau_fwd.hip
+++ b/easydgl_amd/csrc/k_bimau_fwd.hip
@@ -59,6 +59,11 @@
                                   float drop_rate, const uint64_t* rng_state, uint32_t stream_id, const uint32_t* dropbits, float qk_scale,
                                   void* out, float* lam_out, void* saved, float* zero_rows, const int32_t* order, int flags, int dtype,
                                   void* stream);
+extern "C" int edgl_bimau_fwd_st(const void* qkvt, const void* resid, int ld_res, const int64_t* ids, const float* spans,
+                                 const uint8_t* marks, const void* pack, int B, int T, int C, int H, int E,
+                                 float drop_rate, const uint64_t* rng_state, uint32_t stream_id, const uint32_t* dropbits, float qk_scale,
+                                 void* out, float* lam_out, void* saved, float* zero_rows, const int32_t* order, float* stats, int flags,
+                                 int dtype, void* stream);
 
 extern "C" long edgl_bimau_dropbits_bytes(int B, int T, int H) {
     if (B <= 0 || T <= 0 || H <= 0) return -1;
@@ -168,6 +173,21 @@
                                   float drop_rate, const uint64_t* rng_state, uint32_t stream_id, const uint32_t* dropbits, float qk_scale,
                                   void* out, float* lam_out, void* saved, float* zero_rows, const int32_t* order, int flags, int dtype,
                                   void* stream) {
+    return edgl_bimau_fwd_st(qkvt, resid, ld_res, ids, spans, marks, pack, B, T, C, H, E, drop_rate, rng_state, stream_id, dropbits, qk_scale,
+                             out, lam_out, saved, zero_rows, order, nullptr, flags, dtype, stream);
+}
+
+extern "C" long edgl_bimau_stats_bytes(int B, int T, int C, int H, int dtype, int flags) {
+    if (B <= 0 || T <= 0 || H <= 0 || C <= 0 || C % H) return -1;
+    if (dtype != EDGL_BF16 || C / H != 16 || T > 128) return 0;
+    if ((flags & ~(EDGL_MAU_NO_SKIP)) != 0 || bimau::bimau_form(T, C, H, dtype, flags) != 0) return 0;
+    return (long)B * H * T * 2 * (long)sizeof(float);
+}
+extern "C" int edgl_bimau_fwd_st(const void* qkvt, const void* resid, int ld_res, const int64_t* ids, const float* spans,
+                                 const uint8_t* marks, const void* pack, int B, int T, int C, int H, int E,
+                                 float drop_rate, const uint64_t* rng_state, uint32_t stream_id, const uint32_t* dropbits, float qk_scale,
+                                 void* out, float* lam_out, void* saved, float* zero_rows, const int32_t* order, float* stats, int flags,
+                                 int dtype, void* stream) {
     EDGL_REQUIRE(qkvt && resid && ids && spans && marks && pack && out && lam_out, EDGL_ERR_NULL,
                  "edgl_bimau_fwd: null pointer");
     EDGL_REQUIRE(B > 0 && T > 0 && H > 0 && C % H == 0 && E >= 1 && E <= bimau::EP, EDGL_ERR_SHAPE,
@@ -215,6 +235,7 @@
         const bimau::SavedLayout sl = bimau::saved_layout(B, T, C, H, dtype == EDGL_BF16 ? 2 : 4);
         p.hin_out = (char*)saved + sl.off_hin;
         p.z_out = reinterpret_cast<float*>((char*)saved + sl.off_z);
+        if (dtype == EDGL_BF16 && C / H == 16 && E == 16 && T <= 128 && flags == 0) p.stats_out = stats;
     }
     EDGL_REQUIRE(dtype == EDGL_F32 || dtype == EDGL_BF16, EDGL_ERR_DTYPE, "edgl_bimau_fwd: bad dtype %d", dtype);
     edgl_prof_begin(EDGL_KERNEL_BIMAU_FWD, st);
diff --git a/easydgl_amd/csrc/k_bimau_stream.hip b/easydgl_amd/csrc/k_bimau_stream.hip
--- a/easydgl_amd/csrc/k_bimau_stream.hip
+++ b/easydgl_amd/csrc/k_bimau_stream.hip
@@ -203,7 +203,7 @@
 #pragma unroll
         for (int r = 0; r < 4; ++r) {
             const float g = (dtile && g4 + r == l15) ? dval : gacc[r];
-            s[r] = g * __builtin_amdgcn_exp2f(v[r] - mx);
+            s[r] = g * softmax_from_stats(v[r], mx, 1.0f);
         }
         if (dk.thresh != 0u) {
             bool keep[4];
@@ -305,7 +305,7 @@
         for (int r = 0; r < 4; ++r) {
             const bool dg_el = dtile && g4 + r == l15;
             const float gv = dg_el ? dval : gacc[r];
-            const float fp = keep[r] ? __builtin_amdgcn_exp2f(v[r] - mx) * pfac : 0.f;
+            const float fp = keep[r] ? softmax_from_stats(v[r], mx, pfac) : 0.f;
             const float d = da[r] * fp;
             rowdot = fmaf(d, gv, rowdot);
             dg[r] = dg_el ? 0.f : d;
@@ -399,7 +399,7 @@
 #pragma unroll
     for (int r = 0; r < 4; ++r) {
         const float gv = (dtile && g4 + r == l15) ? dval : gacc[r];
-        P[r] = __builtin_amdgcn_exp2f(v[r] - qo.mx) * qo.inv;
+        P[r] = softmax_from_stats(v[r], qo.mx, qo.inv);
         ap[r] = keep[r] ? gv * P[r] : 0.f;
         a[r] = keep[r] ? da[r] * gv : 0.f;
     }
diff --git a/easydgl_amd/engine.py b/easydgl_amd/engine.py
--- a/easydgl_amd/engine.py
+++ b/easydgl_amd/engine.py
@@ -15,6 +15,7 @@
 
 class TrainEngine:
     _SIDE_STREAMS = {}
+    sw_bimau_stats = True
 
     def __init__(self, model, batch: int, use_graph: bool = True, process_group=None, fused_tail=None, flash_ce=None,
                  deterministic=None):
@@ -40,6 +41,7 @@
         self.sw_dx_encode = env("EDGL_DX_ENCODE", "1") != "0"
         self.sw_dw_ride = env("EDGL_DW_RIDE", "1") != "0"
         self.sw_score_strip = env("EDGL_SCORE_STRIP", "1") != "0"
+        self.sw_bimau_stats = bool(type(self).sw_bimau_stats)
         self.m = model
         self.B = batch
         self.use_graph = use_graph
@@ -90,6 +92,8 @@
                      tpp=torch.zeros(max(lib.edgl_tpp_workspace(), lib.edgl_tpp_rows_workspace(B, H, M)), device=dev, dtype=f32))
             nb_bits = int(lib.edgl_bimau_dropbits_bytes(B, T, H)) if m.attention_probs_dropout_rate > 0 else 0
             d["dbits"] = e(nb_bits // 4, dtype=torch.int32) if nb_bits > 0 else None
+            nb_stats = int(lib.edgl_bimau_stats_bytes(B, T, C, H, self.code, _lib.MAU_NO_SKIP)) if (self.sw_bimau_stats and not self.mgroups) else 0
+            d["stats"] = e(nb_stats // 4, dtype=f32) if nb_stats > 0 else None
             if self.mgroups:
                 dh = C // H
                 d["grp"] = []
@@ -372,11 +376,11 @@
             if self.mgroups:
                 self._attention_fwd_groups(b, x, cin, da, st)
             else:
-                check(lib.edgl_bimau_fwd_ord(_ptr(b["qkvt"]), x.data_ptr(), cin, _ptr(self.ids), _ptr(self.spans), _ptr(self.marks),
-                                             _ptr(b["pack"]), B, T, C, H, E, float(da.rate), da.ptr(), da.stream_id, _ptr(b["dbits"]),
-                                             self.qk_scale, _ptr(b["att"]), _ptr(b["lam"]), _ptr(b["saved"]),
-                                             _ptr(b["dlam"]) if (m.ct_reg != 0.0 and not self.fused_tpp) else None, _ptr(self.job_order),
-                                             self.mau_flags, code, st), "edgl_bimau_fwd_ord")
+                check(lib.edgl_bimau_fwd_st(_ptr(b["qkvt"]), x.data_ptr(), cin, _ptr(self.ids), _ptr(self.spans), _ptr(self.marks),
+                                            _ptr(b["pack"]), B, T, C, H, E, float(da.rate), da.ptr(), da.stream_id, _ptr(b["dbits"]),
+                                            self.qk_scale, _ptr(b["att"]), _ptr(b["lam"]), _ptr(b["saved"]),
+                                            _ptr(b["dlam"]) if (m.ct_reg != 0.0 and not self.fused_tpp) else None, _ptr(self.job_order),
+                                            _ptr(b["stats"]), self.mau_flags, code, st), "edgl_bimau_fwd_st")
             if m.ct_reg != 0.0 and not self.fused_tpp:
                 check(lib.edgl_tpp_fwd_bwd_rows(_ptr(b["lam"]), _ptr(self.mpos), _ptr(self.labels), _ptr(self.ts),
                                                 _ptr(m.mark_lookup_table), B, T, H, E, M, float(m.ct_reg / H), _ptr(b["tpp"]),
@@ -526,16 +530,16 @@
                 self._attention_bwd_groups(att, b, da, st)
             else:
                 tp = self.fused_tpp
-                check(lib.edgl_bimau_bwd_ord(_ptr(b["qkvt"]), _ptr(self.ids), _ptr(self.spans), _ptr(self.marks), _ptr(b["pack"]),
-                                             _ptr(self.G2), None if tp else (_ptr(b["dlam"]) if m.ct_reg != 0.0 else None),
-                                             _ptr(self.tpp_desc) if tp else None, M, (_ptr(b["tpp"]) if self._dp else None) if tp else None,
-                                             float(m.ct_reg / H), _ptr(b["tpp_part"]) if tp else None,
-                                             _ptr(b["lam"]), _ptr(b["saved"]), B, T, C, H, E,
-                                             float(da.rate), da.ptr(), da.stream_id, _ptr(b["dbits"]), self.qk_scale, _ptr(self.G4c),
-                                             _ptr(att.st_kernel.grad), _ptr(att.st_bias.grad), _ptr(att.weight.grad),
-                                             _ptr(att.scaling.grad),
-                                             _ptr(self._ws(lib.edgl_bimau_bwd_workspace(B, T, C, H, E, code), torch.uint8)),
-                                             _ptr(self.job_order), self.mau_flags, code, st), "edgl_bimau_bwd_ord")
+                check(lib.edgl_bimau_bwd_st(_ptr(b["qkvt"]), _ptr(self.ids), _ptr(self.spans), _ptr(self.marks), _ptr(b["pack"]),
+                                            _ptr(self.G2), None if tp else (_ptr(b["dlam"]) if m.ct_reg != 0.0 else None),
+                                            _ptr(self.tpp_desc) if tp else None, M, (_ptr(b["tpp"]) if self._dp else None) if tp else None,
+                                            float(m.ct_reg / H), _ptr(b["tpp_part"]) if tp else None,
+                                            _ptr(b["lam"]), _ptr(b["saved"]), B, T, C, H, E,
+                                            float(da.rate), da.ptr(), da.stream_id, _ptr(b["dbits"]), self.qk_scale, _ptr(self.G4c),
+                                            _ptr(att.st_kernel.grad), _ptr(att.st_bias.grad), _ptr(att.weight.grad),
+                                            _ptr(att.scaling.grad),
+                                            _ptr(self._ws(lib.edgl_bimau_bwd_workspace(B, T, C, H, E, code), torch.uint8)),
+                                            _ptr(self.job_order), _ptr(b["stats"]), self.mau_flags, code, st), "edgl_bimau_bwd_st")
             self._dense_dw(x_in, self.G4c, att.dense_kernel, att.dense_bias, cin, 4 * C)
             dx_encode = i == 0 and self._label_fused and self.sw_dx_encode and not self.deterministic and cin == 3 * C and \
                 bool(lib.edgl_dx_encode_supported(B, T, C, code))
diff --git a/include/easydgl_hip.h b/include/easydgl_hip.h
--- a/include/easydgl_hip.h
+++ b/include/easydgl_hip.h
@@ -165,6 +165,19 @@
                        const uint64_t* rng_state, uint32_t stream_id, const uint32_t* dropbits, float qk_scale, void* d_qkvt,
                        float* dW1, float* db1, float* dw, float* dscaling, void* workspace, const int32_t* order, int flags,
                        int dtype, void* stream);
+
+long edgl_bimau_stats_bytes(int B, int T, int C, int H, int dtype, int flags);
+int edgl_bimau_fwd_st(const void* qkvt, const void* resid, int ld_res, const int64_t* ids, const float* spans,
+                      const uint8_t* marks, const void* pack, int B, int T, int C, int H, int E, float drop_rate,
+                      const uint64_t* rng_state, uint32_t stream_id, const uint32_t* dropbits, float qk_scale, void* out,
+                      float* lam_out, void* saved, float* zero_rows, const int32_t* order, float* stats, int flags, int dtype,
+                      void* stream);
+int edgl_bimau_bwd_st(const void* qkvt, const int64_t* ids, const float* spans, const uint8_t* marks, const void* pack,
+                      const void* d_out, const float* d_lam_ext, const void* tpp_desc, int M, const float* tpp_sums, float coef,
+                      float* tpp_part, const float* lam, const void* saved, int B, int T, int C, int H, int E, float drop_rate,
+                      const uint64_t* rng_state, uint32_t stream_id, const uint32_t* dropbits, float qk_scale, void* d_qkvt,
+                      float* dW1, float* db1, float* dw, float* dscaling, void* workspace, const int32_t* order, const float* stats,
+                      int flags, int dtype, void* stream);
 
 long edgl_bimau_bwd_workspace(int B, int T, int C, int H, int E, int dtype);
 long edgl_bimau_bwd_workspace_ex(int B, int T, int C, int H, int E, int dtype, int flags);
```

After: 760,600, median of 6. About the same (+0.7%).
